# Junshuai-Song/Graph-Embedding

Hardware: AMD Instinct MI355X
Metric: walk-steps/sec (node2vec) (higher is better)
Workload: dtype int32 ids / f64 accept tests

## Files before the change

### graph-embedding_amd/csrc/gw_capi.cpp

```cpp
#include <stdarg.h>
#include <stdio.h>
#include <string.h>

#include <algorithm>
#include <string>
#include <vector>

#include <hip/hip_runtime_api.h>

#include "gw_internal.h"

int gw_load_edgelist_impl(gw_graph* g, const char* path, const char* delim, int semantics,
                          int directed, int weighted, int64_t vcount);
int gw_rmat_impl(gw_graph* g, int scale, int edge_factor, double a, double b, double c,
                 uint64_t seed);
int gw_rmat_java_impl(gw_graph* g, int64_t n, int64_t m, double a, double b, double c, uint64_t seed);
int gw_write_walks_impl(const gw_graph* g, const char* path, const int32_t* walks,
                        const int32_t* lens, int64_t nwalks, int walk_len, std::string* err);
int gw_write_sim_dense_impl(const char* path, const double* rows, const int32_t* row_ids,
                            int64_t nrows, int64_t n, int topk, const std::string& sep,
                            int decimals, std::string* err);
int gw_write_sim_topk_impl(const char* path, const int32_t* ids, const double* scores,
                           const int32_t* row_ids, int64_t nrows, int topk,
                           const std::string& sep, int decimals, std::string* err);
void gw_java_double_to_string(double v, std::string* out);
int gw_write_sim_cachemap_impl(const char* path, const int32_t* keys, const float* vals, const int32_t* sizes,
                               const int32_t* row_ids, int64_t nrows, int capacity, int topk,
                               const std::string& sep, std::string* err);
void gw_select_fixed_max_pq_impl(const double* rows, int64_t nrows, int64_t n, int k, double min_score,
                                 int32_t* out_ids);
int gw_hip_device_count(int* count);

static thread_local std::string tls_err;

void gw_set_tls_error(const std::string& s) { tls_err = s; }

int gw_fail(gw_graph* g, int code, const char* fmt, ...) {
  char buf[1024];
  va_list ap;
  va_start(ap, fmt);
  vsnprintf(buf, sizeof buf, fmt, ap);
  va_end(ap);
  if (g) g->err = buf;
  tls_err = buf;
  return code;
}

static int ret(gw_graph* g, int rc) {
  if (rc != GW_OK && g) tls_err = g->err;
  return rc;
}

extern "C" {

const char* gw_version(void) { return "graphwalk 0.1.0 (gfx950)"; }

const char* gw_last_error(const gw_graph* g) {
  if (g) return g->err.c_str();
  return tls_err.c_str();
}

const char* gw_strerror(int code) {
  switch (code) {
    case GW_OK: return "ok";
    case GW_ERR_INVALID: return "invalid argument";
    case GW_ERR_IO: return "I/O error";
    case GW_ERR_PARSE: return "parse error";
    case GW_ERR_NOMEM: return "out of memory";
    case GW_ERR_DEVICE: return "HIP device error";
    case GW_ERR_STATE: return "invalid call order";
    case GW_ERR_UNSUPPORTED: return "unsupported";
    case GW_ERR_RANGE: return "id out of range";
    case GW_ERR_KEY: return "missing key";
    case GW_ERR_ZERODIV: return "division by zero";
    case GW_ERR_CAPACITY: return "capacity exceeded";
    default: return "unknown error";
  }
}

gw_device_guard::gw_device_guard(int dev) {
  if (dev < 0) return;
  int cur = -1;
  if (hipGetDevice(&cur) != hipSuccess) {
    ok = false;
    return;
  }
  if (cur == dev) return;
  if (hipSetDevice(dev) != hipSuccess) {
    ok = false;
    return;
  }
  prev = cur;
}
gw_device_guard::~gw_device_guard() {
  if (prev >= 0) (void)hipSetDevice(prev);
}

int gw_device_count(int* count) {
  if (!count) return gw_fail(nullptr, GW_ERR_INVALID, "count is NULL");
  int rc = gw_hip_device_count(count);
  if (rc != GW_OK) return gw_fail(nullptr, rc, "no HIP device visible");
  return GW_OK;
}

int gw_graph_load_edgelist(const char* path, const char* delim, int semantics, int directed,
                           int weighted, int64_t vcount, gw_graph** out) {
  if (!path || !out) return gw_fail(nullptr, GW_ERR_INVALID, "path/out is NULL");
  *out = nullptr;
  if (semantics == GW_SEM_JAVA_MULTI && (weighted || directed))
    return gw_fail(nullptr, GW_ERR_UNSUPPORTED, "JAVA_MULTI graphs are undirected and unweighted (Graph.java:12)");
  gw_graph* g = new gw_graph();
  int rc = gw_load_edgelist_impl(g, path, delim, semantics, directed, weighted, vcount);
  if (rc != GW_OK) {
    tls_err = g->err;
    delete g;
    return rc;
  }
  *out = g;
  return GW_OK;
}

int gw_graph_from_edges(int64_t m, const int64_t* src, const int64_t* dst, const double* w,
                        int semantics, int directed, int64_t vcount, gw_graph** out) {
  if (!out || m < 0 || (m > 0 && (!src || !dst))) return gw_fail(nullptr, GW_ERR_INVALID, "bad edge arrays");
  *out = nullptr;
  gw_graph* g = new gw_graph();
  int rc;
  if (semantics == GW_SEM_NX_SIMPLE)
    rc = gw_build_nx_simple(g, m, src, dst, w, directed);
  else if (semantics == GW_SEM_JAVA_MULTI)
    rc = (w || directed) ? gw_fail(g, GW_ERR_UNSUPPORTED, "JAVA_MULTI graphs are undirected and unweighted")
                         : gw_build_java_multi(g, m, src, dst, vcount);
  else
    rc = gw_fail(g, GW_ERR_INVALID, "unknown semantics %d", semantics);
  if (rc != GW_OK) {
    tls_err = g->err;
    delete g;
    return rc;
  }
  *out = g;
  return GW_OK;
}

int gw_graph_from_csr(int64_t n, const int64_t* offsets, const int32_t* nbrs, const double* weights,
                      const int64_t* labels, const int32_t* node_order, int semantics, int directed,
                      gw_graph** out) {
  if (!out || n < 0 || !offsets) return gw_fail(nullptr, GW_ERR_INVALID, "bad CSR arguments");
  *out = nullptr;
  if (semantics != GW_SEM_NX_SIMPLE && semantics != GW_SEM_JAVA_MULTI)
    return gw_fail(nullptr, GW_ERR_INVALID, "unknown semantics %d", semantics);
  if (n >= (int64_t)INT32_MAX) return gw_fail(nullptr, GW_ERR_UNSUPPORTED, "too many vertices");
  if (offsets[0] != 0) return gw_fail(nullptr, GW_ERR_INVALID, "offsets[0] != 0");
  for (int64_t v = 0; v < n; ++v)
    if (offsets[v + 1] < offsets[v]) return gw_fail(nullptr, GW_ERR_INVALID, "offsets not monotone at %lld", (long long)v);
  const int64_t nnz = offsets[n];
  if (nnz > 0 && !nbrs) return gw_fail(nullptr, GW_ERR_INVALID, "nbrs is NULL");
  for (int64_t v = 0; v < n; ++v)
    for (int64_t k = offsets[v]; k < offsets[v + 1]; ++k) {
      if (nbrs[k] < 0 || nbrs[k] >= n) return gw_fail(nullptr, GW_ERR_RANGE, "neighbour id %d out of range", nbrs[k]);
      if (semantics == GW_SEM_NX_SIMPLE && k > offsets[v] && nbrs[k] <= nbrs[k - 1])
        return gw_fail(nullptr, GW_ERR_INVALID, "NX_SIMPLE rows must be strictly increasing (row %lld)", (long long)v);
    }
  gw_graph* g = new gw_graph();
  g->semantics = semantics;
  g->directed = directed ? 1 : 0;
  g->weighted = weights ? 1 : 0;
  g->n = n;
  g->nnz = nnz;
  g->offsets.assign(offsets, offsets + n + 1);
  g->nbrs.assign(nbrs, nbrs + nnz);
  if (weights) g->weights.assign(weights, weights + nnz);
  g->labels.resize(n);
  g->order.resize(n);
  std::vector<char> seen(n, 0);
  for (int64_t v = 0; v < n; ++v) {
    g->labels[v] = labels ? labels[v] : v;
    int32_t o = node_order ? node_order[v] : (int32_t)v;
    if (o < 0 || o >= n || seen[o]) {
      delete g;
      return gw_fail(nullptr, GW_ERR_INVALID, "node_order is not a permutation of [0,n)");
    }
    seen[o] = 1;
    g->order[v] = o;
  }
  g->max_degree = 0;
  for (int64_t v = 0; v < n; ++v) g->max_degree = std::max<int64_t>(g->max_degree, offsets[v + 1] - offsets[v]);
  *out = g;
  return GW_OK;
}

int gw_graph_rmat(int scale, int edge_factor, double a, double b, double c, uint64_t seed,
                  gw_graph** out) {
  if (!out) return gw_fail(nullptr, GW_ERR_INVALID, "out is NULL");
  *out = nullptr;
  gw_graph* g = new gw_graph();
  int rc = gw_rmat_impl(g, scale, edge_factor, a, b, c, seed);
  if (rc != GW_OK) {
    tls_err = g->err;
    delete g;
    return rc;
  }
  *out = g;
  return GW_OK;
}

int gw_graph_rmat_java(int64_t n, int64_t m, double a, double b, double c, uint64_t seed, gw_graph** out) {
  if (!out) return gw_fail(nullptr, GW_ERR_INVALID, "out is NULL");
  *out = nullptr;
  gw_graph* g = new gw_graph();
  int rc = gw_rmat_java_impl(g, n, m, a, b, c, seed);
  if (rc != GW_OK) {
    tls_err = g->err;
    delete g;
    return rc;
  }
  *out = g;
  return GW_OK;
}

int gw_graph_info(const gw_graph* g, gw_graph_info_t* info) {
  if (!g || !info) return gw_fail(nullptr, GW_ERR_INVALID, "NULL handle/info");
  info->n = g->n;
  info->nnz = g->nnz;
  info->max_degree = g->max_degree;
  info->edge_alias_entries = g->edge_alias_entries;
  info->semantics = g->semantics;
  info->directed = g->directed;
  info->weighted = g->weighted;
  info->device = g->device;
  info->sampler_bytes = (g->d.bs_nbr ? g->bitset_words * 4 + g->nnz * (int64_t)sizeof(gw_bs_nbr) : 0) +
                        (g->d.sent ? g->nnz * (int64_t)sizeof(gw_ts_ent) : 0) +
                        (g->d.eh ? 4 * g->nnz * (int64_t)sizeof(int32_t) : 0);
  info->n2v_mode = g->n2v_prepared ? g->n2v_mode : -1;
  info->listed = (g->n2v_prepared && g->n2v_mode == GW_N2V_REJECTION && g->d.bs_nbr) ? 1 : 0;
  return GW_OK;
}

int gw_graph_export_csr(const gw_graph* g, int64_t* offsets, int32_t* nbrs, double* weights,
                        int64_t* labels, int32_t* node_order) {
  if (!g) return gw_fail(nullptr, GW_ERR_INVALID, "NULL handle");
  if (offsets) memcpy(offsets, g->offsets.data(), sizeof(int64_t) * (g->n + 1));
  if (nbrs && g->nnz) memcpy(nbrs, g->nbrs.data(), sizeof(int32_t) * g->nnz);
  if (weights && g->nnz) {
    if (g->weighted)
      memcpy(weights, g->weights.data(), sizeof(double) * g->nnz);
    else
      for (int64_t i = 0; i < g->nnz; ++i) weights[i] = 1.0;
  }
  if (labels && g->n) memcpy(labels, g->labels.data(), sizeof(int64_t) * g->n);
  if (node_order && g->n) memcpy(node_order, g->order.data(), sizeof(int32_t) * g->n);
  return GW_OK;
}

int gw_graph_free(gw_graph* g) {
  if (!g) return GW_OK;
  {
    gw_device_guard dg(g->device);
    gw_dev_release(g);
  }
  delete g;
  return GW_OK;
}

int gw_graph_set_options(gw_graph* g, const gw_options_t* opt) {
  if (!g) return gw_fail(nullptr, GW_ERR_INVALID, "NULL handle");
  if (!opt) {
    g->opt = gw_options_t{0, 0, -1, 0, 0, 0, 0};
    return GW_OK;
  }
  if (opt->table_budget_bytes < 0 || opt->expected_steps < 0 || opt->listed < -1 || opt->listed > 1 ||
      opt->simrank_hbm_row < 0 || opt->simrank_hbm_row > 1 || opt->host_chunk_bytes < 0 ||
      opt->topsim_part_shrink < 0 || opt->topsim_part_shrink > 8 || opt->simrank_window < 0)
    return gw_fail(g, GW_ERR_INVALID, "option out of range");
  g->opt = *opt;
  return GW_OK;
}

int gw_graph_get_options(const gw_graph* g, gw_options_t* opt) {
  if (!g || !opt) return gw_fail(nullptr, GW_ERR_INVALID, "NULL argument");
  *opt = g->opt;
  return GW_OK;
}

int gw_graph_to_device(gw_graph* g, int device) {
  if (!g) return gw_fail(nullptr, GW_ERR_INVALID, "NULL handle");
  GW_GUARD_DEVICE(g, device);
  return ret(g, gw_dev_upload(g, device));
}

int gw_n2v_prepare(gw_graph* g, double p, double q, int mode) {
  if (!g) return gw_fail(nullptr, GW_ERR_INVALID, "NULL handle");
  GW_GUARD_DEVICE(g, g->device);
  if (!(p > 0) || !(q > 0)) return ret(g, gw_fail(g, GW_ERR_ZERODIV, "p and q must be > 0 (node2vec.py:70-76 divides by them)"));
  if (mode != GW_N2V_REPLAY && mode != GW_N2V_REJECTION && mode != GW_N2V_BITSET && mode != GW_N2V_AUTO)
    return ret(g, gw_fail(g, GW_ERR_INVALID, "unknown mode %d", mode));
  if (mode == GW_N2V_BITSET && (g->weighted || g->directed || g->semantics != GW_SEM_NX_SIMPLE))
    return ret(g, gw_fail(g, GW_ERR_UNSUPPORTED, "GW_N2V_BITSET needs an unweighted undirected NX_SIMPLE graph"));
  if (g->semantics != GW_SEM_NX_SIMPLE && !(p == 1.0 && q == 1.0))
    return ret(g, gw_fail(g, GW_ERR_UNSUPPORTED, "biased walks need NX_SIMPLE semantics (sorted rows)"));
  if (g->weighted) {
    for (int64_t v = 0; v < g->n; ++v) {
      double s = 0;
      for (int64_t k = g->offsets[v]; k < g->offsets[v + 1]; ++k) s += g->weights[k];
      if (g->offsets[v + 1] > g->offsets[v] && s == 0.0)
        return ret(g, gw_fail(g, GW_ERR_ZERODIV, "weights of vertex %lld sum to 0 (node2vec.py:95)", (long long)g->labels[v]));
    }
  }
  return ret(g, gw_dev_n2v_prepare(g, p, q, mode));
}

int gw_n2v_export_alias(const gw_graph* g_, int32_t* node_J, double* node_q, int64_t* edge_off,
                        int32_t* edge_J, double* edge_q);

int gw_alias_setup(int device, const double* probs, int64_t K, int64_t* J, double* q) {
  if (K < 0 || (K > 0 && (!probs || !J || !q))) return gw_fail(nullptr, GW_ERR_INVALID, "bad arrays");
  std::string err;
  GW_GUARD_DEVICE(nullptr, device);
  int rc = gw_dev_alias_setup(device, probs, K, J, q, &err);
  if (rc != GW_OK) return gw_fail(nullptr, rc, "%s", err.c_str());
  return GW_OK;
}

int gw_n2v_walks_replay(gw_graph* g, int walk_len, int64_t nwalks, const int32_t* starts,
                        const double* uniforms, int64_t n_uniforms, int32_t* out_walks,
                        int32_t* out_len, int64_t* uniforms_used) {
  if (!g) return gw_fail(nullptr, GW_ERR_INVALID, "NULL handle");
  GW_GUARD_DEVICE(g, g->device);
  if (!g->n2v_prepared || g->n2v_mode != GW_N2V_REPLAY)
    return ret(g, gw_fail(g, GW_ERR_STATE, "call gw_n2v_prepare(..., GW_N2V_REPLAY) first"));
  if (walk_len < 1 || nwalks < 0 || (nwalks > 0 && (!starts || !out_walks || !out_len)) ||
      n_uniforms < 0 || (n_uniforms > 0 && !uniforms))
    return ret(g, gw_fail(g, GW_ERR_INVALID, "bad arguments"));
  for (int64_t w = 0; w < nwalks; ++w)
    if (starts[w] < 0 || starts[w] >= g->n) return ret(g, gw_fail(g, GW_ERR_KEY, "start vertex %d not in graph", starts[w]));
  if (nwalks == 0) {
    if (uniforms_used) *uniforms_used = 0;
    return GW_OK;
  }
  return ret(g, gw_dev_n2v_walks_replay(g, walk_len, nwalks, starts, uniforms, n_uniforms, out_walks,
                                        out_len, uniforms_used));
}

int gw_n2v_walks(gw_graph* g, int walk_len, uint64_t seed, int64_t walk_begin, int64_t walk_count,
                 int shuffle, int32_t* out_walks_dev, int32_t* out_len_dev, uint64_t* counters_dev,
                 void* stream) {
  if (!g) return gw_fail(nullptr, GW_ERR_INVALID, "NULL handle");
  GW_GUARD_DEVICE(g, g->device);
  if (!g->n2v_prepared) return ret(g, gw_fail(g, GW_ERR_STATE, "call gw_n2v_prepare first"));
  if (walk_len < 1 || walk_begin < 0 || walk_count < 0 || (walk_count > 0 && !out_walks_dev))
    return ret(g, gw_fail(g, GW_ERR_INVALID, "bad arguments"));
  if (g->n == 0) return walk_count == 0 ? GW_OK : ret(g, gw_fail(g, GW_ERR_INVALID, "empty graph"));
  return ret(g, gw_dev_n2v_walks(g, walk_len, seed, walk_begin, walk_count, shuffle, out_walks_dev,
                                 out_len_dev, counters_dev, stream));
}

int gw_topsim_prepare(gw_graph* g, int variant, int sample, int step, int topk) {
  if (!g) return gw_fail(nullptr, GW_ERR_INVALID, "NULL handle");
  GW_GUARD_DEVICE(g, g->device);
  return ret(g, gw_dev_topsim_prepare(g, variant, sample, step, topk));
}

int gw_topsim(gw_graph* g, int variant, int sample, int step, double C, uint64_t seed,
              const int32_t* sources_dev, int64_t nsrc, int topk, int32_t* out_ids_dev,
              double* out_scores_dev, int64_t* stats_dev, void* stream) {
  if (!g) return gw_fail(nullptr, GW_ERR_INVALID, "NULL handle");
  GW_GUARD_DEVICE(g, g->device);
  if (g->device < 0) return ret(g, gw_fail(g, GW_ERR_STATE, "graph is not on a device"));
  if (nsrc < 0 || (nsrc > 0 && (!sources_dev || !out_ids_dev || !out_scores_dev)) || topk < 0)
    return ret(g, gw_fail(g, GW_ERR_INVALID, "bad arguments"));
  return ret(g, gw_dev_topsim(g, variant, sample, step, C, seed, sources_dev, nsrc, topk, out_ids_dev,
                              out_scores_dev, nullptr, stats_dev, stream));
}

int gw_topsim_dense(gw_graph* g, int variant, int sample, int step, double C, uint64_t seed,
                    const int32_t* sources_dev, int64_t nsrc, double* out_rows_dev,
                    int64_t* stats_dev, void* stream) {
  if (!g) return gw_fail(nullptr, GW_ERR_INVALID, "NULL handle");
  GW_GUARD_DEVICE(g, g->device);
  if (g->device < 0) return ret(g, gw_fail(g, GW_ERR_STATE, "graph is not on a device"));
  if (nsrc < 0 || (nsrc > 0 && (!sources_dev || !out_rows_dev)))
    return ret(g, gw_fail(g, GW_ERR_INVALID, "bad arguments"));
  return ret(g, gw_dev_topsim(g, variant, sample, step, C, seed, sources_dev, nsrc, 0, nullptr, nullptr,
                              out_rows_dev, stats_dev, stream));
}

int gw_topsim_sparse(gw_graph* g, int variant, int sample, int step, double C, uint64_t seed,
                     const int32_t* sources_dev, int64_t nsrc, int64_t capacity, int64_t* row_begin_dev,
                     int32_t* row_len_dev, int32_t* out_ids_dev, double* out_scores_dev, int64_t* used_dev,
                     int64_t* stats_dev, void* stream) {
  if (!g) return gw_fail(nullptr, GW_ERR_INVALID, "NULL handle");
  GW_GUARD_DEVICE(g, g->device);
  if (g->device < 0) return ret(g, gw_fail(g, GW_ERR_STATE, "graph is not on a device"));
  if (nsrc < 0 || capacity < 0 || !used_dev ||
      (nsrc > 0 && (!sources_dev || !row_begin_dev || !row_len_dev || (capacity > 0 && (!out_ids_dev || !out_scores_dev)))))
    return ret(g, gw_fail(g, GW_ERR_INVALID, "bad arguments"));
  if (hipMemsetAsync(used_dev, 0, sizeof(int64_t), (hipStream_t)stream) != hipSuccess)
    return ret(g, gw_fail(g, GW_ERR_DEVICE, "hipMemsetAsync(used_dev) failed"));
  gw_ts_sparse sp;
  sp.cap = capacity;
  sp.begin = row_begin_dev;
  sp.len = row_len_dev;
  sp.ids = out_ids_dev;
  sp.scores = out_scores_dev;
  sp.cursor = reinterpret_cast<unsigned long long*>(used_dev);
  return ret(g, gw_dev_topsim(g, variant, sample, step, C, seed, sources_dev, nsrc, 0, nullptr, nullptr, nullptr,
                              stats_dev, stream, &sp));
}

int gw_topsim_m(gw_graph* g, int variant, int capacity, int sample, int step, double C, uint64_t seed,
                const int32_t* sources_dev, int64_t nsrc, int32_t* out_keys_dev, float* out_vals_dev,
                int32_t* out_size_dev, int64_t* stats_dev, void* stream) {
  if (!g) return gw_fail(nullptr, GW_ERR_INVALID, "NULL handle");
  GW_GUARD_DEVICE(g, g->device);
  if (g->device < 0) return ret(g, gw_fail(g, GW_ERR_STATE, "graph is not on a device"));
  if (nsrc < 0 || capacity < 1 || (nsrc > 0 && (!sources_dev || !out_keys_dev || !out_vals_dev || !out_size_dev)))
    return ret(g, gw_fail(g, GW_ERR_INVALID, "bad arguments"));
  return ret(g, gw_dev_topsim_m(g, variant, capacity, sample, step, C, seed, sources_dev, nsrc, out_keys_dev,
                                out_vals_dev, out_size_dev, stats_dev, stream));
}

int gw_topsim_double(gw_graph* g, int sample, int step, double C, uint64_t seed, double* sim_dev, void* stream) {
  if (!g) return gw_fail(nullptr, GW_ERR_INVALID, "NULL handle");
  GW_GUARD_DEVICE(g, g->device);
  if (g->n > 0 && !sim_dev) return ret(g, gw_fail(g, GW_ERR_INVALID, "bad arguments"));
  return ret(g, gw_dev_topsim_double(g, sample, step, C, seed, sim_dev, stream));
}

int gw_topsim_dev(gw_graph* g, int sample, int step, int topK, int singleStep, double C, uint64_t seed,
                  const int32_t* cand_dev, double* sim_dev, void* stream) {
  if (!g) return gw_fail(nullptr, GW_ERR_INVALID, "NULL handle");
  GW_GUARD_DEVICE(g, g->device);
  if (g->n > 0 && (!sim_dev || (topK > 0 && !cand_dev))) return ret(g, gw_fail(g, GW_ERR_INVALID, "bad arguments"));
  return ret(g, gw_dev_topsim_dev(g, sample, step, topK, singleStep, C, seed, cand_dev, sim_dev, stream));
}

int gw_double_random_walk(gw_graph* g, int sample, int step, double C, uint64_t seed, double* sim_dev, void* stream) {
  if (!g) return gw_fail(nullptr, GW_ERR_INVALID, "NULL handle");
  GW_GUARD_DEVICE(g, g->device);
  if (g->n > 0 && !sim_dev) return ret(g, gw_fail(g, GW_ERR_INVALID, "bad arguments"));
  return ret(g, gw_dev_double_random_walk(g, sample, step, C, seed, sim_dev, stream));
}

int gw_simrank_naive(gw_graph* g, double C, int iters, double* sim_dev, void* stream) {
  if (!g) return gw_fail(nullptr, GW_ERR_INVALID, "NULL handle");
  GW_GUARD_DEVICE(g, g->device);
  if (g->device < 0) return ret(g, gw_fail(g, GW_ERR_STATE, "graph is not on a device"));
  if (g->directed) return ret(g, gw_fail(g, GW_ERR_UNSUPPORTED, "naive SimRank needs an undirected graph"));
  if (iters < 0 || (g->n > 0 && !sim_dev)) return ret(g, gw_fail(g, GW_ERR_INVALID, "bad arguments"));
  return ret(g, gw_dev_simrank_naive(g, C, iters, sim_dev, stream));
}

int gw_write_walks_text(const gw_graph* g, const char* path, const int32_t* walks,
                        const int32_t* lens, int64_t nwalks, int walk_len) {
  if (!g || !path || (nwalks > 0 && !walks) || walk_len < 1)
    return gw_fail(nullptr, GW_ERR_INVALID, "bad arguments");
  std::string err;
  int rc = gw_write_walks_impl(g, path, walks, lens, nwalks, walk_len, &err);
  if (rc != GW_OK) return gw_fail(nullptr, rc, "%s", err.c_str());
  return GW_OK;
}

int gw_write_sim_text_dense(const char* path, const double* rows, const int32_t* row_ids,
                            int64_t nrows, int64_t n, int topk, const char* sep, int decimals) {
  if (!path || (nrows > 0 && !rows) || n < 0 || topk < 0 || decimals < 0 || decimals > 30)
    return gw_fail(nullptr, GW_ERR_INVALID, "bad arguments");
  std::string err;
  int rc = gw_write_sim_dense_impl(path, rows, row_ids, nrows, n, topk, sep ? sep : ",", decimals, &err);
  if (rc != GW_OK) return gw_fail(nullptr, rc, "%s", err.c_str());
  return GW_OK;
}

int gw_write_sim_text_topk(const char* path, const int32_t* ids, const double* scores,
                           const int32_t* row_ids, int64_t nrows, int topk, const char* sep,
                           int decimals) {
  if (!path || (nrows > 0 && (!ids || !scores)) || topk < 0 || decimals < 0 || decimals > 30)
    return gw_fail(nullptr, GW_ERR_INVALID, "bad arguments");
  std::string err;
  int rc = gw_write_sim_topk_impl(path, ids, scores, row_ids, nrows, topk, sep ? sep : ",", decimals, &err);
  if (rc != GW_OK) return gw_fail(nullptr, rc, "%s", err.c_str());
  return GW_OK;
}

int gw_write_sim_text_sparse(const char* path, const int64_t* row_begin, const int32_t* row_len, const int32_t* ids,
                             const double* scores, const int32_t* row_ids, int64_t nrows, int64_t n, int topk,
                             const char* sep, int decimals) {
  if (!path || n < 0 || topk < 0 || decimals < 0 || decimals > 30 || nrows < 0 ||
      (nrows > 0 && (!row_begin || !row_len)))
    return gw_fail(nullptr, GW_ERR_INVALID, "bad arguments");
  for (int64_t r = 0; r < nrows; ++r)
    if (row_len[r] > 0 && (!ids || !scores || row_begin[r] < 0))
      return gw_fail(nullptr, GW_ERR_INVALID, "bad arguments");
  std::string err;
  int rc = gw_write_sim_sparse_impl(path, row_begin, row_len, ids, scores, row_ids, nrows, n, topk, sep ? sep : ",",
                                    decimals, false, &err);
  if (rc != GW_OK) return gw_fail(nullptr, rc, "%s", err.c_str());
  return GW_OK;
}

int gw_select_fixed_max_pq(const double* rows, int64_t nrows, int64_t n, int k, double min_score, int32_t* out_ids) {
  if ((nrows > 0 && (!rows || !out_ids)) || n < 0 || k < 0) return gw_fail(nullptr, GW_ERR_INVALID, "bad arguments");
  gw_select_fixed_max_pq_impl(rows, nrows, n, k, min_score, out_ids);
  return GW_OK;
}

int gw_write_sim_text_cachemap(const char* path, const int32_t* keys, const float* vals, const int32_t* sizes,
                               const int32_t* row_ids, int64_t nrows, int capacity, int topk, const char* sep) {
  if (!path || (nrows > 0 && (!keys || !vals || !sizes)) || capacity < 1 || topk < 0)
    return gw_fail(nullptr, GW_ERR_INVALID, "bad arguments");
  for (int64_t r = 0; r < nrows; ++r)
    if (sizes[r] < 0 || sizes[r] > capacity) return gw_fail(nullptr, GW_ERR_INVALID, "row size outside [0, capacity]");
  std::string err;
  int rc = gw_write_sim_cachemap_impl(path, keys, vals, sizes, row_ids, nrows, capacity, topk, sep ? sep : ",", &err);
  if (rc != GW_OK) return gw_fail(nullptr, rc, "%s", err.c_str());
  return GW_OK;
}

int gw_format_java_double(double v, char* buf, int64_t buflen) {
  std::string s;
  gw_java_double_to_string(v, &s);
  if (!buf || buflen < (int64_t)s.size() + 1) return gw_fail(nullptr, GW_ERR_RANGE, "buffer too small (%lld B needed)",
                                                             (long long)s.size() + 1);
  memcpy(buf, s.c_str(), s.size() + 1);
  return GW_OK;
}

}
```

### graph-embedding_amd/csrc/gw_internal.h

```cpp
#pragma once
#include <stdint.h>

#include <string>
#include <vector>

#include "../../include/graphwalk.h"

#ifdef GW_DIAG
#include <cstdlib>
constexpr bool kGwDiag = true;
#define GW_DIAG_ENV(name) std::getenv(name)
#else
constexpr bool kGwDiag = false;
#define GW_DIAG_ENV(name) ((const char*)nullptr)
#endif

constexpr uint32_t GW_BS_PACK_D = 65536;
struct gw_bs_nbr {
  uint32_t x, d;
  uint32_t off;
  uint32_t meta;
  uint32_t r[12];
};
#if defined(__HIPCC__)
#define GW_BS_HD __host__ __device__
#else
#define GW_BS_HD
#endif
GW_BS_HD inline uint32_t gw_bs_pw(uint32_t d) { return d < GW_BS_PACK_D ? 11u : 10u; }
GW_BS_HD inline uint32_t gw_bs_bits(uint32_t d) { return 32u * gw_bs_pw(d); }
GW_BS_HD inline bool gw_bs_is_list(uint32_t c, uint32_t d) { return c <= 22u && d < GW_BS_PACK_D; }
GW_BS_HD inline bool gw_bs_is_inline(uint32_t d) { return d <= gw_bs_bits(d); }
GW_BS_HD inline int gw_bs_ef_l(uint32_t c, uint32_t d) { return 31 - __builtin_clz(d / c); }
GW_BS_HD inline bool gw_bs_is_ef(uint32_t c, uint32_t d) {
  if (gw_bs_is_list(c, d) || gw_bs_is_inline(d) || c == 0) return false;
  const int l = gw_bs_ef_l(c, d);
  return (uint64_t)c * l + c + ((d - 1) >> l) + 1 <= (uint64_t)gw_bs_bits(d);
}
static_assert(sizeof(gw_bs_nbr) == 64, "bitset entry must be one 64 B sector");

struct alignas(16) gw_ts_ent {
  int32_t x, d;
  int64_t off;
};

struct gw_dev_graph {
  int64_t n = 0, nnz = 0;
  int64_t* offsets = nullptr;
  int32_t* nbrs = nullptr;
  double* weights = nullptr;
  double* wsum = nullptr;
  int32_t* order = nullptr;
  int32_t* deg = nullptr;
  int32_t* node_J = nullptr;
  double* node_q = nullptr;
  int64_t* edge_off = nullptr;
  int32_t* edge_J = nullptr;
  double* edge_q = nullptr;
  uint32_t* bitmap = nullptr;
  int32_t* eh = nullptr;
  uint32_t* bs_region = nullptr;
  gw_bs_nbr* bs_nbr = nullptr;
  gw_ts_ent* sent = nullptr;
};



struct gw_topsim_ws {
  int variant = -1, sample = 0, step = 0, topk = 0;
  int blocks = 0;
  int64_t level_cap = 0;
  int64_t spawn_cap = 0;
  int64_t touch_cap = 0;
  int lds_row = 0;
  size_t lds_bytes = 0;
  int32_t* lvl_vertex = nullptr;
  int32_t* lvl_parent = nullptr;
  int32_t* lvl_deg = nullptr;
  int64_t* lvl_off = nullptr;
  gw_ts_ent* ent = nullptr;
  double* lvl_mass = nullptr;
  int32_t* child_off = nullptr;
  int32_t* spawn_node = nullptr;
  int32_t* spawn_level = nullptr;
  int32_t* spawn_first = nullptr;
  double* spawn_mass = nullptr;
  double* acc_row = nullptr;
  double* ov_list = nullptr;
  int32_t* touched = nullptr;
  int64_t app_cap = 0;
  double* app = nullptr;
  int32_t* claim = nullptr;
  long long* redo = nullptr;
  int pipe = 0;
  int diag_pipe = -1;
  int64_t enum_cap = 0;
  int32_t* enum_tgt = nullptr;
  double* enum_val = nullptr;
  int32_t* dsel_id = nullptr;
  double* dsel_val = nullptr;
  unsigned int* src_counter = nullptr;
  int* error_flag = nullptr;
  char kernel[32] = {0};
  int last_launches = 0;
};

struct gw_ts_sparse {
  int64_t cap = 0;
  int64_t* begin = nullptr;
  int32_t* len = nullptr;
  int32_t* ids = nullptr;
  double* scores = nullptr;
  unsigned long long* cursor = nullptr;
};

struct gw_graph {
  gw_options_t opt{0, 0, -1, 0, 0, 0, 0};
  int semantics = 0;
  int directed = 0;
  int weighted = 0;
  int64_t n = 0, nnz = 0, max_degree = 0;
  std::vector<int64_t> offsets;
  std::vector<int32_t> nbrs;
  std::vector<double> weights;
  std::vector<int64_t> labels;
  std::vector<int32_t> order;
  int device = -1;
  gw_dev_graph d;
  int n2v_prepared = 0;
  int n2v_mode = -1;
  double p = 1.0, q = 1.0;
  int64_t edge_alias_entries = 0;
  int64_t bitset_words = 0;
  double bs_model_s = -1.0;
  gw_topsim_ws ts;
  double* sr_work = nullptr;
  double* sr_x = nullptr;
  uint32_t* sr_ent = nullptr;
  uint16_t* sr_heads = nullptr;
  int64_t* sr_off = nullptr;
  int64_t* sr_poff = nullptr;
  int32_t* sr_rows = nullptr;
  int64_t sr_n = 0, sr_m = 0;
  std::string err;
};

struct gw_device_guard {
  int prev = -1;
  bool ok = true;
  explicit gw_device_guard(int dev);
  ~gw_device_guard();
  gw_device_guard(const gw_device_guard&) = delete;
  gw_device_guard& operator=(const gw_device_guard&) = delete;
};

#define GW_GUARD_DEVICE(g, dev)                                                              \
  gw_device_guard gw_dg_(dev);                                                               \
  if (!gw_dg_.ok) return gw_fail((g), GW_ERR_DEVICE, "cannot select HIP device %d", (int)(dev))

int gw_write_sim_sparse_impl(const char* path, const int64_t* begin, const int32_t* len, const int32_t* ids,
                             const double* scores, const int32_t* row_ids, int64_t nrows, int64_t n, int topk,
                             const std::string& sep, int decimals, bool append, std::string* err);

int gw_fail(gw_graph* g, int code, const char* fmt, ...);
void gw_set_tls_error(const std::string& s);

int gw_build_nx_simple(gw_graph* g, int64_t m, const int64_t* src,
                       const int64_t* dst, const double* w, int directed);
int gw_build_java_multi(gw_graph* g, int64_t m, const int64_t* src,
                        const int64_t* dst, int64_t vcount);

int gw_dev_upload(gw_graph* g, int device);
void gw_dev_release(gw_graph* g);
int gw_dev_n2v_prepare(gw_graph* g, double p, double q, int mode);
int gw_dev_alias_setup(int device, const double* probs, int64_t K, int64_t* J,
                       double* q, std::string* err);
int gw_dev_n2v_walks_replay(gw_graph* g, int walk_len, int64_t nwalks,
                            const int32_t* starts, const double* uniforms,
                            int64_t n_uniforms, int32_t* out_walks,
                            int32_t* out_len, int64_t* uniforms_used);
void gw_dev_bitset_release(gw_graph* g);
void gw_dev_simrank_release(gw_graph* g);
int gw_dev_topsim_double(gw_graph* g, int sample, int step, double C, uint64_t seed, double* sim_dev, void* stream);
int gw_dev_topsim_dev(gw_graph* g, int sample_total, int step, int topK, int singleStep, double C, uint64_t seed,
                      const int32_t* cand_dev, double* sim_dev, void* stream);
int gw_dev_double_random_walk(gw_graph* g, int sample, int step, double C, uint64_t seed, double* sim_dev,
                              void* stream);
int gw_dev_topsim_m(gw_graph* g, int variant, int capacity, int sample, int step, double C, uint64_t seed,
                    const int32_t* sources_dev, int64_t nsrc, int32_t* out_keys_dev, float* out_vals_dev,
                    int32_t* out_size_dev, int64_t* stats_dev, void* stream);
int gw_dev_simrank_naive(gw_graph* g, double C, int iters, double* sim_dev, void* stream);
int gw_dev_bitset_build(gw_graph* g, int64_t budget_bytes, bool lists_only = false);
double gw_bitset_build_model_s(gw_graph* g);
int gw_dev_walk_bitset_launch(gw_graph* g, int L, uint64_t seed, int64_t walk_begin, int64_t walk_count,
                              int shuffle, int32_t* out_dev, int32_t* len_dev, uint64_t* counters_dev,
                              void* stream);
int gw_dev_walk_listed_launch(gw_graph* g, int L, uint64_t seed, int64_t walk_begin, int64_t walk_count,
                              int shuffle, int32_t* out_dev, int32_t* len_dev, uint64_t* counters_dev,
                              void* stream);
int gw_dev_n2v_walks(gw_graph* g, int walk_len, uint64_t seed,
                     int64_t walk_begin, int64_t walk_count, int shuffle,
                     int32_t* out_walks_dev, int32_t* out_len_dev,
                     uint64_t* counters_dev, void* stream);
int gw_dev_topsim_prepare(gw_graph* g, int variant, int sample, int step,
                          int topk);
int gw_dev_topsim(gw_graph* g, int variant, int sample, int step, double C,
                  uint64_t seed, const int32_t* sources_dev, int64_t nsrc,
                  int topk, int32_t* out_ids_dev, double* out_scores_dev,
                  double* out_rows_dev, int64_t* stats_dev, void* stream,
                  const gw_ts_sparse* sparse = nullptr);
```

### graph-embedding_amd/csrc/gw_n2v.hip

```cpp
#include <hip/hip_runtime.h>
#include <hipcub/hipcub.hpp>

#include <algorithm>
#include <cmath>
#include <cstdlib>
#include <vector>

#include "gw_device_common.h"

namespace {

constexpr int kBlock = 256;

inline unsigned grid_for(int64_t n, int block = kBlock) {
  int64_t g = (n + block - 1) / block;
  return (unsigned)std::max<int64_t>(1, g);
}

template <typename T>
int dev_alloc(gw_graph* g, T** p, int64_t count) {
  *p = nullptr;
  if (count <= 0) return GW_OK;
  hipError_t e = hipMalloc((void**)p, sizeof(T) * (size_t)count);
  if (e != hipSuccess) {
    g->err = std::string("hipMalloc(") + std::to_string(sizeof(T) * (size_t)count) + " B): " + hipGetErrorString(e);
    *p = nullptr;
    return GW_ERR_NOMEM;
  }
  return GW_OK;
}

template <typename T>
void dev_free(T*& p) {
  if (p) (void)hipFree(p);
  p = nullptr;
}

__global__ void k_degree_wsum(int64_t n, const int64_t* __restrict__ off,
                              const double* __restrict__ w, int32_t* __restrict__ deg,
                              double* __restrict__ wsum) {
  int64_t v = (int64_t)blockIdx.x * blockDim.x + threadIdx.x;
  if (v >= n) return;
  int64_t b = off[v], e = off[v + 1];
  deg[v] = (int32_t)(e - b);
  if (w) {
    double s = 0.0;
    for (int64_t k = b; k < e; ++k) s += w[k];
    wsum[v] = s;
  }
}

__global__ void k_alias_nodes(int64_t n, const int64_t* __restrict__ off,
                              const double* __restrict__ w, int32_t* __restrict__ J,
                              double* __restrict__ q, int32_t* __restrict__ stack) {
  int64_t v = (int64_t)blockIdx.x * blockDim.x + threadIdx.x;
  if (v >= n) return;
  int64_t b = off[v], e = off[v + 1];
  int64_t K = e - b;
  if (K == 0) return;
  double norm = 0.0;
  if (w) {
    for (int64_t k = b; k < e; ++k) norm += w[k];
  } else {
    norm = (double)K;
  }
  for (int64_t k = 0; k < K; ++k) q[b + k] = (w ? w[b + k] : 1.0) / norm;
  gw_alias_build<int32_t>(q + b, J + b, stack + b, K);
}

__global__ void k_edge_sizes(int64_t nnz, const int32_t* __restrict__ nbrs,
                             const int32_t* __restrict__ deg, int64_t* __restrict__ sz) {
  int64_t e = (int64_t)blockIdx.x * blockDim.x + threadIdx.x;
  if (e >= nnz) return;
  sz[e] = deg[nbrs[e]];
}

__global__ void k_alias_edges(int64_t n, int64_t nnz, const int64_t* __restrict__ off,
                              const int32_t* __restrict__ nbrs, const double* __restrict__ w,
                              double p, double q, const int64_t* __restrict__ eoff,
                              int32_t* __restrict__ eJ, double* __restrict__ eq,
                              int32_t* __restrict__ stack) {
  int64_t e = (int64_t)blockIdx.x * blockDim.x + threadIdx.x;
  if (e >= nnz) return;
  int64_t lo = 0, hi = n;
  while (lo < hi) {
    int64_t mid = (lo + hi) >> 1;
    if (off[mid + 1] <= e)
      lo = mid + 1;
    else
      hi = mid;
  }
  const int32_t src = (int32_t)lo;
  const int32_t dst = nbrs[e];
  const int64_t db = off[dst], de = off[dst + 1];
  const int64_t K = de - db;
  if (K == 0) return;
  double* qt = eq + eoff[e];
  double norm = 0.0;
  for (int64_t k = 0; k < K; ++k) {
    const int32_t x = nbrs[db + k];
    const double wx = w ? w[db + k] : 1.0;
    double u;
    if (x == src) {
      u = wx / p;
    } else if (gw_row_find(nbrs, off[x], off[x + 1], src) >= 0) {
      u = wx;
    } else {
      u = wx / q;
    }
    qt[k] = u;
    norm += u;
  }
  for (int64_t k = 0; k < K; ++k) qt[k] = qt[k] / norm;
  gw_alias_build<int32_t>(qt, eJ + eoff[e], stack + eoff[e], K);
}

__global__ void k_alias_single(const double* __restrict__ probs, int64_t K,
                               int64_t* __restrict__ J, double* __restrict__ q,
                               int32_t* __restrict__ stack) {
  if (blockIdx.x != 0 || threadIdx.x != 0) return;
  for (int64_t k = 0; k < K; ++k) q[k] = probs[k];
  gw_alias_build<int64_t>(q, J, stack, K);
}

__global__ void k_walk_replay(gw_dev_graph G, int L, int64_t nwalks,
                              const int32_t* __restrict__ starts,
                              const double* __restrict__ U, int64_t nU,
                              const int64_t* __restrict__ uoff,
                              int32_t* __restrict__ out, int32_t* __restrict__ lens,
                              int* __restrict__ overrun) {
  int64_t w = (int64_t)blockIdx.x * blockDim.x + threadIdx.x;
  if (w >= nwalks) return;
  int32_t* row = out + w * (int64_t)L;
  int32_t cur = starts[w];
  row[0] = cur;
  int len = 1;
  int64_t o = uoff[w];
  int64_t slot = -1;
  while (len < L) {
    const int64_t b = G.offsets[cur], e = G.offsets[cur + 1];
    const int64_t d = e - b;
    if (d == 0) break;
    if (o + 2 > nU) {
      atomicOr(overrun, 1);
      break;
    }
    const double u1 = U[o], u2 = U[o + 1];
    o += 2;
    int64_t kk = (int64_t)floor(u1 * (double)d);
    if (kk >= d) kk = d - 1;
    const int32_t* J;
    const double* q;
    if (len == 1) {
      J = G.node_J + b;
      q = G.node_q + b;
    } else {
      const int64_t t0 = G.edge_off[slot];
      J = G.edge_J + t0;
      q = G.edge_q + t0;
    }
    const int64_t idx = (u2 < q[kk]) ? kk : (int64_t)J[kk];
    slot = b + idx;
    cur = G.nbrs[slot];
    row[len++] = cur;
  }
  for (int t = len; t < L; ++t) row[t] = -1;
  lens[w] = len;
}

struct N2VParams {
  double a_p, a_q;
  double M;
  double lo;
  double extra;
  double h_prev;
  uint32_t k0, k1;
  uint32_t pk0, pk1;
  uint32_t diag;
  double mix_o;
  double mix_p;
  double mix_prev;
};

template <bool WEIGHTED>
__device__ __forceinline__ int64_t draw_first_order(const gw_dev_graph& G, int64_t b,
                                                    int64_t d, uint32_t ux, uint32_t ulo, uint32_t uy) {
  int64_t kk = (int64_t)gw_index(ux, ulo, (uint32_t)d);
  if (!WEIGHTED) return kk;
  return (gw_u01(uy) < G.node_q[b + kk]) ? kk : (int64_t)G.node_J[b + kk];
}

__device__ __forceinline__ uint64_t gw_bm_bit(int64_t rowb, int64_t deg, int32_t key) {
  const uint32_t h = (uint32_t)key * 0x9E3779B1u;
  return 16ull * (uint64_t)rowb + (((uint64_t)h * (uint64_t)(16 * deg)) >> 32);
}

__device__ __forceinline__ bool gw_has_edge(const gw_dev_graph& G, int64_t rb, int64_t re,
                                            int32_t key) {
  if (G.eh) return gw_eh_has(G.eh, rb, re, key);
  if (G.bitmap) {
    const uint64_t bit = gw_bm_bit(rb, re - rb, key);
    if (!((G.bitmap[bit >> 5] >> (bit & 31)) & 1u)) return false;
  }
  return gw_row_find(G.nbrs, rb, re, key) >= 0;
}

__global__ void k_scale_ent(gw_dev_graph G, gw_ts_ent* __restrict__ ent) {
  const int64_t e = (int64_t)blockIdx.x * blockDim.x + threadIdx.x;
  if (e >= G.nnz) return;
  const int32_t x = G.nbrs[e];
  gw_ts_ent v;
  v.x = x;
  v.off = G.offsets[x];
  v.d = (int32_t)(G.offsets[x + 1] - v.off);
  ent[e] = v;
}

__global__ void k_build_ehash(gw_dev_graph G, int32_t* __restrict__ eh) {
  const int64_t e = (int64_t)blockIdx.x * blockDim.x + threadIdx.x;
  if (e >= G.nnz) return;
  int64_t lo = 0, hi = G.n;
  while (lo < hi) {
    const int64_t mid = (lo + hi) >> 1;
    if (G.offsets[mid + 1] <= e)
      lo = mid + 1;
    else
      hi = mid;
  }
  const int64_t rb = G.offsets[lo];
  const uint32_t nbk = (uint32_t)(G.offsets[lo + 1] - rb);
  const int32_t key = G.nbrs[e];
  int32_t* t = eh + 4 * rb;
  uint32_t h = gw_eh_slot(key, nbk);
  for (uint32_t i = 0; i < nbk; ++i) {
    for (int j = 0; j < 4; ++j) {
      const int32_t old = atomicCAS(&t[4 * h + j], -1, key);
      if (old == -1 || old == key) return;
    }
    h = h + 1 == nbk ? 0u : h + 1;
  }
}

__global__ void k_build_bitmap(int64_t n, const int64_t* __restrict__ off,
                               const int32_t* __restrict__ nbrs, uint32_t* __restrict__ bm) {
  int64_t v = (int64_t)blockIdx.x * blockDim.x + threadIdx.x;
  if (v >= n) return;
  const int64_t b = off[v], e = off[v + 1];
  for (int64_t k = b; k < e; ++k) {
    const uint64_t bit = gw_bm_bit(b, e - b, nbrs[k]);
    atomicOr(&bm[bit >> 5], 1u << (bit & 31));
  }
}

constexpr int kStage = 16;

template <bool FIRST_ORDER, bool WEIGHTED, bool DIRECTED, bool ENT, bool MIX = false>
__global__ void __launch_bounds__(kBlock)
k_walk_scale(gw_dev_graph G, N2VParams P, int L, int64_t walk_begin, int64_t walk_count,
             int shuffle, int32_t* __restrict__ out, int32_t* __restrict__ lens,
             unsigned long long* __restrict__ counters) {
  __shared__ int32_t s_stage[kBlock / 64][kStage][64];
  __shared__ int32_t s_ids[kBlock / 64][64];
  const int lane = threadIdx.x & 63;
  int32_t* stage = &s_stage[threadIdx.x >> 6][0][lane];
  const int64_t i = (int64_t)blockIdx.x * blockDim.x + threadIdx.x;
  const bool valid = i < walk_count;
  unsigned long long my_steps = 0, my_trials = 0;
  const int64_t w = walk_begin + (valid ? i : 0);
  int32_t cur = -1;
  int32_t prev = -1;
  int64_t pb = 0, pe = 0;
  double w_back = 1.0;
  bool back_ok = false;
  const bool vec_ok = (L & 3) == 0;
  int len = L;
  uint32_t trial = 0;
  const uint32_t c0 = (uint32_t)w, c1 = (uint32_t)((uint64_t)w >> 32);
  int64_t b = 0, e = 0;
  int64_t nb = 0;
  int32_t nd = 0;
  double Wcur = 0.0;
  if (valid) {
    const uint64_t it = (uint64_t)w / (uint64_t)G.n;
    const uint64_t pos = (uint64_t)w % (uint64_t)G.n;
    const uint64_t sp = shuffle ? gw_feistel_perm(pos, (uint64_t)G.n, P.pk0, P.pk1, (uint32_t)it) : pos;
    cur = G.order[sp];
    len = 1;
    b = G.offsets[cur];
    e = G.offsets[cur + 1];
    Wcur = WEIGHTED ? G.wsum[cur] : (double)(e - b);
  }
  stage[0] = cur;
  for (;;) {
    const bool active = len < L && e != b;
    if (__ballot(active) == 0ull) break;
    bool ready = false;
    int flen = 0;
    if (active) {
      const int64_t d = e - b;
      bool acc;
      int64_t slot;
      int32_t next;
      if (FIRST_ORDER || len == 1) {
        gw_u4 u = gw_philox(c0, c1, (uint32_t)len, 0u, P.k0, P.k1);
        trial = 1;
        slot = b + draw_first_order<WEIGHTED>(G, b, d, u.x, u.z, u.y);
        if (FIRST_ORDER && ENT) {
          const gw_ts_ent en = gw_ts_load(G.sent + slot);
          next = en.x;
          nb = en.off;
          nd = en.d;
        } else {
          next = G.nbrs[slot];
        }
        acc = true;
      } else if (MIX && pe - pb < d) {
        const gw_u4 u = gw_philox(c0, c1, (uint32_t)len, trial, P.k0, P.k1);
        ++trial;
        const int64_t dp = pe - pb;
        const double Ac = (double)d * P.a_q;
        const double H = P.mix_o + Ac + (double)dp * P.mix_p;
        const double r = gw_u01(u.z) * H;
        if (r < P.mix_o) {
          slot = -1;
          next = prev;
          acc = true;
        } else {
          const bool from_cur = r < P.mix_o + Ac;
          slot = (from_cur ? b : pb) + (int64_t)gw_index(u.x, u.y, (uint32_t)(from_cur ? d : dp));
          if (ENT) {
            const gw_ts_ent en = gw_ts_load(G.sent + slot);
            next = en.x;
            nb = en.off;
            nd = en.d;
          } else {
            next = G.nbrs[slot];
          }
          if (from_cur)
            acc = next != prev || gw_u01(u.w) < P.mix_prev;
          else
            acc = next != prev && gw_has_edge(G, b, e, next);
          if (trial >= (1u << 24) && from_cur) acc = true;
        }
      } else {
        const gw_u4 u = gw_philox(c0, c1, (uint32_t)len, trial, P.k0, P.k1);
        ++trial;
        const double out_area = (back_ok && P.extra > 0.0) ? P.extra * w_back : 0.0;
        const double A = P.M * Wcur + out_area;
        if (out_area > 0.0 && gw_u01(u.z) * A < out_area) {
          slot = -1;
          next = prev;
          acc = true;
        } else {
          const uint32_t ulo =
              WEIGHTED ? gw_philox(c0, c1, (uint32_t)len, (trial - 1u) | 0x80000000u, P.k0, P.k1).x : u.y;
          slot = b + draw_first_order<WEIGHTED>(G, b, d, u.x, ulo, u.y);
          if (ENT) {
            const gw_ts_ent en = gw_ts_load(G.sent + slot);
            next = en.x;
            nb = en.off;
            nd = en.d;
          } else {
            next = G.nbrs[slot];
          }
          const double t = gw_u01(u.w) * P.M;
          if (next == prev) {
            acc = t < P.h_prev;
          } else if (t < P.lo) {
            acc = true;
          } else {
            bool adj;
            if (DIRECTED)
              adj = ENT ? gw_has_edge(G, nb, nb + nd, prev)
                           : gw_has_edge(G, G.offsets[next], G.offsets[next + 1], prev);
            else
              adj = gw_has_edge(G, pb, pe, next);
            acc = t < (adj ? 1.0 : P.a_q);
          }
          if (trial >= (1u << 24)) acc = true;
        }
      }
      if (acc) {
        my_trials += trial;
        trial = 0;
        if (DIRECTED) {
          if (!FIRST_ORDER && P.extra > 0.0) {
            const int64_t bs = gw_row_find(G.nbrs, G.offsets[next], G.offsets[next + 1], cur);
            back_ok = bs >= 0;
            w_back = (back_ok && WEIGHTED) ? G.weights[bs] : 1.0;
          }
        } else if (slot >= 0) {
          back_ok = true;
          w_back = WEIGHTED ? G.weights[slot] : 1.0;
        }
        const int64_t ob = pb, oe = pe;
        prev = cur;
        pb = b;
        pe = e;
        cur = next;
        stage[64 * (len & (kStage - 1))] = cur;
        ready = (len & (kStage - 1)) == kStage - 1;
        flen = len;
        ++len;
        if (FIRST_ORDER && ENT) {
          b = nb;
          e = nb + nd;
        } else if (ENT && !FIRST_ORDER && len > 2) {
          if (slot >= 0) {
            b = nb;
            e = nb + nd;
          } else {
            b = ob;
            e = oe;
          }
        } else {
          b = G.offsets[cur];
          e = G.offsets[cur + 1];
        }
        if (WEIGHTED) Wcur = G.wsum[cur];
        else Wcur = (double)(e - b);
      }
    }
    const unsigned long long rm = __ballot(ready);
    if (rm && !(kGwDiag && P.diag)) {
      if (vec_ok) {
        const int nready = __popcll(rm);
        int32_t* ids = s_ids[threadIdx.x >> 6];
        __builtin_amdgcn_wave_barrier();
        if (ready)
          ids[__builtin_amdgcn_mbcnt_hi((uint32_t)(rm >> 32), __builtin_amdgcn_mbcnt_lo((uint32_t)rm, 0u))] = lane;
        __builtin_amdgcn_wave_barrier();
        const int32_t* sw = &s_stage[threadIdx.x >> 6][0][0];
        for (int j = 0; 16 * j < nready; ++j) {
          const int q = 16 * j + (lane >> 2), p4 = 4 * (lane & 3);
          const int r = ids[q < nready ? q : nready - 1];
          const int lr = __shfl(flen, r, 64);
          const int64_t ir = ((int64_t)__shfl((int)(i >> 32), r, 64) << 32) | (uint32_t)__shfl((int)i, r, 64);
          if (q < nready) {
            const int4 v = make_int4(sw[64 * p4 + r], sw[64 * (p4 + 1) + r], sw[64 * (p4 + 2) + r], sw[64 * (p4 + 3) + r]);
            *reinterpret_cast<int4*>(out + ir * (int64_t)L + (lr - (kStage - 1)) + p4) = v;
          }
        }
        __builtin_amdgcn_wave_barrier();
      } else if (ready) {
        int32_t* dst = out + i * (int64_t)L + (flen - (kStage - 1));
        for (int j = 0; j < kStage; ++j) dst[j] = stage[64 * j];
      }
    }
  }
  if (valid) {
    int32_t* row = out + i * (int64_t)L;
    const int base = len & ~(kStage - 1);
    for (int t = base; t < len; ++t) row[t] = stage[64 * (t - base)];
    for (int t = len; t < L; ++t) row[t] = -1;
    if (lens) lens[i] = len;
    my_steps = (unsigned long long)(len - 1);
  }
  if (counters) {
    for (int off = 32; off > 0; off >>= 1) {
      my_steps += __shfl_down(my_steps, off, 64);
      my_trials += __shfl_down(my_trials, off, 64);
    }
    if ((threadIdx.x & 63) == 0) {
      atomicAdd(&counters[0], my_steps);
      atomicAdd(&counters[1], my_trials);
    }
  }
}

}

void gw_dev_release(gw_graph* g) {
  if (g->device < 0) return;
  (void)hipSetDevice(g->device);
  gw_dev_graph& d = g->d;
  dev_free(d.offsets);
  dev_free(d.nbrs);
  dev_free(d.weights);
  dev_free(d.wsum);
  dev_free(d.order);
  dev_free(d.deg);
  dev_free(d.node_J);
  dev_free(d.node_q);
  dev_free(d.edge_off);
  dev_free(d.edge_J);
  dev_free(d.edge_q);
  dev_free(d.bitmap);
  dev_free(d.eh);
  dev_free(d.sent);
  gw_dev_bitset_release(g);
  gw_dev_simrank_release(g);
  gw_topsim_ws& t = g->ts;
  dev_free(t.lvl_vertex);
  dev_free(t.lvl_parent);
  dev_free(t.lvl_deg);
  dev_free(t.lvl_off);
  dev_free(t.ent);
  dev_free(t.lvl_mass);
  dev_free(t.child_off);
  dev_free(t.spawn_node);
  dev_free(t.spawn_mass);
  dev_free(t.spawn_level);
  dev_free(t.spawn_first);
  dev_free(t.acc_row);
  dev_free(t.ov_list);
  dev_free(t.touched);
  dev_free(t.app);
  dev_free(t.enum_tgt);
  dev_free(t.enum_val);
  dev_free(t.dsel_id);
  dev_free(t.dsel_val);
  dev_free(t.src_counter);
  dev_free(t.error_flag);
  t = gw_topsim_ws();
  g->n2v_prepared = 0;
  g->bs_model_s = -1.0;
  g->device = -1;
}

int gw_dev_upload(gw_graph* g, int device) {
  int count = 0;
  if (hipGetDeviceCount(&count) != hipSuccess || count == 0) {
    g->err = "no HIP device visible (libgraphwalk has no CPU fallback)";
    return GW_ERR_DEVICE;
  }
  if (device < 0 || device >= count) {
    g->err = "device ordinal out of range";
    return GW_ERR_INVALID;
  }
  if (g->device >= 0) gw_dev_release(g);
  GW_HIP_TRY(hipSetDevice(device));
  g->device = device;
  gw_dev_graph& d = g->d;
  d.n = g->n;
  d.nnz = g->nnz;
  int rc;
  if ((rc = dev_alloc(g, &d.offsets, g->n + 1)) || (rc = dev_alloc(g, &d.nbrs, g->nnz)) ||
      (rc = dev_alloc(g, &d.order, g->n)) || (rc = dev_alloc(g, &d.deg, g->n))) {
    gw_dev_release(g);
    return rc;
  }
  GW_HIP_TRY(hipMemcpy(d.offsets, g->offsets.data(), sizeof(int64_t) * (g->n + 1), hipMemcpyHostToDevice));
  if (g->nnz) GW_HIP_TRY(hipMemcpy(d.nbrs, g->nbrs.data(), sizeof(int32_t) * g->nnz, hipMemcpyHostToDevice));
  if (g->n) GW_HIP_TRY(hipMemcpy(d.order, g->order.data(), sizeof(int32_t) * g->n, hipMemcpyHostToDevice));
  if (g->weighted) {
    if ((rc = dev_alloc(g, &d.weights, g->nnz)) || (rc = dev_alloc(g, &d.wsum, g->n))) {
      gw_dev_release(g);
      return rc;
    }
    if (g->nnz) GW_HIP_TRY(hipMemcpy(d.weights, g->weights.data(), sizeof(double) * g->nnz, hipMemcpyHostToDevice));
  }
  if (g->n) {
    k_degree_wsum<<<grid_for(g->n), kBlock>>>(g->n, d.offsets, d.weights, d.deg, d.wsum);
    GW_HIP_TRY(hipGetLastError());
  }
  GW_HIP_TRY(hipDeviceSynchronize());
  return GW_OK;
}

static int64_t table_budget(gw_graph* g) {
  size_t fr = 0, tot = 0;
  int64_t budget = hipMemGetInfo(&fr, &tot) == hipSuccess ? (int64_t)(fr / 2) : 0;
  if (g->opt.table_budget_bytes > 0) budget = std::min(budget, g->opt.table_budget_bytes);
  return budget;
}

static bool listed_pays(gw_graph* g, double q) {
  if (q >= 1.0) return false;
  if (g->opt.listed == 0) return false;
  if (g->opt.listed == 1 || g->opt.expected_steps <= 0) return true;
  const double save_s = (double)g->opt.expected_steps * (0.46 / 4.9e10);
  const double build_s = gw_bitset_build_model_s(g);
  if (build_s < 0) {
    (void)hipGetLastError();
    return false;
  }
  return save_s > build_s;
}

constexpr double kBitsetStepSeconds = 1.0 / 3.2e10;
constexpr double kRejTrialSeconds = 3.0e-11;

static int n2v_prepare_auto(gw_graph* g, double p, double q) {
  const bool bs_ok = !g->weighted && !g->directed && g->semantics == GW_SEM_NX_SIMPLE && !(p == 1.0 && q == 1.0) &&
                     g->nnz > 0 && g->nnz < (int64_t)0xFFFFFFFF;
  auto bitset_or_rejection = [&]() {
    int rc = gw_dev_n2v_prepare(g, p, q, GW_N2V_BITSET);
    if (rc == GW_ERR_CAPACITY || rc == GW_ERR_NOMEM || rc == GW_ERR_UNSUPPORTED) {
      (void)hipGetLastError();
      g->err.clear();
      rc = gw_dev_n2v_prepare(g, p, q, GW_N2V_REJECTION);
    }
    return rc;
  };
  if (!bs_ok) return gw_dev_n2v_prepare(g, p, q, GW_N2V_REJECTION);
  const int64_t steps = g->opt.expected_steps;
  if (steps <= 0) return bitset_or_rejection();
  const int32_t listed_opt = g->opt.listed;
  g->opt.listed = 0;
  int rc = gw_dev_n2v_prepare(g, p, q, GW_N2V_REJECTION);
  g->opt.listed = listed_opt;
  if (rc != GW_OK) return rc;
  auto keep_rejection = [&]() {
    if (listed_opt != 0 && listed_pays(g, q)) return gw_dev_n2v_prepare(g, p, q, GW_N2V_REJECTION);
    return GW_OK;
  };
  const int64_t pw = std::min<int64_t>(65536, std::max<int64_t>(g->n, 1));
  const int L = 80;
  int32_t* buf = nullptr;
  uint64_t* cnt = nullptr;
  double t_rej = -1.0;
  if (dev_alloc(g, &buf, pw * L) == GW_OK && dev_alloc(g, &cnt, 2) == GW_OK) {
    uint64_t h[2] = {0, 0};
    const bool ok = hipMemset(cnt, 0, 2 * sizeof(uint64_t)) == hipSuccess &&
                    gw_dev_n2v_walks(g, L, 0x5eedull, 0, pw, 1, buf, nullptr, cnt, nullptr) == GW_OK &&
                    hipMemcpy(h, cnt, sizeof h, hipMemcpyDeviceToHost) == hipSuccess;
    if (ok && h[0] > 0) t_rej = (double)h[1] / (double)h[0] * kRejTrialSeconds;
  }
  dev_free(buf);
  dev_free(cnt);
  (void)hipGetLastError();
  if (t_rej < 0) return keep_rejection();
  const double build = gw_bitset_build_model_s(g);
  (void)hipGetLastError();
  const double bitset_s = build + (double)steps * kBitsetStepSeconds;
  const double rejection_s = (double)steps * t_rej;
  if (build < 0 || bitset_s >= rejection_s) return keep_rejection();
  return bitset_or_rejection();
}

int gw_dev_n2v_prepare(gw_graph* g, double p, double q, int mode) {
  if (mode == GW_N2V_AUTO) return n2v_prepare_auto(g, p, q);
  if (g->device < 0) {
    g->err = "graph is not on a device (call gw_graph_to_device)";
    return GW_ERR_STATE;
  }
  GW_HIP_TRY(hipSetDevice(g->device));
  gw_dev_graph& d = g->d;
  dev_free(d.node_J);
  dev_free(d.node_q);
  dev_free(d.edge_off);
  dev_free(d.edge_J);
  dev_free(d.edge_q);
  g->edge_alias_entries = 0;
  g->n2v_prepared = 0;
  const bool need_node_alias = g->weighted || mode == GW_N2V_REPLAY;
  int rc;
  int32_t* stack = nullptr;
  if (need_node_alias && g->nnz) {
    if ((rc = dev_alloc(g, &d.node_J, g->nnz)) || (rc = dev_alloc(g, &d.node_q, g->nnz)) ||
        (rc = dev_alloc(g, &stack, g->nnz)))
      return rc;
    k_alias_nodes<<<grid_for(g->n), kBlock>>>(g->n, d.offsets, d.weights, d.node_J, d.node_q, stack);
    GW_HIP_TRY(hipGetLastError());
    GW_HIP_TRY(hipDeviceSynchronize());
    dev_free(stack);
  }
  if (mode == GW_N2V_REPLAY && g->nnz) {
    int64_t* sz = nullptr;
    if ((rc = dev_alloc(g, &d.edge_off, g->nnz + 1)) || (rc = dev_alloc(g, &sz, g->nnz + 1))) return rc;
    k_edge_sizes<<<grid_for(g->nnz), kBlock>>>(g->nnz, d.nbrs, d.deg, sz);
    GW_HIP_TRY(hipMemset(sz + g->nnz, 0, sizeof(int64_t)));
    size_t tmp_bytes = 0;
    GW_HIP_TRY(hipcub::DeviceScan::ExclusiveSum(nullptr, tmp_bytes, sz, d.edge_off, g->nnz + 1));
    void* tmp = nullptr;
    if ((rc = dev_alloc(g, (char**)&tmp, (int64_t)tmp_bytes + 1))) return rc;
    GW_HIP_TRY(hipcub::DeviceScan::ExclusiveSum(tmp, tmp_bytes, sz, d.edge_off, g->nnz + 1));
    GW_HIP_TRY(hipDeviceSynchronize());
    dev_free(tmp);
    dev_free(sz);
    int64_t total = 0;
    GW_HIP_TRY(hipMemcpy(&total, d.edge_off + g->nnz, sizeof(int64_t), hipMemcpyDeviceToHost));
    if (total > (int64_t)1 << 30) {
      dev_free(d.edge_off);
      g->err = "per-edge alias tables need " + std::to_string(total) +
               " entries (sum of deg^2); use GW_N2V_REJECTION at this scale";
      return GW_ERR_CAPACITY;
    }
    if ((rc = dev_alloc(g, &d.edge_J, total)) || (rc = dev_alloc(g, &d.edge_q, total)) ||
        (rc = dev_alloc(g, &stack, total)))
      return rc;
    k_alias_edges<<<grid_for(g->nnz), kBlock>>>(g->n, g->nnz, d.offsets, d.nbrs, d.weights, p, q,
                                                d.edge_off, d.edge_J, d.edge_q, stack);
    GW_HIP_TRY(hipGetLastError());
    GW_HIP_TRY(hipDeviceSynchronize());
    dev_free(stack);
    g->edge_alias_entries = total;
  }
  dev_free(d.bitmap);
  dev_free(d.eh);
  gw_dev_bitset_release(g);
  g->bitset_words = 0;
  const char* nobm = GW_DIAG_ENV("GW_DIAG_NO_BITMAP");
  const char* noeh = GW_DIAG_ENV("GW_DIAG_NO_EHASH");
  if (mode == GW_N2V_REJECTION && !(p == 1.0 && q == 1.0) && g->nnz && g->semantics == GW_SEM_NX_SIMPLE &&
      !(noeh && noeh[0] == '1')) {
    size_t fr = 0, tot = 0;
    const int64_t slots = 4 * g->nnz;
    if (hipMemGetInfo(&fr, &tot) == hipSuccess && (int64_t)fr / 2 > slots * 4) {
      if (dev_alloc(g, &d.eh, slots) == GW_OK) {
        GW_HIP_TRY(hipMemset(d.eh, 0xFF, sizeof(int32_t) * (size_t)slots));
        k_build_ehash<<<grid_for(g->nnz), kBlock>>>(d, d.eh);
        GW_HIP_TRY(hipGetLastError());
        GW_HIP_TRY(hipDeviceSynchronize());
      } else {
        d.eh = nullptr;
        (void)hipGetLastError();
      }
    }
  }
  if (mode == GW_N2V_REJECTION && !(p == 1.0 && q == 1.0) && !d.eh && g->nnz && !(nobm && nobm[0] == '1')) {
    const int64_t words = (16 * g->nnz + 31) / 32 + 1;
    if ((rc = dev_alloc(g, &d.bitmap, words))) return rc;
    GW_HIP_TRY(hipMemset(d.bitmap, 0, sizeof(uint32_t) * words));
    k_build_bitmap<<<grid_for(g->n), kBlock>>>(g->n, d.offsets, d.nbrs, d.bitmap);
    GW_HIP_TRY(hipGetLastError());
    GW_HIP_TRY(hipDeviceSynchronize());
  }
  dev_free(d.sent);
  const bool fo = (p == 1.0 && q == 1.0);
  bool listed = false;
  if (mode == GW_N2V_REJECTION && !fo && g->nnz && !g->weighted && !g->directed &&
      g->semantics == GW_SEM_NX_SIMPLE && !GW_DIAG_ENV("GW_DIAG_NO_LISTS") && listed_pays(g, q)) {
    rc = gw_dev_bitset_build(g, table_budget(g), true);
    if (rc == GW_OK) {
      listed = true;
    } else if (rc == GW_ERR_CAPACITY || rc == GW_ERR_NOMEM || rc == GW_ERR_UNSUPPORTED) {
      gw_dev_bitset_release(g);
      (void)hipGetLastError();
      g->err.clear();
    } else {
      return rc;
    }
  }
  const char* nosent = GW_DIAG_ENV("GW_DIAG_NO_SENT");
  if ((mode == GW_N2V_REJECTION || fo) && !listed && g->nnz && !(nosent && nosent[0] == '1')) {
    const int64_t ent_bytes = g->nnz * (int64_t)sizeof(gw_ts_ent);
    if (ent_bytes <= table_budget(g)) {
      if (dev_alloc(g, &d.sent, g->nnz) == GW_OK) {
        k_scale_ent<<<grid_for(g->nnz), kBlock>>>(d, d.sent);
        GW_HIP_TRY(hipGetLastError());
        GW_HIP_TRY(hipDeviceSynchronize());
      } else {
        d.sent = nullptr;
        (void)hipGetLastError();
      }
    }
  }
  if (mode == GW_N2V_BITSET && !(p == 1.0 && q == 1.0)) {
    if ((rc = gw_dev_bitset_build(g, table_budget(g)))) return rc;
  }
  g->p = p;
  g->q = q;
  g->n2v_mode = mode;
  g->n2v_prepared = 1;
  return GW_OK;
}

int gw_dev_alias_setup(int device, const double* probs, int64_t K, int64_t* J,
                       double* q, std::string* err) {
  int count = 0;
  if (hipGetDeviceCount(&count) != hipSuccess || count == 0) {
    *err = "no HIP device visible (libgraphwalk has no CPU fallback)";
    return GW_ERR_DEVICE;
  }
  if (K <= 0) return GW_OK;
  if (hipSetDevice(device) != hipSuccess) {
    *err = "hipSetDevice failed";
    return GW_ERR_DEVICE;
  }
  double *dp = nullptr, *dq = nullptr;
  int64_t* dJ = nullptr;
  int32_t* st = nullptr;
  hipError_t e = hipMalloc((void**)&dp, K * sizeof(double));
  if (e == hipSuccess) e = hipMalloc((void**)&dq, K * sizeof(double));
  if (e == hipSuccess) e = hipMalloc((void**)&dJ, K * sizeof(int64_t));
  if (e == hipSuccess) e = hipMalloc((void**)&st, K * sizeof(int32_t));
  if (e == hipSuccess) e = hipMemcpy(dp, probs, K * sizeof(double), hipMemcpyHostToDevice);
  if (e == hipSuccess) {
    k_alias_single<<<1, 64>>>(dp, K, dJ, dq, st);
    e = hipGetLastError();
  }
  if (e == hipSuccess) e = hipMemcpy(J, dJ, K * sizeof(int64_t), hipMemcpyDeviceToHost);
  if (e == hipSuccess) e = hipMemcpy(q, dq, K * sizeof(double), hipMemcpyDeviceToHost);
  if (dp) (void)hipFree(dp);
  if (dq) (void)hipFree(dq);
  if (dJ) (void)hipFree(dJ);
  if (st) (void)hipFree(st);
  if (e != hipSuccess) {
    *err = hipGetErrorString(e);
    return GW_ERR_DEVICE;
  }
  return GW_OK;
}

int gw_dev_n2v_walks_replay(gw_graph* g, int L, int64_t nwalks, const int32_t* starts,
                            const double* uniforms, int64_t nU, int32_t* out_walks,
                            int32_t* out_len, int64_t* used) {
  GW_HIP_TRY(hipSetDevice(g->device));
  int rc;
  int32_t *d_starts = nullptr, *d_out = nullptr, *d_len = nullptr;
  double* d_U = nullptr;
  int64_t* d_uoff = nullptr;
  int* d_over = nullptr;
  auto cleanup = [&]() {
    dev_free(d_starts);
    dev_free(d_out);
    dev_free(d_len);
    dev_free(d_U);
    dev_free(d_uoff);
    dev_free(d_over);
  };
  if ((rc = dev_alloc(g, &d_starts, nwalks)) || (rc = dev_alloc(g, &d_out, nwalks * (int64_t)L)) ||
      (rc = dev_alloc(g, &d_len, nwalks)) || (rc = dev_alloc(g, &d_U, std::max<int64_t>(nU, 1))) ||
      (rc = dev_alloc(g, &d_uoff, nwalks)) || (rc = dev_alloc(g, &d_over, 1))) {
    cleanup();
    return rc;
  }
  GW_HIP_TRY(hipMemcpy(d_starts, starts, nwalks * sizeof(int32_t), hipMemcpyHostToDevice));
  if (nU) GW_HIP_TRY(hipMemcpy(d_U, uniforms, nU * sizeof(double), hipMemcpyHostToDevice));
  GW_HIP_TRY(hipMemset(d_over, 0, sizeof(int)));
  std::vector<int64_t> uoff(nwalks);
  std::vector<int32_t> lens(nwalks, L);
  for (int64_t w = 0; w < nwalks; ++w) {
    int64_t s = starts[w];
    if (g->offsets[s + 1] == g->offsets[s]) lens[w] = 1;
  }
  std::vector<int32_t> got(nwalks);
  int64_t first_unsettled = 0;
  for (int pass = 0;; ++pass) {
    int64_t acc = 0;
    for (int64_t w = 0; w < nwalks; ++w) {
      uoff[w] = acc;
      acc += 2 * (int64_t)(lens[w] - 1);
    }
    GW_HIP_TRY(hipMemcpy(d_uoff, uoff.data(), nwalks * sizeof(int64_t), hipMemcpyHostToDevice));
    GW_HIP_TRY(hipMemset(d_over, 0, sizeof(int)));
    const int64_t todo = nwalks - first_unsettled;
    k_walk_replay<<<grid_for(todo), kBlock>>>(g->d, L, todo, d_starts + first_unsettled, d_U, nU,
                                              d_uoff + first_unsettled, d_out + first_unsettled * (int64_t)L,
                                              d_len + first_unsettled, d_over);
    GW_HIP_TRY(hipGetLastError());
    GW_HIP_TRY(hipMemcpy(got.data(), d_len, nwalks * sizeof(int32_t), hipMemcpyDeviceToHost));
    int64_t mism = -1;
    for (int64_t w = first_unsettled; w < nwalks; ++w)
      if (got[w] != lens[w]) {
        mism = w;
        break;
      }
    if (mism < 0) {
      int over = 0;
      GW_HIP_TRY(hipMemcpy(&over, d_over, sizeof(int), hipMemcpyDeviceToHost));
      if (over) {
        cleanup();
        g->err = "uniform stream exhausted (supply 2*(walk_len-1) uniforms per walk)";
        return GW_ERR_INVALID;
      }
      if (used) *used = acc;
      break;
    }
    for (int64_t w = first_unsettled; w < nwalks; ++w) lens[w] = got[w];
    first_unsettled = mism + 1;
    if (first_unsettled >= nwalks) {
      int64_t a2 = 0;
      for (int64_t w = 0; w < nwalks; ++w) a2 += 2 * (int64_t)(lens[w] - 1);
      if (used) *used = a2;
      break;
    }
  }
  GW_HIP_TRY(hipMemcpy(out_walks, d_out, nwalks * (int64_t)L * sizeof(int32_t), hipMemcpyDeviceToHost));
  GW_HIP_TRY(hipMemcpy(out_len, d_len, nwalks * sizeof(int32_t), hipMemcpyDeviceToHost));
  cleanup();
  return GW_OK;
}

int gw_dev_n2v_walks(gw_graph* g, int L, uint64_t seed, int64_t walk_begin, int64_t walk_count,
                     int shuffle, int32_t* out_dev, int32_t* len_dev, uint64_t* counters_dev,
                     void* stream) {
  if (walk_count <= 0) return GW_OK;
  constexpr int64_t kMaxLaunch = (int64_t)1 << 31;
  if (walk_count > kMaxLaunch) {
    for (int64_t o = 0; o < walk_count; o += kMaxLaunch) {
      const int rc = gw_dev_n2v_walks(g, L, seed, walk_begin + o, std::min(kMaxLaunch, walk_count - o), shuffle,
                                      out_dev + o * (int64_t)L, len_dev ? len_dev + o : nullptr, counters_dev,
                                      stream);
      if (rc != GW_OK) return rc;
    }
    return GW_OK;
  }
  const bool first_order = (g->p == 1.0 && g->q == 1.0);
  if (!first_order && g->semantics != GW_SEM_NX_SIMPLE) {
    g->err = "second-order walks need sorted rows (NX_SIMPLE semantics)";
    return GW_ERR_UNSUPPORTED;
  }
  N2VParams P;
  P.a_p = 1.0 / g->p;
  P.a_q = 1.0 / g->q;
  P.M = std::max(1.0, P.a_q);
  P.lo = std::min(1.0, P.a_q);
  P.extra = P.a_p > P.M ? P.a_p - P.M : 0.0;
  P.h_prev = std::min(P.a_p, P.M);
  P.mix_o = std::max(0.0, P.a_p - P.a_q);
  P.mix_p = 1.0 - P.a_q;
  P.mix_prev = std::min(1.0, P.a_p / P.a_q);
  P.k0 = (uint32_t)seed;
  P.k1 = (uint32_t)(seed >> 32) ^ GW_TAG_N2V_STEP;
  P.pk0 = (uint32_t)seed;
  P.pk1 = (uint32_t)(seed >> 32) ^ GW_TAG_N2V_PERM;
  {
    const char* ns = GW_DIAG_ENV("GW_DIAG_NO_STORE");
    P.diag = (ns && ns[0] == '1') ? 1u : 0u;
  }
  if (g->n2v_mode == GW_N2V_BITSET && !first_order)
    return gw_dev_walk_bitset_launch(g, L, seed, walk_begin, walk_count, shuffle, out_dev, len_dev, counters_dev,
                                     stream);
  if (g->n2v_mode == GW_N2V_REJECTION && !first_order && g->d.bs_nbr)
    return gw_dev_walk_listed_launch(g, L, seed, walk_begin, walk_count, shuffle, out_dev, len_dev, counters_dev,
                                     stream);
  hipStream_t s = (hipStream_t)stream;
  const unsigned grid = grid_for(walk_count);
  unsigned long long* C = (unsigned long long*)counters_dev;
#define GW_LAUNCH_MIX(FO, WT, DI, MX)                                                                              \
  do {                                                                                                             \
    if (g->d.sent)                                                                                                 \
      k_walk_scale<FO, WT, DI, true, MX><<<grid, kBlock, 0, s>>>(g->d, P, L, walk_begin, walk_count, shuffle,      \
                                                                 out_dev, len_dev, C);                             \
    else                                                                                                           \
      k_walk_scale<FO, WT, DI, false, MX><<<grid, kBlock, 0, s>>>(g->d, P, L, walk_begin, walk_count, shuffle,     \
                                                                  out_dev, len_dev, C);                            \
  } while (0)
#define GW_LAUNCH(FO, WT, DI) GW_LAUNCH_MIX(FO, WT, DI, false)
  const bool wt = g->weighted != 0, di = g->directed != 0;
  if (first_order) {
    if (wt) GW_LAUNCH(true, true, false);
    else GW_LAUNCH(true, false, false);
  } else if (wt) {
    if (di) GW_LAUNCH(false, true, true);
    else GW_LAUNCH(false, true, false);
  } else {
    if (di) GW_LAUNCH(false, false, true);
    else if (P.a_q < 1.0) GW_LAUNCH_MIX(false, false, false, true);
    else GW_LAUNCH(false, false, false);
  }
#undef GW_LAUNCH
#undef GW_LAUNCH_MIX
  GW_HIP_TRY(hipGetLastError());
  return GW_OK;
}

__global__ void k_philox(const uint32_t* __restrict__ in, int64_t n, uint32_t* __restrict__ out) {
  const int64_t i = (int64_t)blockIdx.x * blockDim.x + threadIdx.x;
  if (i >= n) return;
  const uint32_t* a = in + 6 * i;
  const gw_u4 r = gw_philox(a[0], a[1], a[2], a[3], a[4], a[5]);
  uint32_t* o = out + 4 * i;
  o[0] = r.x;
  o[1] = r.y;
  o[2] = r.z;
  o[3] = r.w;
}

extern "C" int gw_philox4x32(int device, const uint32_t* in, int64_t n, uint32_t* out) {
  if (n < 0 || (n > 0 && (!in || !out))) return gw_fail(nullptr, GW_ERR_INVALID, "bad arrays");
  if (n == 0) return GW_OK;
  if (device < 0) {
    for (int64_t i = 0; i < n; ++i) {
      const uint32_t* a = in + 6 * i;
      const gw_u4 r = gw_philox(a[0], a[1], a[2], a[3], a[4], a[5]);
      out[4 * i] = r.x;
      out[4 * i + 1] = r.y;
      out[4 * i + 2] = r.z;
      out[4 * i + 3] = r.w;
    }
    return GW_OK;
  }
  int count = 0;
  if (hipGetDeviceCount(&count) != hipSuccess || count == 0)
    return gw_fail(nullptr, GW_ERR_DEVICE, "no HIP device visible (libgraphwalk has no CPU fallback)");
  if (device >= count) return gw_fail(nullptr, GW_ERR_INVALID, "device ordinal out of range");
  GW_GUARD_DEVICE(nullptr, device);
  uint32_t *d_in = nullptr, *d_out = nullptr;
  hipError_t e = hipMalloc((void**)&d_in, sizeof(uint32_t) * 6 * (size_t)n);
  if (e == hipSuccess) e = hipMalloc((void**)&d_out, sizeof(uint32_t) * 4 * (size_t)n);
  if (e == hipSuccess) e = hipMemcpy(d_in, in, sizeof(uint32_t) * 6 * (size_t)n, hipMemcpyHostToDevice);
  if (e == hipSuccess) {
    k_philox<<<grid_for(n), kBlock>>>(d_in, n, d_out);
    e = hipGetLastError();
  }
  if (e == hipSuccess) e = hipMemcpy(out, d_out, sizeof(uint32_t) * 4 * (size_t)n, hipMemcpyDeviceToHost);
  if (d_in) (void)hipFree(d_in);
  if (d_out) (void)hipFree(d_out);
  if (e != hipSuccess) return gw_fail(nullptr, GW_ERR_DEVICE, "%s", hipGetErrorString(e));
  return GW_OK;
}

int gw_hip_device_count(int* count) {
  int c = 0;
  if (hipGetDeviceCount(&c) != hipSuccess) c = 0;
  *count = c;
  return c > 0 ? GW_OK : GW_ERR_DEVICE;
}

extern "C" int gw_n2v_export_alias(const gw_graph* gc, int32_t* node_J, double* node_q,
                                   int64_t* edge_off, int32_t* edge_J, double* edge_q) {
  gw_graph* g = const_cast<gw_graph*>(gc);
  if (!g) return gw_fail(nullptr, GW_ERR_INVALID, "NULL handle");
  GW_GUARD_DEVICE(g, g->device);
  if (!g->n2v_prepared) return gw_fail(g, GW_ERR_STATE, "call gw_n2v_prepare first");
  GW_HIP_TRY(hipSetDevice(g->device));
  const gw_dev_graph& d = g->d;
  if ((node_J || node_q) && !d.node_J)
    return gw_fail(g, GW_ERR_STATE, "no per-node alias tables (unweighted REJECTION mode draws uniformly)");
  if (node_J && g->nnz) GW_HIP_TRY(hipMemcpy(node_J, d.node_J, sizeof(int32_t) * g->nnz, hipMemcpyDeviceToHost));
  if (node_q && g->nnz) GW_HIP_TRY(hipMemcpy(node_q, d.node_q, sizeof(double) * g->nnz, hipMemcpyDeviceToHost));
  if (edge_off || edge_J || edge_q) {
    if (g->n2v_mode != GW_N2V_REPLAY) return gw_fail(g, GW_ERR_STATE, "per-edge tables exist only in GW_N2V_REPLAY mode");
    if (edge_off) GW_HIP_TRY(hipMemcpy(edge_off, d.edge_off, sizeof(int64_t) * (g->nnz + 1), hipMemcpyDeviceToHost));
    if (edge_J && g->edge_alias_entries)
      GW_HIP_TRY(hipMemcpy(edge_J, d.edge_J, sizeof(int32_t) * g->edge_alias_entries, hipMemcpyDeviceToHost));
    if (edge_q && g->edge_alias_entries)
      GW_HIP_TRY(hipMemcpy(edge_q, d.edge_q, sizeof(double) * g->edge_alias_entries, hipMemcpyDeviceToHost));
  }
  return GW_OK;
}

extern "C" int gw_n2v_walks_host(gw_graph* g, int walk_len, uint64_t seed, int64_t walk_begin,
                                 int64_t walk_count, int shuffle, int32_t* out_walks, int32_t* out_len,
                                 uint64_t* counters) {
  if (!g) return gw_fail(nullptr, GW_ERR_INVALID, "NULL handle");
  GW_GUARD_DEVICE(g, g->device);
  if (!g->n2v_prepared) return gw_fail(g, GW_ERR_STATE, "call gw_n2v_prepare first");
  if (walk_len < 1 || walk_begin < 0 || walk_count < 0 || (walk_count > 0 && !out_walks))
    return gw_fail(g, GW_ERR_INVALID, "bad arguments");
  if (walk_count == 0) return GW_OK;
  GW_HIP_TRY(hipSetDevice(g->device));
  const int64_t chunk_bytes = g->opt.host_chunk_bytes > 0 ? g->opt.host_chunk_bytes : (int64_t)256 << 20;
  const int64_t chunk = std::max<int64_t>(1, std::min<int64_t>(walk_count, chunk_bytes / (4 * (int64_t)walk_len)));
  const int64_t nch = (walk_count + chunk - 1) / chunk;
  int32_t *d_out[2] = {nullptr, nullptr}, *d_len[2] = {nullptr, nullptr};
  uint64_t* d_cnt = nullptr;
  hipStream_t sc = nullptr, sx = nullptr;
  hipEvent_t done[2] = {nullptr, nullptr};
  auto release = [&]() {
    for (int b = 0; b < 2; ++b) {
      dev_free(d_out[b]);
      dev_free(d_len[b]);
      if (done[b]) (void)hipEventDestroy(done[b]);
    }
    dev_free(d_cnt);
    if (sc) (void)hipStreamDestroy(sc);
    if (sx) (void)hipStreamDestroy(sx);
  };
  int rc = GW_OK;
  const int nb = nch > 1 ? 2 : 1;
  for (int b = 0; b < nb && rc == GW_OK; ++b)
    if ((rc = dev_alloc(g, &d_out[b], chunk * (int64_t)walk_len)) == GW_OK) rc = dev_alloc(g, &d_len[b], chunk);
  if (rc == GW_OK) rc = dev_alloc(g, &d_cnt, 2);
  if (rc != GW_OK) {
    release();
    return rc;
  }
  hipError_t e = hipStreamCreateWithFlags(&sc, hipStreamNonBlocking);
  if (e == hipSuccess) e = hipStreamCreateWithFlags(&sx, hipStreamNonBlocking);
  for (int b = 0; b < nb && e == hipSuccess; ++b) e = hipEventCreateWithFlags(&done[b], hipEventDisableTiming);
  if (e == hipSuccess) e = hipMemsetAsync(d_cnt, 0, 2 * sizeof(uint64_t), sc);
  auto launch = [&](int64_t k) -> int {
    const int64_t c0 = k * chunk, cn = std::min(chunk, walk_count - c0);
    const int b = (int)(k & 1);
    int r = gw_dev_n2v_walks(g, walk_len, seed, walk_begin + c0, cn, shuffle, d_out[b], d_len[b], d_cnt, sc);
    if (r == GW_OK && hipEventRecord(done[b], sc) != hipSuccess) r = GW_ERR_DEVICE;
    return r;
  };
  if (e == hipSuccess) rc = launch(0);
  for (int64_t k = 0; k < nch && e == hipSuccess && rc == GW_OK; ++k) {
    if (k + 1 < nch && (rc = launch(k + 1)) != GW_OK) break;
    const int64_t c0 = k * chunk, cn = std::min(chunk, walk_count - c0);
    const int b = (int)(k & 1);
    e = hipStreamWaitEvent(sx, done[b], 0);
    if (e == hipSuccess)
      e = hipMemcpyAsync(out_walks + c0 * walk_len, d_out[b], cn * walk_len * sizeof(int32_t),
                         hipMemcpyDeviceToHost, sx);
    if (e == hipSuccess && out_len)
      e = hipMemcpyAsync(out_len + c0, d_len[b], cn * sizeof(int32_t), hipMemcpyDeviceToHost, sx);
    if (e == hipSuccess) e = hipStreamSynchronize(sx);
  }
  if (rc == GW_OK && e == hipSuccess) e = hipStreamSynchronize(sc);
  if (rc == GW_OK && e == hipSuccess && counters)
    e = hipMemcpy(counters, d_cnt, 2 * sizeof(uint64_t), hipMemcpyDeviceToHost);
  release();
  if (rc != GW_OK) return rc;
  if (e != hipSuccess) return gw_fail(g, GW_ERR_DEVICE, "%s", hipGetErrorString(e));
  return GW_OK;
}
```

### graph-embedding_amd/csrc/gw_n2v_bitset.hip

```cpp
#include <hip/hip_runtime.h>
#include <hipcub/hipcub.hpp>

#include <algorithm>
#include <cstdlib>
#include <string>
#include <vector>

#include "gw_device_common.h"

namespace {

constexpr int kB = 256;
constexpr int kBlk = 16;
constexpr int kDirBits = 512;
constexpr int kStage = 16;

constexpr int kPDir = 8;

__host__ __device__ __forceinline__ int64_t bs_ndir(int64_t d) { return d > kDirBits ? (d + kDirBits - 1) / kDirBits : 0; }
__host__ __device__ __forceinline__ int64_t bs_round(int64_t w) { return (w + kBlk - 1) / kBlk * kBlk; }
__host__ __device__ __forceinline__ int64_t bs_boff(int64_t d) {
  return (gw_bs_is_inline((uint32_t)d) || bs_ndir(d) <= kPDir) ? 0 : bs_round(bs_ndir(d));
}
__host__ __device__ __forceinline__ int64_t bs_words(int64_t d) {
  return gw_bs_is_inline((uint32_t)d) ? 0 : bs_boff(d) + bs_round((d + 31) / 32);
}

__device__ __forceinline__ bool bs_has_edge(const gw_dev_graph& G, int64_t rb, int64_t re, int32_t key) {
  if (G.eh) return gw_eh_has(G.eh, rb, re, key);
  if (G.bitmap) {
    const uint32_t h = (uint32_t)key * 0x9E3779B1u;
    const uint64_t bit = 16ull * (uint64_t)rb + (((uint64_t)h * (uint64_t)(16 * (re - rb))) >> 32);
    if (!((G.bitmap[bit >> 5] >> (bit & 31)) & 1u)) return false;
  }
  return gw_row_find(G.nbrs, rb, re, key) >= 0;
}

__host__ __device__ __forceinline__ uint32_t bs_filt_buckets(int64_t ndir, uint32_t d) {
  return 32u * (gw_bs_pw(d) - ((ndir > 0 && ndir <= kPDir) ? 5u : 1u));
}
__host__ __device__ __forceinline__ uint32_t bs_filt_word(int64_t ndir) { return (ndir > 0 && ndir <= kPDir) ? 5u : 1u; }

__device__ __forceinline__ int word_select(uint32_t x, uint32_t j) {
  int pos = 0;
#pragma unroll
  for (int w = 16; w >= 1; w >>= 1) {
    const uint32_t lowc = (uint32_t)__popc(x & ((1u << w) - 1u));
    if (j >= lowc) {
      j -= lowc;
      x >>= w;
      pos += w;
    }
  }
  return pos;
}


enum { BS_LIST = 0, BS_INLINE = 1, BS_EF = 2, BS_REGION = 3 };
constexpr uint32_t kFiltL = 320;

__device__ __forceinline__ int64_t bs_div32(int64_t k, uint32_t d, double inv, bool* exact) {
  int64_t q = (int64_t)((double)k * inv);
  int64_t r = (k << 32) - q * (int64_t)d;
  if (r < 0) {
    --q;
    r += d;
  } else if (r >= (int64_t)d) {
    ++q;
    r -= d;
  }
  *exact = r == 0;
  return q;
}
__device__ __forceinline__ void bs_draw_range(int64_t k, uint32_t d, double inv, uint32_t* ylo, uint32_t* yhi) {
  bool ex;
  *ylo = (uint32_t)bs_div32(k, d, inv, &ex);
  const int64_t q1 = bs_div32(k + 1, d, inv, &ex);
  *yhi = (uint32_t)(q1 - (ex ? 1 : 0));
}
__device__ __forceinline__ double bs_inv32(uint32_t d) { return 4294967296.0 / (double)d; }

__device__ __forceinline__ void bs_filter_only(uint32_t* w, int64_t k, uint32_t d, double inv) {
  uint32_t ulo, uhi;
  bs_draw_range(k, d, inv, &ulo, &uhi);
  const uint32_t b0 = gw_bounded(ulo, kFiltL), b1 = gw_bounded(uhi, kFiltL);
  for (uint32_t b = b0; b <= b1; ++b) atomicOr(&w[b >> 5], 1u << (b & 31));
}
__device__ __forceinline__ int bs_mode(uint32_t c, uint32_t d) {
  return gw_bs_is_list(c, d) ? BS_LIST : gw_bs_is_inline(d) ? BS_INLINE : gw_bs_is_ef(c, d) ? BS_EF : BS_REGION;
}

constexpr uint32_t kDualC = 6;
constexpr uint32_t kMetaDual = 0x40000000u;
constexpr uint32_t kMetaStash = 0x80000000u;

__device__ __forceinline__ uint32_t bs_meta(uint32_t c, uint32_t d) {
  const uint32_t mode = (uint32_t)bs_mode(c, d);
  uint32_t l = 0, U = 0;
  if (mode == BS_EF) {
    l = (uint32_t)gw_bs_ef_l(c, d);
    U = c + ((d - 1) >> l) + 1;
  }
  const uint32_t bblk = (mode == BS_REGION) ? (uint32_t)(bs_boff(d) / kBlk) : 0u;
  return mode | (l << 2) | (U << 7) | (bblk << 16);
}
__device__ __forceinline__ bool bs_dual(uint32_t c, uint32_t c_rev, uint32_t d, uint32_t du) {
  return c <= kDualC && c_rev <= kDualC && d < GW_BS_PACK_D && du < GW_BS_PACK_D;
}
__device__ __forceinline__ uint32_t bs_meta_slot(uint32_t c, uint32_t c_rev, uint32_t d, uint32_t du) {
  return bs_dual(c, c_rev, d, du) ? (kMetaDual | (c_rev << 2)) : bs_meta(c, d);
}

struct BsEmit {
  int mode;
  bool nobits;
  uint32_t* w;
  uint32_t* dir;
  uint16_t* pdir;
  uint32_t* bits;
  int64_t ndir;
  uint32_t d;
  double inv;
  int l;
  uint32_t U;
  __device__ void operator()(int64_t k, uint32_t idx, int64_t kprev) const {
    const uint32_t bit = 1u << (k & 31);
    if (mode == BS_LIST) {
      reinterpret_cast<uint16_t*>(w)[idx] = (uint16_t)k;
    } else if (mode == BS_INLINE) {
      atomicOr(&w[k >> 5], bit);
    } else if (mode == BS_EF) {
      const uint32_t hp = (uint32_t)(k >> l) + idx;
      atomicOr(&w[hp >> 5], 1u << (hp & 31));
      if (l > 0) {
        const uint32_t lowv = (uint32_t)k & ((1u << l) - 1u), off = U + idx * (uint32_t)l, sh = off & 31;
        atomicOr(&w[off >> 5], lowv << sh);
        if (sh + (uint32_t)l > 32u) atomicOr(&w[(off >> 5) + 1], lowv >> (32 - sh));
      }
    } else {
      if (!nobits) atomicOr(&bits[k >> 5], bit);
      set_dir((kprev < 0 ? -1 : kprev / kDirBits) + 1, k / kDirBits, idx);
      uint32_t ulo, uhi;
      bs_draw_range(k, d, inv, &ulo, &uhi);
      const uint32_t F = bs_filt_buckets(ndir, d), w0 = bs_filt_word(ndir);
      const uint32_t b0 = gw_bounded(ulo, F), b1 = gw_bounded(uhi, F);
      for (uint32_t b = b0; b <= b1; ++b) atomicOr(&w[w0 + (b >> 5)], 1u << (b & 31));
    }
  }
  __device__ void set_dir(int64_t g0, int64_t g1, uint32_t count) const {
    if (ndir == 0) return;
    for (int64_t g = g0; g <= g1 && g < ndir; ++g) {
      if (pdir)
        pdir[g] = (uint16_t)count;
      else
        dir[g] = count;
    }
  }
};

__device__ __forceinline__ uint32_t* bs_payload(gw_bs_nbr* en, uint32_t d) { return en->r + (d < GW_BS_PACK_D ? 1 : 2); }
__device__ __forceinline__ uint32_t bs_c(const gw_bs_nbr* en, uint32_t d) { return d < GW_BS_PACK_D ? en->r[0] >> 16 : en->r[1]; }

__device__ __forceinline__ BsEmit bs_emit(gw_bs_nbr* en, uint32_t* reg, const uint64_t* roff, int64_t e, uint32_t c,
                                          uint32_t d) {
  BsEmit E;
  E.mode = bs_mode(c, d);
  E.nobits = false;
  E.w = bs_payload(en, d);
  E.ndir = 0;
  E.dir = E.bits = nullptr;
  E.pdir = nullptr;
  E.d = d;
  E.inv = bs_inv32(d);
  E.l = 0;
  E.U = 0;
  if (E.mode == BS_EF) {
    E.l = gw_bs_ef_l(c, d);
    E.U = c + ((d - 1) >> E.l) + 1;
  } else if (E.mode == BS_REGION) {
    E.ndir = bs_ndir(d);
    E.dir = reg + roff[e];
    E.bits = E.dir + bs_boff(d);
    if (E.ndir <= kPDir) {
      E.pdir = reinterpret_cast<uint16_t*>(E.w + 1);
      E.dir = nullptr;
    }
  }
  return E;
}

__global__ void k_bs_sizes(gw_dev_graph G, const gw_bs_nbr* __restrict__ bsn, uint64_t* __restrict__ sz,
                           int lists_only) {
  const int64_t e = (int64_t)blockIdx.x * blockDim.x + threadIdx.x;
  if (e >= G.nnz) return;
  const uint32_t d = (uint32_t)G.deg[G.nbrs[e]];
  sz[e] = (!lists_only && !gw_bs_is_inline(d) && bs_mode(bs_c(bsn + e, d), d) == BS_REGION)
              ? (uint64_t)bs_words(d) : 0ull;
}

constexpr int kTB = 512;
constexpr int kTW = kTB / 64;
constexpr int kTriH = 4096;
constexpr int kTriS = 2 * kTriH;
constexpr int kTriEB = 512;
constexpr int kTriAhead = 4;
constexpr int32_t kTriNotOwned = INT32_MIN;

constexpr double kBuildProbeRate = 7.7e10;
constexpr double kBuildSlotSeconds = 5.0e-11;

struct TriItem {
  int32_t u, j0;
};

__global__ void k_bs_iota(int64_t n, int32_t* __restrict__ a) {
  const int64_t i = (int64_t)blockIdx.x * blockDim.x + threadIdx.x;
  if (i < n) a[i] = (int32_t)i;
}

__global__ void k_bs_nitems(gw_dev_graph G, const int32_t* __restrict__ order, uint32_t* __restrict__ nit) {
  const int64_t i = (int64_t)blockIdx.x * blockDim.x + threadIdx.x;
  if (i > G.n) return;
  nit[i] = i < G.n ? (uint32_t)((G.deg[order[i]] + kTriEB - 1) / kTriEB) : 0u;
}

__global__ void k_bs_items(gw_dev_graph G, const int32_t* __restrict__ order, const uint32_t* __restrict__ itoff,
                           TriItem* __restrict__ items) {
  const int64_t i = (int64_t)blockIdx.x * blockDim.x + threadIdx.x;
  if (i >= G.n) return;
  const int32_t u = order[i];
  const uint32_t b = itoff[i], e = itoff[i + 1];
  for (uint32_t t = b; t < e; ++t) items[t] = TriItem{u, (int32_t)((t - b) * kTriEB)};
}

struct TriSlot {
  BsEmit E;
  uint32_t* gw;
  bool filt;
  bool dual;
  __device__ void operator()(int64_t k, uint32_t idx, int64_t kprev) const {
    if (filt)
      bs_filter_only(E.w, k, E.d, E.inv);
    else
      E(k, idx, kprev);
  }
};

__device__ __forceinline__ TriSlot tri_slot(gw_bs_nbr* en, uint32_t* reg, const uint64_t* roff, int64_t e, uint32_t c,
                                            uint32_t d, int lists_only, uint32_t* stage, int lane) {
  TriSlot T;
  T.filt = lists_only && bs_mode(c, d) == BS_REGION;
  T.dual = (en->meta & kMetaDual) != 0u;
  T.E = bs_emit(en, reg, roff, e, c, d);
  T.gw = T.E.w;
  T.E.w = stage;
  if (T.E.pdir) T.E.pdir = reinterpret_cast<uint16_t*>(stage + 1);
  if (lane < 12) stage[lane] = 0u;
  __builtin_amdgcn_wave_barrier();
  return T;
}

__device__ __forceinline__ void tri_prologue(const TriSlot& T, int64_t e, const uint64_t* roff, int lane) {
  if (!T.filt && T.E.mode == BS_REGION && lane == 0) T.E.w[0] = (uint32_t)(roff[e] / kBlk);
}

__device__ __forceinline__ void tri_epilogue(const TriSlot& T, int64_t klast, uint32_t c, uint32_t c_rev, int lane) {
  if (T.filt) return;
  if (T.dual) {
    if (lane < 2 * (int)kDualC && (lane < (int)kDualC ? lane >= (int)c : lane - (int)kDualC >= (int)c_rev))
      reinterpret_cast<uint16_t*>(T.E.w)[lane] = 0xFFFFu;
    return;
  }
  if (T.E.mode == BS_LIST && lane >= (int)c && lane < 2 * (int)gw_bs_pw(T.E.d))
    reinterpret_cast<uint16_t*>(T.E.w)[lane] = 0xFFFFu;
  if (T.E.mode != BS_REGION) return;
  for (int64_t g = (klast < 0 ? -1 : klast / kDirBits) + 1 + lane; g < T.E.ndir; g += 64) T.E.set_dir(g, g, c);
}

__device__ __forceinline__ void tri_flush(const TriSlot& T, bool merge, int lane) {
  __builtin_amdgcn_wave_barrier();
  const int pw = (int)gw_bs_pw(T.E.d);
  if (lane < pw) {
    const uint32_t v = T.E.w[lane];
    if (!merge)
      T.gw[lane] = v;
    else if (v)
      atomicOr(&T.gw[lane], v);
  }
  __builtin_amdgcn_wave_barrier();
}

__device__ __forceinline__ void tri_header(gw_bs_nbr* en, uint32_t x, uint32_t d, uint32_t off, uint32_t meta,
                                           uint32_t kp, uint32_t c) {
  *reinterpret_cast<uint4*>(en) = make_uint4(x, d, off, meta);
  *reinterpret_cast<uint2*>(&en->r[0]) =
      d < GW_BS_PACK_D ? make_uint2((kp & 0xFFFFu) | (c << 16), 0u) : make_uint2(kp, c);
}

template <class F>
__device__ __forceinline__ void tri_emit(const F& f, bool on, int64_t pos, uint32_t* cnt, int64_t* last, int lane,
                                         uint16_t* rev, bool need_prev) {
  const unsigned long long m = __ballot(on);
  if (!m) return;
  const unsigned long long lt = m & ((1ull << lane) - 1ull);
  const int32_t p32 = (int32_t)pos;
  int64_t prev = *last;
  if (need_prev) {
    const int32_t pin = __shfl(p32, lt ? 63 - __clzll(lt) : 0, 64);
    if (lt) prev = pin;
  }
  if (on) {
    const uint32_t idx = *cnt + (uint32_t)__popcll(lt);
    f(pos, idx, prev);
    if (rev) rev[kDualC + idx] = (uint16_t)pos;
  }
  *last = __builtin_amdgcn_readlane(p32, 63 - __clzll(m));
  *cnt += (uint32_t)__popcll(m);
}

template <bool FILL>
__global__ void __launch_bounds__(kTB) __attribute__((amdgpu_waves_per_eu(4))) k_bs_tri(gw_dev_graph G, const TriItem* __restrict__ items, uint32_t nitems,
                                                gw_bs_nbr* __restrict__ bsn,
                                                const uint64_t* __restrict__ roff, uint32_t* __restrict__ reg,
                                                int lists_only) {
  __shared__ int32_t s_key[kTriS];
  __shared__ uint16_t s_pos[kTriS];
  __shared__ uint32_t s_cuv[kTriEB], s_cvu[kTriEB], s_cur[kTriEB];
  __shared__ int32_t s_luv[kTriEB], s_lvu[kTriEB], s_kp[kTriEB];
  __shared__ int32_t s_nx[kTriEB];
  __shared__ uint32_t s_stage[kTW][2][12];
  __shared__ uint32_t s_win[kTW][kTriH / 32];
  const int tid = threadIdx.x, lane = tid & 63, wave = tid >> 6;
  const int diag = kGwDiag ? (lists_only >> 8) : 0;
  lists_only &= 1;
  if (FILL) {
    for (int i = lane; i < kTriH / 32; i += 64) s_win[wave][i] = 0u;
  }
  for (uint32_t item = blockIdx.x; item < nitems; item += gridDim.x) {
    if (item != blockIdx.x) __syncthreads();
    const TriItem it = items[item];
    const int32_t u = it.u;
    const int64_t ub = G.offsets[u], du = G.offsets[u + 1] - ub;
    const int64_t j0 = it.j0, j1 = min(du, j0 + (int64_t)kTriEB);
    const int nch = (int)((du + kTriH - 1) / kTriH);
    const int64_t hk = min(du, (int64_t)kTriH);
    int lg = 6;
    while ((1 << lg) < 2 * hk) ++lg;
    const uint32_t S = 1u << lg, smask = S - 1u;
    const int sh = 32 - lg;
    for (int ch = 0; ch < nch; ++ch) {
      const int64_t p0 = (int64_t)ch * kTriH, p1 = min(du, p0 + kTriH);
      if (ch > 0) __syncthreads();
      for (uint32_t i = tid; i < S; i += kTB) s_key[i] = -1;
      __syncthreads();
      for (int64_t i = tid; i < p1 - p0; i += kTB) {
        const int32_t x = G.nbrs[ub + p0 + i];
        uint32_t h = ((uint32_t)x * 0x9E3779B1u) >> sh;
        while (atomicCAS(&s_key[h], -1, x) != -1) h = (h + 1) & smask;
        s_pos[h] = (uint16_t)i;
      }
      __syncthreads();
      const int32_t hi = ch == nch - 1 ? INT32_MAX : G.nbrs[ub + p1 - 1];
      int64_t jp = j0 + wave;
      int32_t pv_n = jp + kTW < j1 ? G.nbrs[ub + jp + kTW] : 0;
      int32_t pv = 0;
      int64_t pvb = 0, pve = 0;
      if (jp < j1) {
        pv = G.nbrs[ub + jp];
        pvb = G.offsets[pv];
        pve = G.offsets[pv + 1];
      }
      for (int64_t j = jp; j < j1; j += kTW) {
        const int32_t v = pv;
        const int64_t vb = pvb, dv = pve - pvb;
        if (j + kTW < j1) {
          pv = pv_n;
          pvb = G.offsets[pv];
          pve = G.offsets[pv + 1];
        }
        if (j + 2 * kTW < j1) pv_n = G.nbrs[ub + j + 2 * kTW];
        const int li = (int)(j - j0);
        if (ch > 0) {
          const int32_t nx = s_nx[li];
          if (nx == kTriNotOwned || (ch + 1 < nch && nx > hi)) continue;
        }
        if (!(du > dv || (du == dv && u <= v))) {
          if (nch > 1 && lane == 0) s_nx[li] = kTriNotOwned;
          continue;
        }
        const int64_t e = ub + j;
        uint32_t cuv = 0, cvu = 0, cur = 0;
        int64_t luv = -1, lvu = -1, kp = -1;
        if (ch > 0) {
          cuv = s_cuv[li];
          cvu = s_cvu[li];
          cur = s_cur[li];
          luv = s_luv[li];
          lvu = s_lvu[li];
          kp = s_kp[li];
        }
        int64_t k = (int64_t)cur + lane;
        int32_t x = k < dv ? G.nbrs[vb + k] : INT32_MAX;
        int32_t xa[kTriAhead - 1];
#pragma unroll
        for (int r = 0; r < kTriAhead - 1; ++r) xa[r] = k + 64 * (r + 1) < dv ? G.nbrs[vb + k + 64 * (r + 1)] : INT32_MAX;
        TriSlot Tuv, Tvu;
        int64_t er = -1;
        bool vu_win = false;
        if (FILL) {
          gw_bs_nbr* en = bsn + e;
          const uint32_t c = bs_c(en, (uint32_t)dv);
          Tuv = tri_slot(en, reg, roff, e, c, (uint32_t)dv, lists_only, s_stage[wave][0], lane);
          Tuv.E.nobits = true;
          if (ch == 0) tri_prologue(Tuv, e, roff, lane);
          if (u != v) {
            const uint32_t kpv = (uint32_t)dv < GW_BS_PACK_D ? (en->r[0] & 0xFFFFu) : en->r[0];
            er = vb + kpv;
            gw_bs_nbr* enr = bsn + er;
            const uint32_t cr = bs_c(enr, (uint32_t)du);
            Tvu = tri_slot(enr, reg, roff, er, cr, (uint32_t)du, lists_only, s_stage[wave][1], lane);
            if (ch == 0) tri_prologue(Tvu, er, roff, lane);
            vu_win = !Tvu.filt && Tvu.E.mode == BS_REGION;
            Tvu.E.nobits = vu_win;
          }
        }
        int32_t nx = INT32_MAX;
        for (;;) {
          const int64_t kf = k + 64 * kTriAhead;
          const int32_t xf = kf < dv ? G.nbrs[vb + kf] : INT32_MAX;
          const bool inr = k < dv && x <= hi;
          bool hit = false;
          uint32_t pu = 0;
          if (inr) {
            uint32_t h = ((uint32_t)x * 0x9E3779B1u) >> sh;
            for (;;) {
              const int32_t kk = s_key[h];
              if (kk == x) {
                hit = true;
                pu = (uint32_t)p0 + s_pos[h];
                break;
              }
              if (kk == -1) break;
              h = (h + 1) & smask;
            }
          }
          const unsigned long long mu = __ballot(inr && x == u);
          if (mu) kp = (int64_t)cur + (__ffsll(mu) - 1);
          const bool cu = hit && x != u;
          const bool cv = hit && x != v && u != v;
          if (FILL && !(diag & 1)) {
            if (!(diag & 2) && !Tuv.filt && Tuv.E.mode == BS_REGION) {
              const unsigned long long m = __ballot(cu);
              if (m) {
                const uint32_t sh = cur & 31u;
                const unsigned long long lo = m << sh;
                const uint32_t hi3 = sh ? (uint32_t)(m >> (64 - sh)) : 0u;
                const uint32_t wv = lane == 0 ? (uint32_t)lo : lane == 1 ? (uint32_t)(lo >> 32) : hi3;
                if (lane < 3 && wv) atomicOr(&Tuv.E.bits[(cur >> 5) + lane], wv);
              }
            }
            const bool dual = u != v && Tuv.dual;
            tri_emit(Tuv, cu, k, &cuv, &luv, lane, dual ? reinterpret_cast<uint16_t*>(Tvu.E.w) : nullptr,
                     !Tuv.filt && Tuv.E.mode == BS_REGION);
            if (u != v) {
              tri_emit(Tvu, cv, (int64_t)pu, &cvu, &lvu, lane, dual ? reinterpret_cast<uint16_t*>(Tuv.E.w) : nullptr,
                       !Tvu.filt && Tvu.E.mode == BS_REGION);
              if (cv && vu_win && !(diag & 2)) atomicOr(&s_win[wave][(pu - (uint32_t)p0) >> 5], 1u << (pu & 31u));
            }
          } else if (!FILL) {
            const unsigned long long m1 = __ballot(cu), m2 = __ballot(cv);
            cuv += (uint32_t)__popcll(m1);
            cvu += (uint32_t)__popcll(m2);
          }
          const int nin = __popcll(__ballot(inr));
          cur += (uint32_t)nin;
          if (nin < 64) {
            nx = __shfl(x, nin, 64);
            break;
          }
          k += 64;
          x = xa[0];
#pragma unroll
          for (int r = 0; r < kTriAhead - 2; ++r) xa[r] = xa[r + 1];
          xa[kTriAhead - 2] = xf;
        }
        if (FILL && ch + 1 == nch) {
          tri_epilogue(Tuv, luv, cuv, cvu, lane);
          if (u != v) tri_epilogue(Tvu, lvu, cvu, cuv, lane);
        }
        if (FILL && !(diag & 4)) {
          tri_flush(Tuv, nch > 1, lane);
          if (u != v) tri_flush(Tvu, nch > 1, lane);
          if (vu_win) {
            __builtin_amdgcn_wave_barrier();
            for (int i = lane; i < kTriH / 32; i += 64) {
              const uint32_t wv = s_win[wave][i];
              if (wv) {
                Tvu.E.bits[(p0 >> 5) + i] = wv;
                s_win[wave][i] = 0u;
              }
            }
            __builtin_amdgcn_wave_barrier();
          }
        }
        if (ch + 1 < nch) {
          if (lane == 0) {
            s_cuv[li] = cuv;
            s_cvu[li] = cvu;
            s_cur[li] = cur;
            s_luv[li] = (int32_t)luv;
            s_lvu[li] = (int32_t)lvu;
            s_kp[li] = (int32_t)kp;
            s_nx[li] = nx;
          }
          continue;
        }
        if (!FILL) {
          const uint32_t k32 = kp >= 0 ? (uint32_t)kp : 0xFFFFFFFFu;
          if (lane == 0)
            tri_header(bsn + e, (uint32_t)v, (uint32_t)dv, (uint32_t)vb,
                       bs_meta_slot(cuv, u != v ? cvu : 0xFFFFu, (uint32_t)dv, (uint32_t)du), k32, cuv);
          if (lane == 1 && u != v && kp >= 0)
            tri_header(bsn + vb + kp, (uint32_t)u, (uint32_t)du, (uint32_t)ub,
                       bs_meta_slot(cvu, cuv, (uint32_t)du, (uint32_t)dv), (uint32_t)j, cvu);
        }
      }
    }
  }
}

template <int NW>
__device__ __forceinline__ int regs_select(const uint32_t* wd, uint32_t j) {
  uint32_t S = 0, T = 0, below = 0, x = wd[0];
#pragma unroll
  for (int t = 0; t < NW; ++t) {
    S += (uint32_t)__popc(wd[t]);
    const bool le = S <= j;
    T += le ? 1u : 0u;
    below = le ? S : below;
    if (t + 1 < NW) x = le ? wd[t + 1] : x;
  }
  return 32 * (int)T + word_select(x, j - below);
}

constexpr int kPW = 11;
__device__ __forceinline__ uint32_t pickw(const uint32_t (&pl)[kPW], uint32_t idx) {
  const bool b0 = idx & 1u, b1 = idx & 2u, b2 = idx & 4u, b3 = idx & 8u;
  const uint32_t a0 = b0 ? pl[1] : pl[0], a1 = b0 ? pl[3] : pl[2], a2 = b0 ? pl[5] : pl[4];
  const uint32_t a3 = b0 ? pl[7] : pl[6], a4 = b0 ? pl[9] : pl[8];
  const uint32_t c0 = b1 ? a1 : a0, c1 = b1 ? a3 : a2, c2 = b1 ? pl[10] : a4;
  const uint32_t e0 = b2 ? c1 : c0;
  return b3 ? c2 : e0;
}

__device__ __forceinline__ uint32_t bits32(const uint32_t (&pl)[kPW], uint32_t pos) {
  const uint32_t w = pos >> 5;
  return __builtin_amdgcn_alignbit(pickw(pl, w + 1), pickw(pl, w), pos & 31u);
}

__device__ __forceinline__ bool ef_bucket_has(const uint32_t (&pl)[kPW], uint32_t U, uint32_t l, uint32_t s,
                                              uint32_t e0, uint32_t k, uint32_t lw) {
  uint32_t hw = bits32(pl, s), run = 0;
  while (hw == 0xFFFFFFFFu && run < 320u) {
    run += 32u;
    hw = bits32(pl, s + run);
  }
  run += (uint32_t)__builtin_ctz(~hw);
  if (l == 0) return run > 0;
  const uint32_t mask = (1u << l) - 1u, lowk = k & mask;
  uint32_t o = 0;
  for (uint32_t i = 0; i < run; ++i) {
    if (o + l > 32u) {
      lw = bits32(pl, U + (e0 + i) * l);
      o = 0;
    }
    const uint32_t f = (lw >> o) & mask;
    if (f >= lowk) return f == lowk;
    o += l;
  }
  return false;
}

__device__ __forceinline__ bool list_has(const uint32_t (&pl)[kPW], uint32_t k, bool dual = false) {
  bool hit = false;
#pragma unroll
  for (int t = 0; t < kPW; ++t)
    hit |= (t < (int)kDualC / 2 || !dual) && ((pl[t] & 0xFFFFu) == k || (pl[t] >> 16) == k);
  return hit;
}

struct BsParams {
  double a_p, a_q;
  uint32_t k0, k1, pk0, pk1;
  uint32_t diag;
};

__device__ __forceinline__ void unpack_entry(const uint32_t (&E)[16], uint32_t* kp, uint32_t* c, uint32_t (&pl)[kPW]) {
  const bool packed = E[1] < GW_BS_PACK_D;
  *kp = packed ? (E[4] & 0xFFFFu) : E[4];
  *c = packed ? (E[4] >> 16) : E[5];
#pragma unroll
  for (int q = 0; q < kPW - 1; ++q) pl[q] = packed ? E[5 + q] : E[6 + q];
  pl[kPW - 1] = packed ? E[15] : 0u;
}

__device__ __forceinline__ uint4 coop_piece(uint64_t sec, int lane, int j) {
  const int src = 16 * j + (lane >> 2);
  const uint64_t sj = ((uint64_t)(uint32_t)__shfl((int)(uint32_t)(sec >> 32), src, 64) << 32) |
                      (uint32_t)__shfl((int)(uint32_t)sec, src, 64);
  uint4 r = make_uint4(0u, 0u, 0u, 0u);
  if (sj != 0ull) r = reinterpret_cast<const uint4*>(sj)[lane & 3];
  return r;
}

__global__ void __launch_bounds__(kB) __attribute__((amdgpu_waves_per_eu(5, 5)))
k_walk_bitset(gw_dev_graph G, BsParams P, int L, int64_t walk_begin, int64_t walk_count, int shuffle,
              int32_t* __restrict__ out, int32_t* __restrict__ lens, unsigned long long* __restrict__ counters) {
  __shared__ int32_t s_stage[kB / 64][kStage][64];
  __shared__ uint4 s_ex[kB / 64][64];
  const int lane = threadIdx.x & 63;
  const int wv = threadIdx.x >> 6;
  int32_t* stage = &s_stage[wv][0][lane];
  uint4* ex = s_ex[wv];
  const uint4* __restrict__ ents = reinterpret_cast<const uint4*>(G.bs_nbr);

  const int64_t i = (int64_t)blockIdx.x * blockDim.x + threadIdx.x;
  const bool valid = i < walk_count;
  unsigned long long my_steps = 0;
  uint32_t my_trials = 0;
  const int64_t w = walk_begin + (valid ? i : 0);
  int32_t cur = -1;
  int len = L;
  if (valid) {
    const uint64_t it = (uint64_t)w / (uint64_t)G.n;
    const uint64_t pos = (uint64_t)w % (uint64_t)G.n;
    const uint64_t sp = shuffle ? gw_feistel_perm(pos, (uint64_t)G.n, P.pk0, P.pk1, (uint32_t)it) : pos;
    cur = G.order[sp];
    len = 1;
  }
  const bool vec_ok = (L & 3) == 0;
  const uint32_t c0 = (uint32_t)w, c1 = (uint32_t)((uint64_t)w >> 32);
  stage[0] = cur;
  uint32_t trial = 0;
  uint32_t b = 0, d = 0;
  if (valid) {
    b = (uint32_t)G.offsets[cur];
    d = (uint32_t)(G.offsets[cur + 1] - G.offsets[cur]);
  }
  uint32_t c = 0, kp = 0, meta = 0;
  uint32_t pl[kPW];
#pragma unroll
  for (int t = 0; t < kPW; ++t) pl[t] = 0xFFFFFFFFu;
  uint32_t ph = 0, t = 0;
  int64_t g = 0;
  uint32_t dw0 = 0u, dw1 = 0u, kb = 0u;
  uint32_t dg_iter = 0, dg_act = 0;
  for (;;) {
    const bool active = len < L && d != 0;
    if (__ballot(active) == 0ull) break;
    if (kGwDiag && (P.diag & 64)) {
      ++dg_iter;
      dg_act += active ? 1u : 0u;
    }
    uint32_t slot = 0xFFFFFFFFu;
    bool spec = false;
    uint32_t sw = 0u, sbit = 0u;
    uint64_t sec = 0ull;
    bool isblk = false;
    bool virt = false;
    if (active) {
      const uint32_t mode = meta & 3u;
      const int efl = (int)((meta >> 2) & 31u);
      const uint32_t efU = (meta >> 7) & 511u;
      const uint32_t* hreg = G.bs_region + (uint64_t)pl[0] * kBlk;
      const int64_t ndir = bs_ndir(d);
      int64_t k = 0;
      bool acc = false;
      if (ph == 3) {
        k = kb;
        acc = true;
        ph = 0;
      } else if (ph == 1) {
        const uint32_t lo = dw0, hi = g + 1 < ndir ? dw1 : c;
        if (t < lo || t >= hi) {
          g += t < lo ? -1 : 1;
          dw0 = hreg[g];
          dw1 = g + 1 < ndir ? hreg[g + 1] : 0u;
        } else {
          t -= lo;
          ph = 2;
        }
      } else {
        const gw_u4 u = gw_philox(c0, c1, (uint32_t)len, trial, P.k0, P.k1);
        ++trial;
        int op = 0;
        uint32_t j = 0;
        if (len == 1) {
          k = (int64_t)gw_index(u.x, u.z, d);
          acc = true;
        } else {
          bool other = trial > 1;
          if (!other) {
            const double Z = (P.a_p + (double)c) + (double)((int64_t)d - 1 - (int64_t)c) * P.a_q;
            const double r = gw_u01(u.x) * Z;
            if (r < P.a_p) {
              k = kp;
              acc = true;
            } else if (r - P.a_p < (double)c) {
              j = (uint32_t)(r - P.a_p);
              if (j >= c) j = c - 1;
              op = 1;
            } else {
              other = true;
            }
          }
          if (other) {
            k = (int64_t)gw_index(u.y, u.z, d);
            op = 2;
          }
        }
        if (kGwDiag && P.diag) {
          if (op == 1 && (P.diag & 1)) {
            k = (int64_t)((uint64_t)j * (uint64_t)d / c);
            acc = true;
            op = 0;
          }
          if (op == 2 && (P.diag & 2)) {
            acc = k != (int64_t)kp;
            op = 0;
          }
        }
        bool common = false;
        const uint32_t eh = (uint32_t)k >> efl;
        const bool ef_mem = op == 2 && mode == BS_EF && eh <= efU - c;
        int pos = 0;
        if ((op == 1 && (mode == BS_INLINE || mode == BS_EF)) || (ef_mem && eh > 0)) {
          const bool inv = op == 2;
          uint32_t wp[kPW];
#pragma unroll
          for (int q = 0; q < kPW; ++q) wp[q] = inv ? ~pl[q] : pl[q];
          pos = regs_select<kPW>(wp, inv ? eh - 1 : j);
        }
        const uint32_t es = (ef_mem && eh > 0) ? (uint32_t)pos + 1u : 0u;
        const uint32_t fb = gw_bounded(u.y, bs_filt_buckets(ndir, d));
        const uint32_t wpos = mode == BS_LIST     ? 16u * j
                              : mode == BS_INLINE ? (uint32_t)k
                              : mode == BS_EF     ? efU + (op == 1 ? j : es - eh) * (uint32_t)efl
                                                  : 32u * bs_filt_word(ndir) + fb;
        const uint32_t win = bits32(pl, wpos);
        if (op == 1) {
          if (mode == BS_INLINE) {
            k = (int64_t)pos;
            acc = true;
          } else if (mode == BS_EF) {
            k = ((int64_t)(uint32_t)(pos - (int)j) << efl) | (win & ((1u << efl) - 1u));
            acc = true;
          } else if (mode == BS_LIST) {
            k = (int64_t)(win & 0xFFFFu);
            acc = true;
          } else {
            if (ndir > kPDir) {
              g = (int64_t)((float)j * (float)ndir * __builtin_amdgcn_rcpf((float)c));
              if (g >= ndir) g = ndir - 1;
              dw0 = hreg[g];
              dw1 = g + 1 < ndir ? hreg[g + 1] : 0u;
              t = j;
              ph = 1;
            } else {
              uint32_t lo = 0;
              g = 0;
#pragma unroll
              for (int q = 1; q < kPDir; ++q) {
                const uint32_t dq = (pl[1 + (q >> 1)] >> (16 * (q & 1))) & 0xFFFFu;
                const bool in = q < ndir && dq <= j;
                g += in ? 1 : 0;
                lo = in ? dq : lo;
              }
              t = j - lo;
              ph = 2;
            }
          }
        } else if (op == 2) {
          if (mode == BS_LIST) {
            common = c != 0u && list_has(pl, (uint32_t)k, (meta & kMetaDual) != 0u);
          } else if (mode == BS_INLINE) {
            common = win & 1u;
          } else if (mode == BS_EF) {
            common = ef_mem && ef_bucket_has(pl, efU, (uint32_t)efl, es, es - eh, (uint32_t)k, win);
          } else if (k != (int64_t)kp && trial < (1u << 24)) {
            if (win & 1u) {
              sw = (kGwDiag && (P.diag & 8)) ? G.bs_region[((uint32_t)k >> 5) & 0xFFFFu]
                                : hreg[(meta >> 16) * kBlk + (k >> 5)];
              sbit = (uint32_t)(k & 31);
              spec = true;
            }
          }
          acc = (k != (int64_t)kp && !common) || trial >= (1u << 24);
        }
      }
      if (ph == 2 && !acc) {
        sec = (kGwDiag && (P.diag & 4)) ? (uint64_t)(G.bs_region + kBlk * ((pl[0] + (uint32_t)g) & 0xFFFu))
                           : (uint64_t)(hreg + ((meta >> 16) + (uint32_t)g) * kBlk);
        isblk = true;
      }
      if (acc) {
        if ((meta & kMetaStash) && k == (int64_t)kp) {
          virt = true;
        } else {
          slot = b + (uint32_t)k;
          sec = (uint64_t)(ents + (uint64_t)slot * 4u);
        }
      }
    }
    const uint4 r0 = coop_piece(sec, lane, 0), r1 = coop_piece(sec, lane, 1);
    const uint4 r2 = coop_piece(sec, lane, 2), r3 = coop_piece(sec, lane, 3);
    if (spec && ((sw >> sbit) & 1u)) {
      slot = 0xFFFFFFFFu;
      sec = 0ull;
    }
    uint32_t E[16];
#pragma unroll
    for (int q = 0; q < 4; ++q) {
      __builtin_amdgcn_wave_barrier();
      if ((lane & 3) == q) {
        ex[lane >> 2] = r0;
        ex[16 + (lane >> 2)] = r1;
        ex[32 + (lane >> 2)] = r2;
        ex[48 + (lane >> 2)] = r3;
      }
      __builtin_amdgcn_wave_barrier();
      const uint4 v = ex[lane];
      E[4 * q] = v.x;
      E[4 * q + 1] = v.y;
      E[4 * q + 2] = v.z;
      E[4 * q + 3] = v.w;
    }
    __builtin_amdgcn_wave_barrier();
    if (isblk) {
      kb = (uint32_t)(g * kDirBits) + (uint32_t)regs_select<kBlk>(E, t);
      ph = 3;
    }
    if (slot != 0xFFFFFFFFu) {
      const uint32_t ou = (uint32_t)cur, od = d, ob = b, ok = slot - b;
      cur = (int32_t)E[0];
      d = E[1];
      b = E[2];
      meta = E[3];
      unpack_entry(E, &kp, &c, pl);
      if (meta & kMetaDual) {
        pl[6] = ou;
        pl[7] = od;
        pl[8] = ob;
        pl[9] = ok;
        meta |= kMetaStash;
      }
    }
    if (virt) {
      const uint32_t tc = (uint32_t)cur, td = d, tb = b, tk = kp;
      cur = (int32_t)pl[6];
      d = pl[7];
      b = pl[8];
      kp = pl[9];
      pl[6] = tc;
      pl[7] = td;
      pl[8] = tb;
      pl[9] = tk;
#pragma unroll
      for (int q = 0; q < (int)kDualC / 2; ++q) {
        const uint32_t t = pl[q];
        pl[q] = pl[q + kDualC / 2];
        pl[q + kDualC / 2] = t;
      }
      const uint32_t c_rev = (meta >> 2) & 7u;
      meta = kMetaDual | kMetaStash | (c << 2);
      c = c_rev;
    }
    const bool moved = slot != 0xFFFFFFFFu || virt;
    if (moved) {
      my_trials += trial;
      trial = 0;
    }
    bool ready = false;
    int flen = 0;
    if (moved) {
      stage[64 * (len & (kStage - 1))] = cur;
      ready = (len & (kStage - 1)) == kStage - 1;
      flen = len;
      ++len;
    }
    const unsigned long long rm = __ballot(ready);
    if (rm && !(kGwDiag && (P.diag & 32))) {
      if (vec_ok) {
        const int nready = __popcll(rm);
        int32_t* ids = reinterpret_cast<int32_t*>(ex);
        __builtin_amdgcn_wave_barrier();
        if (ready)
          ids[__builtin_amdgcn_mbcnt_hi((uint32_t)(rm >> 32), __builtin_amdgcn_mbcnt_lo((uint32_t)rm, 0u))] = lane;
        __builtin_amdgcn_wave_barrier();
        const int32_t* sw = &s_stage[wv][0][0];
        for (int j = 0; 16 * j < nready; ++j) {
          const int q = 16 * j + (lane >> 2), p4 = 4 * (lane & 3);
          const int r = ids[q < nready ? q : nready - 1];
          const int lr = __shfl(flen, r, 64);
          const int64_t ir = ((int64_t)__shfl((int)(i >> 32), r, 64) << 32) | (uint32_t)__shfl((int)i, r, 64);
          if (q < nready) {
            const int4 v = make_int4(sw[64 * p4 + r], sw[64 * (p4 + 1) + r], sw[64 * (p4 + 2) + r], sw[64 * (p4 + 3) + r]);
            *reinterpret_cast<int4*>(out + ir * (int64_t)L + (lr - (kStage - 1)) + p4) = v;
          }
        }
        __builtin_amdgcn_wave_barrier();
      } else if (ready) {
        int32_t* dst = out + i * (int64_t)L + (flen - (kStage - 1));
        for (int j = 0; j < kStage; ++j) dst[j] = stage[64 * j];
      }
    }
  }
  if (valid) {
    int32_t* row = out + i * (int64_t)L;
    const int base = len & ~(kStage - 1);
    for (int t = base; t < len; ++t) row[t] = stage[64 * (t - base)];
    for (int t = len; t < L; ++t) row[t] = -1;
    if (lens) lens[i] = len;
    my_steps = (unsigned long long)(len - 1);
  }
  if (counters) {
    for (int off = 32; off > 0; off >>= 1) {
      my_steps += __shfl_down(my_steps, off, 64);
      my_trials += __shfl_down(my_trials, off, 64);
    }
    if ((threadIdx.x & 63) == 0) {
      atomicAdd(&counters[0], my_steps);
      atomicAdd(&counters[1], my_trials);
    }
    if (kGwDiag && (P.diag & 64)) {
      unsigned long long a = dg_act;
      for (int off = 32; off > 0; off >>= 1) a += __shfl_down(a, off, 64);
      if ((threadIdx.x & 63) == 0) {
        atomicAdd(&counters[2], 64ull * dg_iter);
        atomicAdd(&counters[3], a);
      }
    }
  }
}

struct LsParams {
  double a_q, M, lo, extra, h_prev;
  uint32_t k0, k1, pk0, pk1;
};

__device__ __forceinline__ bool payload_has(const uint32_t (&pl)[kPW], uint32_t meta, uint32_t c, uint32_t k) {
  const uint32_t mode = meta & 3u;
  const uint32_t efl = (meta >> 2) & 31u, efU = (meta >> 7) & 511u;
  if (mode == BS_LIST) return list_has(pl, k, (meta & 0x8000u) != 0u);
  const uint32_t eh = k >> efl;
  uint32_t es = 0;
  if (mode == BS_EF && eh > 0) {
    uint32_t wp[kPW];
#pragma unroll
    for (int q = 0; q < kPW; ++q) wp[q] = ~pl[q];
    es = (uint32_t)regs_select<kPW>(wp, eh - 1) + 1u;
  }
  const uint32_t win = bits32(pl, mode == BS_INLINE ? k : efU + (es - eh) * efl);
  if (mode == BS_INLINE) return win & 1u;
  return eh <= efU - c && ef_bucket_has(pl, efU, efl, es, es - eh, k, win);
}

__global__ void __launch_bounds__(kB) __attribute__((amdgpu_waves_per_eu(5, 5)))
k_walk_listed(gw_dev_graph G, LsParams P, int L, int64_t walk_begin, int64_t walk_count, int shuffle,
              int32_t* __restrict__ out, int32_t* __restrict__ lens, unsigned long long* __restrict__ counters) {
  __shared__ int32_t s_stage[kB / 64][kStage][64];
  __shared__ uint4 s_ex[kB / 64][64];
  const int lane = threadIdx.x & 63;
  const int wv = threadIdx.x >> 6;
  int32_t* stage = &s_stage[wv][0][lane];
  uint4* ex = s_ex[wv];
  const uint4* __restrict__ ents = reinterpret_cast<const uint4*>(G.bs_nbr);

  const int64_t i = (int64_t)blockIdx.x * blockDim.x + threadIdx.x;
  const bool valid = i < walk_count;
  unsigned long long my_steps = 0, my_trials = 0;
  const int64_t w = walk_begin + (valid ? i : 0);
  int32_t cur = -1, prev = -1;
  int len = L;
  if (valid) {
    const uint64_t it = (uint64_t)w / (uint64_t)G.n;
    const uint64_t pos = (uint64_t)w % (uint64_t)G.n;
    const uint64_t sp = shuffle ? gw_feistel_perm(pos, (uint64_t)G.n, P.pk0, P.pk1, (uint32_t)it) : pos;
    cur = G.order[sp];
    len = 1;
  }
  const bool vec_ok = (L & 3) == 0;
  const uint32_t c0 = (uint32_t)w, c1 = (uint32_t)((uint64_t)w >> 32);
  stage[0] = cur;
  uint32_t trial = 0;
  uint32_t b = 0, d = 0, pb = 0, pd = 0;
  if (valid) {
    b = (uint32_t)G.offsets[cur];
    d = (uint32_t)(G.offsets[cur + 1] - G.offsets[cur]);
  }
  uint32_t meta = BS_REGION;
  uint32_t pl[kPW];
#pragma unroll
  for (int t = 0; t < kPW; ++t) pl[t] = 0u;
  bool pend = false;
  int32_t px = 0;
  uint32_t pdx = 0, poff = 0, pmeta = 0;
  double t = 0.0;
  bool filt = false;
  uint32_t fb = 0;
  for (;;) {
    const bool active = len < L && d != 0;
    if (__ballot(active) == 0ull) break;
    uint64_t sec = 0ull;
    uint32_t k = 0;
    bool ret = false;
    uint32_t hs = 0;
    int4 h0 = make_int4(-1, -1, -1, -1);
    if (pend) {
      hs = gw_eh_slot(px, pd);
      h0 = gw_eh_row(G.eh, pb)[hs];
    }
    if (active && !pend) {
      if (len == 1) {
        const gw_u4 u = gw_philox(c0, c1, 1u, 0u, P.k0, P.k1);
        trial = 1;
        k = gw_index(u.x, u.z, d);
      } else {
        const gw_u4 u = gw_philox(c0, c1, (uint32_t)len, trial, P.k0, P.k1);
        ++trial;
        const double A = P.M * (double)d + P.extra;
        if (P.extra > 0.0 && gw_u01(u.z) * A < P.extra) {
          ret = true;
        } else {
          k = gw_index(u.x, u.y, d);
          t = gw_u01(u.w) * P.M;
          fb = (uint32_t)(((uint64_t)u.x * kFiltL) >> 32);
        }
      }
      if (!ret) sec = (uint64_t)(ents + (uint64_t)(b + k) * 4u);
    }
    const uint4 r0 = coop_piece(sec, lane, 0), r1 = coop_piece(sec, lane, 1);
    const uint4 r2 = coop_piece(sec, lane, 2), r3 = coop_piece(sec, lane, 3);
    uint32_t E[16];
#pragma unroll
    for (int q = 0; q < 4; ++q) {
      __builtin_amdgcn_wave_barrier();
      if ((lane & 3) == q) {
        ex[lane >> 2] = r0;
        ex[16 + (lane >> 2)] = r1;
        ex[32 + (lane >> 2)] = r2;
        ex[48 + (lane >> 2)] = r3;
      }
      __builtin_amdgcn_wave_barrier();
      const uint4 v = ex[lane];
      E[4 * q] = v.x;
      E[4 * q + 1] = v.y;
      E[4 * q + 2] = v.z;
      E[4 * q + 3] = v.w;
    }
    __builtin_amdgcn_wave_barrier();
    bool acc = ret, take = false;
    if (pend) {
      const int r0 = gw_eh_scan(h0, px);
      const bool adj = r0 > 0 || (r0 < 0 && gw_eh_has_from(G.eh, pb, pd, hs, px));
      acc = t < (adj ? 1.0 : P.a_q) || trial >= (1u << 24);
      pend = false;
    } else if (sec != 0ull) {
      const int32_t next = (int32_t)E[0];
      if (len == 1) {
        acc = true;
      } else if (next == prev) {
        acc = t < P.h_prev;
      } else if (t < P.lo) {
        acc = true;
      } else if ((meta & 3u) != BS_REGION) {
        acc = t < (payload_has(pl, meta, meta >> 16, k) ? 1.0 : P.a_q);
      } else if (filt && !((pickw(pl, fb >> 5) >> (fb & 31)) & 1u)) {
        acc = t < P.a_q;
      } else if (G.eh) {
        pend = true;
        filt = false;
        px = next;
      } else {
        acc = t < (bs_has_edge(G, pb, (int64_t)pb + pd, next) ? 1.0 : P.a_q);
      }
      if (trial >= (1u << 24) && !pend) acc = true;
      take = true;
    }
    if (take && (pend || acc)) {
      uint32_t ekp, ec;
      unpack_entry(E, &ekp, &ec, pl);
      pdx = E[1];
      poff = E[2];
      pmeta = (E[3] & 0x7FFFu) | ((E[3] & kMetaDual) ? 0x8000u : 0u) | (min(ec, 0xFFFFu) << 16);
    }
    bool ready = false;
    int flen = 0;
    if (acc) {
      my_trials += trial;
      trial = 0;
      const int32_t next = ret ? prev : take ? (int32_t)E[0] : px;
      const uint32_t ob = pb, od = pd;
      prev = cur;
      pb = b;
      pd = d;
      cur = next;
      if (ret) {
        b = ob;
        d = od;
        meta = BS_REGION;
      } else {
        d = pdx;
        b = poff;
        meta = pmeta;
      }
      filt = !ret && (meta & 3u) == BS_REGION;
      stage[64 * (len & (kStage - 1))] = cur;
      ready = (len & (kStage - 1)) == kStage - 1;
      flen = len;
      ++len;
    }
    const unsigned long long rm = __ballot(ready);
    if (rm) {
      if (vec_ok) {
        const int nready = __popcll(rm);
        int32_t* ids = reinterpret_cast<int32_t*>(ex);
        __builtin_amdgcn_wave_barrier();
        if (ready)
          ids[__builtin_amdgcn_mbcnt_hi((uint32_t)(rm >> 32), __builtin_amdgcn_mbcnt_lo((uint32_t)rm, 0u))] = lane;
        __builtin_amdgcn_wave_barrier();
        const int32_t* sw = &s_stage[wv][0][0];
        for (int j = 0; 16 * j < nready; ++j) {
          const int q = 16 * j + (lane >> 2), p4 = 4 * (lane & 3);
          const int r = ids[q < nready ? q : nready - 1];
          const int lr = __shfl(flen, r, 64);
          const int64_t ir = ((int64_t)__shfl((int)(i >> 32), r, 64) << 32) | (uint32_t)__shfl((int)i, r, 64);
          if (q < nready) {
            const int4 v = make_int4(sw[64 * p4 + r], sw[64 * (p4 + 1) + r], sw[64 * (p4 + 2) + r], sw[64 * (p4 + 3) + r]);
            *reinterpret_cast<int4*>(out + ir * (int64_t)L + (lr - (kStage - 1)) + p4) = v;
          }
        }
        __builtin_amdgcn_wave_barrier();
      } else if (ready) {
        int32_t* dst = out + i * (int64_t)L + (flen - (kStage - 1));
        for (int j = 0; j < kStage; ++j) dst[j] = stage[64 * j];
      }
    }
  }
  if (valid) {
    int32_t* row = out + i * (int64_t)L;
    const int base = len & ~(kStage - 1);
    for (int t = base; t < len; ++t) row[t] = stage[64 * (t - base)];
    for (int t = len; t < L; ++t) row[t] = -1;
    if (lens) lens[i] = len;
    my_steps = (unsigned long long)(len - 1);
  }
  if (counters) {
    for (int off = 32; off > 0; off >>= 1) {
      my_steps += __shfl_down(my_steps, off, 64);
      my_trials += __shfl_down(my_trials, off, 64);
    }
    if ((threadIdx.x & 63) == 0) {
      atomicAdd(&counters[0], my_steps);
      atomicAdd(&counters[1], my_trials);
    }
  }
}

template <typename T>
int bs_alloc(gw_graph* g, T** p, int64_t count) {
  *p = nullptr;
  if (count <= 0) count = 1;
  hipError_t e = hipMalloc((void**)p, sizeof(T) * (size_t)count);
  if (e != hipSuccess) {
    g->err = std::string("hipMalloc(bitset ") + std::to_string(sizeof(T) * (size_t)count) + " B): " + hipGetErrorString(e);
    *p = nullptr;
    return GW_ERR_NOMEM;
  }
  return GW_OK;
}

template <typename T>
void bs_free(T*& p) {
  if (p) (void)hipFree(p);
  p = nullptr;
}

}

void gw_dev_bitset_release(gw_graph* g) {
  bs_free(g->d.bs_region);
  bs_free(g->d.bs_nbr);
}

__device__ __forceinline__ int64_t bs_row_of(const gw_dev_graph& G, int64_t e) {
  int64_t lo = 0, hi = G.n;
  while (lo < hi) {
    const int64_t mid = (lo + hi) >> 1;
    if (G.offsets[mid + 1] <= e)
      lo = mid + 1;
    else
      hi = mid;
  }
  return lo;
}

constexpr int kWorkChunk = 16;
__global__ void k_bs_work(gw_dev_graph G, unsigned long long* __restrict__ acc) {
  const int64_t e0 = ((int64_t)blockIdx.x * blockDim.x + threadIdx.x) * kWorkChunk;
  unsigned long long w = 0;
  if (e0 < G.nnz) {
    const int64_t e1 = e0 + kWorkChunk < G.nnz ? e0 + kWorkChunk : G.nnz;
    int64_t u = bs_row_of(G, e0);
    int64_t ue = G.offsets[u + 1];
    int64_t du = ue - G.offsets[u];
    for (int64_t e = e0; e < e1; ++e) {
      if (e >= ue) {
        u = bs_row_of(G, e);
        ue = G.offsets[u + 1];
        du = ue - G.offsets[u];
      }
      const int32_t v = G.nbrs[e];
      const int64_t dv = G.deg[v];
      if (du > dv || (du == dv && u <= v)) w += (unsigned long long)dv;
    }
  }
  for (int o = 32; o > 0; o >>= 1) w += __shfl_down(w, o, 64);
  if ((threadIdx.x & 63) == 0 && w) atomicAdd(acc, w);
}

int gw_dev_bitset_build(gw_graph* g, int64_t budget_bytes, bool lists_only) {
  gw_dev_graph& d = g->d;
  gw_dev_bitset_release(g);
  const int64_t nnz = g->nnz, n = g->n;
  if (nnz == 0) return GW_OK;
  if (nnz >= (int64_t)0xFFFFFFFF) {
    g->err = "bitset mode supports < 2^32 - 1 adjacency entries: use GW_N2V_REJECTION";
    return GW_ERR_CAPACITY;
  }
  if (nnz * (int64_t)sizeof(gw_bs_nbr) > budget_bytes) {
    g->err = "bitset entries need " + std::to_string(nnz * (int64_t)sizeof(gw_bs_nbr)) + " B; over the " +
             std::to_string(budget_bytes) + " B budget: use GW_N2V_REJECTION";
    return GW_ERR_CAPACITY;
  }
  if (g->max_degree >= ((int64_t)1 << 27)) {
    g->err = "bitset mode supports vertex degrees < 2^27: use GW_N2V_REJECTION";
    return GW_ERR_UNSUPPORTED;
  }
  int rc;
  uint64_t* sz = nullptr;
  uint64_t* roff = nullptr;
  int32_t *ids = nullptr, *order = nullptr;
  int32_t* dkey = nullptr;
  uint32_t* nit = nullptr;
  uint32_t* itoff = nullptr;
  TriItem* items = nullptr;
  void* tmp = nullptr;
  auto cleanup = [&]() {
    bs_free(sz);
    bs_free(roff);
    bs_free(ids);
    bs_free(order);
    bs_free(nit);
    bs_free(itoff);
    bs_free(items);
    bs_free(tmp);
    bs_free(dkey);
  };
  auto fail = [&](int code) {
    cleanup();
    gw_dev_bitset_release(g);
    return code;
  };
#define BS_TRY(expr)                                                 \
  do {                                                               \
    hipError_t _e = (expr);                                          \
    if (_e != hipSuccess) {                                          \
      g->err = std::string(#expr) + ": " + hipGetErrorString(_e);    \
      return fail(GW_ERR_DEVICE);                                    \
    }                                                                \
  } while (0)
  if ((rc = bs_alloc(g, &d.bs_nbr, nnz)) || (rc = bs_alloc(g, &ids, n)) ||
      (rc = bs_alloc(g, &order, n)) || (rc = bs_alloc(g, &nit, n + 1)) || (rc = bs_alloc(g, &itoff, n + 1)))
    return fail(rc);
  const unsigned gn = (unsigned)((n + kB - 1) / kB), gn1 = (unsigned)((n + 1 + kB - 1) / kB);
  BS_TRY(hipMemset(d.bs_nbr, 0, (size_t)nnz * sizeof(gw_bs_nbr)));
  k_bs_iota<<<gn, kB>>>(n, ids);
  BS_TRY(hipGetLastError());
  size_t tb = 0, tb2 = 0;
  BS_TRY(hipcub::DeviceRadixSort::SortPairsDescending(nullptr, tb, (const int32_t*)nullptr, (int32_t*)nullptr,
                                                      (const int32_t*)nullptr, (int32_t*)nullptr, (int)n));
  BS_TRY(hipcub::DeviceScan::ExclusiveSum(nullptr, tb2, nit, itoff, (int)(n + 1)));
  if ((rc = bs_alloc(g, (char**)&tmp, (int64_t)std::max(tb, tb2) + 1))) return fail(rc);
  if ((rc = bs_alloc(g, &dkey, n))) return fail(rc);
  BS_TRY(hipcub::DeviceRadixSort::SortPairsDescending(tmp, tb, d.deg, dkey, ids, order, (int)n));
  int bs_diag = 0;
  if (const char* dg = GW_DIAG_ENV("GW_DIAG_BS_FILL")) bs_diag = std::atoi(dg);
  int64_t nbig = 0;
  if (bs_diag & 8) {
    std::vector<int32_t> hk((size_t)n);
    BS_TRY(hipMemcpy(hk.data(), dkey, (size_t)n * 4, hipMemcpyDeviceToHost));
    while (nbig < n && hk[(size_t)nbig] > 64) ++nbig;
  }
  bs_free(dkey);
  k_bs_nitems<<<gn1, kB>>>(d, order, nit);
  BS_TRY(hipGetLastError());
  BS_TRY(hipcub::DeviceScan::ExclusiveSum(tmp, tb2, nit, itoff, (int)(n + 1)));
  uint32_t nitems = 0, isplit = 0;
  BS_TRY(hipMemcpy(&nitems, itoff + n, sizeof(uint32_t), hipMemcpyDeviceToHost));
  if (bs_diag & 8) BS_TRY(hipMemcpy(&isplit, itoff + nbig, sizeof(uint32_t), hipMemcpyDeviceToHost));
  if ((rc = bs_alloc(g, &items, std::max<int64_t>(nitems, 1)))) return fail(rc);
  k_bs_items<<<gn, kB>>>(d, order, itoff, items);
  BS_TRY(hipGetLastError());
  bs_free(tmp);
  bs_free(ids);
  bs_free(order);
  bs_free(nit);
  bs_free(itoff);
  auto tri = [&](bool fill, const TriItem* it, uint32_t cnt) {
    if (!cnt) return;
    const unsigned tgrid = std::min<uint32_t>(cnt, 1u << 20);
    if (fill)
      k_bs_tri<true><<<tgrid, kTB>>>(d, it, cnt, d.bs_nbr, roff, d.bs_region, (lists_only ? 1 : 0) | (bs_diag << 8));
    else
      k_bs_tri<false><<<tgrid, kTB>>>(d, it, cnt, d.bs_nbr, nullptr, nullptr, lists_only ? 1 : 0);
  };
  auto tri_all = [&](bool fill) {
    if (bs_diag & 8) {
      tri(fill, items, isplit);
      tri(fill, items + isplit, nitems - isplit);
    } else {
      tri(fill, items, nitems);
    }
  };
  tri_all(false);
  BS_TRY(hipGetLastError());
  if ((rc = bs_alloc(g, &sz, nnz + 1)) || (rc = bs_alloc(g, &roff, nnz + 1))) return fail(rc);
  const unsigned grid = (unsigned)((nnz + kB - 1) / kB);
  k_bs_sizes<<<grid, kB>>>(d, d.bs_nbr, sz, lists_only ? 1 : 0);
  BS_TRY(hipGetLastError());
  BS_TRY(hipMemset(sz + nnz, 0, sizeof(uint64_t)));
  size_t tmpb = 0;
  BS_TRY(hipcub::DeviceScan::ExclusiveSum(nullptr, tmpb, sz, roff, nnz + 1));
  if ((rc = bs_alloc(g, (char**)&tmp, (int64_t)tmpb + 1))) return fail(rc);
  BS_TRY(hipcub::DeviceScan::ExclusiveSum(tmp, tmpb, sz, roff, nnz + 1));
  BS_TRY(hipDeviceSynchronize());
  bs_free(tmp);
  bs_free(sz);
  uint64_t words = 0;
  BS_TRY(hipMemcpy(&words, roff + nnz, sizeof(uint64_t), hipMemcpyDeviceToHost));
  const int64_t need = (int64_t)words * 4 + nnz * (int64_t)sizeof(gw_bs_nbr);
  if (need > budget_bytes) {
    g->err = "per-edge bitsets need " + std::to_string(need) + " B; over the " + std::to_string(budget_bytes) +
             " B budget: use GW_N2V_REJECTION";
    return fail(GW_ERR_CAPACITY);
  }
  if (words == 0) words = 1;
  if ((rc = bs_alloc(g, &d.bs_region, (int64_t)words))) return fail(rc);
  BS_TRY(hipMemset(d.bs_region, 0, (size_t)words * 4));
  tri_all(true);
  BS_TRY(hipGetLastError());
  BS_TRY(hipDeviceSynchronize());
#undef BS_TRY
  cleanup();
  g->bitset_words = (int64_t)words;
  return GW_OK;
}

double gw_bitset_build_model_s(gw_graph* g) {
  if (g->bs_model_s >= 0.0) return g->bs_model_s;
  unsigned long long* acc = nullptr;
  if (hipMalloc((void**)&acc, sizeof(unsigned long long)) != hipSuccess) return -1.0;
  unsigned long long w = 0;
  bool ok = hipMemset(acc, 0, sizeof w) == hipSuccess;
  if (ok && g->nnz > 0) {
    const int64_t threads = (g->nnz + kWorkChunk - 1) / kWorkChunk;
    k_bs_work<<<(unsigned)((threads + kB - 1) / kB), kB>>>(g->d, acc);
    ok = hipGetLastError() == hipSuccess;
  }
  ok = ok && hipMemcpy(&w, acc, sizeof w, hipMemcpyDeviceToHost) == hipSuccess;
  (void)hipFree(acc);
  if (!ok) return -1.0;
  g->bs_model_s = 2.0 * (double)w / kBuildProbeRate + (double)g->nnz * kBuildSlotSeconds;
  return g->bs_model_s;
}

int gw_dev_walk_bitset_launch(gw_graph* g, int L, uint64_t seed, int64_t walk_begin, int64_t walk_count,
                              int shuffle, int32_t* out_dev, int32_t* len_dev, uint64_t* counters_dev,
                              void* stream) {
  BsParams P;
  P.a_p = 1.0 / g->p;
  P.a_q = 1.0 / g->q;
  P.k0 = (uint32_t)seed;
  P.k1 = (uint32_t)(seed >> 32) ^ GW_TAG_N2V_STEP;
  P.pk0 = (uint32_t)seed;
  P.pk1 = (uint32_t)(seed >> 32) ^ GW_TAG_N2V_PERM;
  const char* dg = GW_DIAG_ENV("GW_DIAG_BS");
  P.diag = dg ? (uint32_t)atoi(dg) : 0u;
  if (const char* ns = GW_DIAG_ENV("GW_DIAG_NO_STORE")) P.diag |= ns[0] == '1' ? 32u : 0u;
  const unsigned grid = (unsigned)std::max<int64_t>(1, (walk_count + kB - 1) / kB);
  k_walk_bitset<<<grid, kB, 0, (hipStream_t)stream>>>(g->d, P, L, walk_begin, walk_count, shuffle, out_dev,
                                                       len_dev, (unsigned long long*)counters_dev);
  GW_HIP_TRY(hipGetLastError());
  return GW_OK;
}

int gw_dev_walk_listed_launch(gw_graph* g, int L, uint64_t seed, int64_t walk_begin, int64_t walk_count,
                              int shuffle, int32_t* out_dev, int32_t* len_dev, uint64_t* counters_dev,
                              void* stream) {
  LsParams P;
  const double a_p = 1.0 / g->p;
  P.a_q = 1.0 / g->q;
  P.M = std::max(1.0, P.a_q);
  P.lo = std::min(1.0, P.a_q);
  P.extra = a_p > P.M ? a_p - P.M : 0.0;
  P.h_prev = std::min(a_p, P.M);
  P.k0 = (uint32_t)seed;
  P.k1 = (uint32_t)(seed >> 32) ^ GW_TAG_N2V_STEP;
  P.pk0 = (uint32_t)seed;
  P.pk1 = (uint32_t)(seed >> 32) ^ GW_TAG_N2V_PERM;
  const unsigned grid = (unsigned)std::max<int64_t>(1, (walk_count + kB - 1) / kB);
  k_walk_listed<<<grid, kB, 0, (hipStream_t)stream>>>(g->d, P, L, walk_begin, walk_count, shuffle, out_dev,
                                                       len_dev, (unsigned long long*)counters_dev);
  GW_HIP_TRY(hipGetLastError());
  return GW_OK;
}
```

### graph-embedding_amd/gwamd/_lib.py

```python
import ctypes
import os

try:
    import torch
except Exception:
    torch = None

_HERE = os.path.dirname(os.path.abspath(__file__))
LIB_PATH = os.environ.get("GW_LIB", os.path.join(_HERE, "libgraphwalk.so"))

GW_OK = 0
GW_ERR_INVALID = -1
GW_ERR_IO = -2
GW_ERR_PARSE = -3
GW_ERR_NOMEM = -4
GW_ERR_DEVICE = -5
GW_ERR_STATE = -6
GW_ERR_UNSUPPORTED = -7
GW_ERR_RANGE = -8
GW_ERR_KEY = -9
GW_ERR_ZERODIV = -10
GW_ERR_CAPACITY = -11

SEM_NX_SIMPLE = 0
SEM_JAVA_MULTI = 1
N2V_REPLAY = 0
N2V_REJECTION = 1
N2V_BITSET = 2
N2V_AUTO = 3
TOPSIM_SINGLE_SAMPLE = 0
TOPSIM_ENUMERATE = 1
TOPSIM_SINGLE_RW = 2
DOUBLE_SAMPLE = 0
DOUBLE_DEV = 1
DOUBLE_RANDOM_WALK = 2


class GraphWalkError(RuntimeError):
    def __init__(self, code, msg):
        super().__init__(f"[{code}] {msg}")
        self.code = code


class DeviceError(GraphWalkError):
    pass


class CapacityError(GraphWalkError):
    pass


class StateError(GraphWalkError):
    pass


class UnsupportedError(GraphWalkError):
    pass


class GraphInfo(ctypes.Structure):
    _fields_ = [("n", ctypes.c_int64), ("nnz", ctypes.c_int64),
                ("max_degree", ctypes.c_int64), ("edge_alias_entries", ctypes.c_int64),
                ("semantics", ctypes.c_int32), ("directed", ctypes.c_int32),
                ("weighted", ctypes.c_int32), ("device", ctypes.c_int32),
                ("sampler_bytes", ctypes.c_int64), ("n2v_mode", ctypes.c_int32), ("listed", ctypes.c_int32)]


class Options(ctypes.Structure):
    _fields_ = [("table_budget_bytes", ctypes.c_int64), ("expected_steps", ctypes.c_int64),
                ("listed", ctypes.c_int32), ("simrank_hbm_row", ctypes.c_int32),
                ("host_chunk_bytes", ctypes.c_int64), ("topsim_part_shrink", ctypes.c_int32),
                ("simrank_window", ctypes.c_int32)]


class SgnsParams(ctypes.Structure):
    _fields_ = [("struct_size", ctypes.c_int32), ("dim", ctypes.c_int32), ("window", ctypes.c_int32),
                ("negative", ctypes.c_int32), ("epochs", ctypes.c_int32), ("reserved0", ctypes.c_int32),
                ("alpha", ctypes.c_double), ("min_alpha", ctypes.c_double), ("sample", ctypes.c_double),
                ("seed", ctypes.c_uint64)]

    def __init__(self, dim=128, window=5, negative=5, epochs=5, alpha=0.025, min_alpha=0.0001, sample=1e-3, seed=0):
        super().__init__(ctypes.sizeof(SgnsParams), dim, window, negative, epochs, 0, alpha, min_alpha, sample, seed)


class SgnsStats(ctypes.Structure):
    _fields_ = [("tokens_kept", ctypes.c_int64), ("pairs", ctypes.c_int64), ("negatives", ctypes.c_int64),
                ("negatives_centre", ctypes.c_int64), ("targets_clipped", ctypes.c_int64)]

    def as_tuple(self):
        return tuple(getattr(self, f) for f, _ in self._fields_)


DEEPSIM_FALLBACK_ROW_MIN = 0
DEEPSIM_FALLBACK_POSITION = 1


class DeepSimParams(ctypes.Structure):
    _fields_ = [("struct_size", ctypes.c_int32), ("dim", ctypes.c_int32), ("window", ctypes.c_int32),
                ("batch", ctypes.c_int32), ("fallback", ctypes.c_int32), ("reserved0", ctypes.c_int32),
                ("vertex_num", ctypes.c_int64), ("learning_rate", ctypes.c_double), ("beta1", ctypes.c_double),
                ("beta2", ctypes.c_double), ("epsilon", ctypes.c_double), ("score_scale", ctypes.c_double),
                ("seed", ctypes.c_uint64)]

    def __init__(self, vertex_num=0, dim=128, window=10, batch=128, fallback=DEEPSIM_FALLBACK_ROW_MIN,
                 learning_rate=0.001, beta1=0.9, beta2=0.999, epsilon=1e-8, score_scale=1.0, seed=0):
        super().__init__(ctypes.sizeof(DeepSimParams), dim, window, batch, fallback, 0, vertex_num, learning_rate,
                         beta1, beta2, epsilon, score_scale, seed)


P = ctypes.c_void_p
I32 = ctypes.c_int32
I64 = ctypes.c_int64
U64 = ctypes.c_uint64
D = ctypes.c_double
CP = ctypes.c_char_p
PI32 = ctypes.POINTER(ctypes.c_int32)
PI64 = ctypes.POINTER(ctypes.c_int64)
PD = ctypes.POINTER(ctypes.c_double)
PP = ctypes.POINTER(ctypes.c_void_p)

SIGNATURES = {
    "gw_version": (CP, []),
    "gw_last_error": (CP, [P]),
    "gw_strerror": (CP, [ctypes.c_int]),
    "gw_device_count": (ctypes.c_int, [PI32]),
    "gw_philox4x32": (ctypes.c_int, [ctypes.c_int, P, I64, P]),
    "gw_graph_load_edgelist": (ctypes.c_int, [CP, CP, ctypes.c_int, ctypes.c_int, ctypes.c_int, I64, PP]),
    "gw_graph_from_edges": (ctypes.c_int, [I64, P, P, P, ctypes.c_int, ctypes.c_int, I64, PP]),
    "gw_graph_from_csr": (ctypes.c_int, [I64, P, P, P, P, P, ctypes.c_int, ctypes.c_int, PP]),
    "gw_graph_rmat": (ctypes.c_int, [ctypes.c_int, ctypes.c_int, D, D, D, U64, PP]),
    "gw_graph_rmat_java": (ctypes.c_int, [I64, I64, D, D, D, U64, PP]),
    "gw_graph_info": (ctypes.c_int, [P, ctypes.POINTER(GraphInfo)]),
    "gw_graph_set_options": (ctypes.c_int, [P, ctypes.POINTER(Options)]),
    "gw_graph_get_options": (ctypes.c_int, [P, ctypes.POINTER(Options)]),
    "gw_graph_export_csr": (ctypes.c_int, [P, P, P, P, P, P]),
    "gw_graph_free": (ctypes.c_int, [P]),
    "gw_graph_to_device": (ctypes.c_int, [P, ctypes.c_int]),
    "gw_n2v_prepare": (ctypes.c_int, [P, D, D, ctypes.c_int]),
    "gw_n2v_export_alias": (ctypes.c_int, [P, P, P, P, P, P]),
    "gw_alias_setup": (ctypes.c_int, [ctypes.c_int, P, I64, P, P]),
    "gw_n2v_walks_replay": (ctypes.c_int, [P, ctypes.c_int, I64, P, P, I64, P, P, PI64]),
    "gw_n2v_walks": (ctypes.c_int, [P, ctypes.c_int, U64, I64, I64, ctypes.c_int, P, P, P, P]),
    "gw_n2v_walks_host": (ctypes.c_int, [P, ctypes.c_int, U64, I64, I64, ctypes.c_int, P, P, P]),
    "gw_topsim_host": (ctypes.c_int, [P, ctypes.c_int, ctypes.c_int, ctypes.c_int, D, U64, P, I64,
                                      ctypes.c_int, P, P, P, P]),
    "gw_topsim_prepare":(ctypes.c_int, [P, ctypes.c_int, ctypes.c_int, ctypes.c_int, ctypes.c_int]),
    "gw_topsim_kernel": (ctypes.c_char_p, [P]),
    "gw_topsim_last_launches": (ctypes.c_int, [P]),
    "gw_topsim_kernel_attrs": (ctypes.c_int, [P, P, P, P]),
    "gw_topsim": (ctypes.c_int, [P, ctypes.c_int, ctypes.c_int, ctypes.c_int, D, U64, P, I64,
                                 ctypes.c_int, P, P, P, P]),
    "gw_topsim_dense": (ctypes.c_int, [P, ctypes.c_int, ctypes.c_int, ctypes.c_int, D, U64, P, I64,
                                       P, P, P]),
    "gw_topsim_sparse": (ctypes.c_int, [P, ctypes.c_int, ctypes.c_int, ctypes.c_int, D, U64, P, I64, I64,
                                        P, P, P, P, P, P, P]),
    "gw_topsim_write_text": (ctypes.c_int, [P, ctypes.c_int, ctypes.c_int, ctypes.c_int, D, U64, P, I64,
                                            ctypes.c_int, CP, CP, ctypes.c_int, P]),
    "gw_topsim_m": (ctypes.c_int, [P, ctypes.c_int, ctypes.c_int, ctypes.c_int, ctypes.c_int, D, U64, P, I64,
                                   P, P, P, P, P]),
    "gw_topsim_m_host": (ctypes.c_int, [P, ctypes.c_int, ctypes.c_int, ctypes.c_int, ctypes.c_int, D, U64, P,
                                        I64, P, P, P, P]),
    "gw_topsim_double": (ctypes.c_int, [P, ctypes.c_int, ctypes.c_int, D, U64, P, P]),
    "gw_topsim_dev": (ctypes.c_int, [P, ctypes.c_int, ctypes.c_int, ctypes.c_int, ctypes.c_int, D, U64, P, P, P]),
    "gw_double_random_walk": (ctypes.c_int, [P, ctypes.c_int, ctypes.c_int, D, U64, P, P]),
    "gw_double_sim_host": (ctypes.c_int, [P, ctypes.c_int, ctypes.c_int, ctypes.c_int, ctypes.c_int, ctypes.c_int,
                                          D, U64, P, P]),
    "gw_select_fixed_max_pq": (ctypes.c_int, [P, I64, I64, ctypes.c_int, D, P]),
    "gw_format_java_double": (ctypes.c_int, [D, ctypes.c_char_p, I64]),
    "gw_simrank_naive": (ctypes.c_int, [P, D, ctypes.c_int, P, P]),
    "gw_simrank_naive_host": (ctypes.c_int, [P, D, ctypes.c_int, P]),
    "gw_write_walks_text": (ctypes.c_int, [P, CP, P, P, I64, ctypes.c_int]),
    "gw_write_sim_text_dense": (ctypes.c_int, [CP, P, P, I64, I64, ctypes.c_int, CP, ctypes.c_int]),
    "gw_write_sim_text_topk": (ctypes.c_int, [CP, P, P, P, I64, ctypes.c_int, CP, ctypes.c_int]),
    "gw_write_sim_text_sparse": (ctypes.c_int, [CP, P, P, P, P, P, I64, I64, ctypes.c_int, CP, ctypes.c_int]),
    "gw_write_sim_text_cachemap": (ctypes.c_int, [CP, P, P, P, P, I64, ctypes.c_int, ctypes.c_int, CP]),
    "gw_sgns_create": (ctypes.c_int, [ctypes.c_int, I64, ctypes.POINTER(SgnsParams), PP]),
    "gw_sgns_free": (ctypes.c_int, [P]),
    "gw_sgns_last_error": (CP, [P]),
    "gw_sgns_build_vocab": (ctypes.c_int, [P, P, I64, ctypes.c_int]),
    "gw_sgns_train": (ctypes.c_int, [P, P, I64, ctypes.c_int, ctypes.c_int, ctypes.c_int, ctypes.c_int,
                                     ctypes.POINTER(SgnsStats), P]),
    "gw_sgns_export": (ctypes.c_int, [P, P, P, P]),
    "gw_sgns_sampler_export": (ctypes.c_int, [P, P, P, P]),
    "gw_sgns_vectors_dev": (ctypes.c_int, [P, PP, PI64]),
    "gw_sgns_auto_concurrency_for": (ctypes.c_int, [P, I64, PI32]),
    "gw_sgns_kernel_attrs": (ctypes.c_int, [P, ctypes.c_int, PI32, PI32, PI32]),
    "gw_write_word2vec_text": (ctypes.c_int, [CP, P, P, P, I64, ctypes.c_int]),
    "gw_deepsim_create": (ctypes.c_int, [ctypes.c_int, ctypes.POINTER(DeepSimParams), PP]),
    "gw_deepsim_free": (ctypes.c_int, [P]),
    "gw_deepsim_last_error": (CP, [P]),
    "gw_deepsim_set_simrank": (ctypes.c_int, [P, P, P, ctypes.c_int]),
    "gw_deepsim_set_walks": (ctypes.c_int, [P, P, I64, ctypes.c_int, P, I64]),
    "gw_deepsim_train": (ctypes.c_int, [P, I64, I64, P, P]),
    "gw_deepsim_gradients": (ctypes.c_int, [P, I64, P, P, P, P]),
    "gw_deepsim_batch": (ctypes.c_int, [P, I64, P, P, P, P, P]),
    "gw_deepsim_export": (ctypes.c_int, [P, PP, PP, PP]),
    "gw_deepsim_vectors_dev": (ctypes.c_int, [P, PP, PI64]),
    "gw_deepsim_kernel_attrs": (ctypes.c_int, [P, ctypes.c_int, ctypes.POINTER(CP), PI32, PI32, PI32, PI32]),
    "gw_write_deepsim_text": (ctypes.c_int, [CP, P, I64, ctypes.c_int]),
    "gw_comm_unique_id": (ctypes.c_int, [P]),
    "gw_comm_init": (ctypes.c_int, [P, ctypes.c_int, ctypes.c_int, ctypes.c_int, PP]),
    "gw_comm_allgather": (ctypes.c_int, [P, P, P, I64, ctypes.c_int, P]),
    "gw_comm_free": (ctypes.c_int, [P]),
    "gw_comm_last_error": (CP, [P]),
}

_lib = None


def lib():
    global _lib
    if _lib is None:
        if not os.path.exists(LIB_PATH):
            raise ImportError(
                f"libgraphwalk.so not found at {LIB_PATH}: run `python graph-embedding_amd/build.py` "
                "(there is no CPU fallback)")
        L = ctypes.CDLL(LIB_PATH)
        for name, (res, args) in SIGNATURES.items():
            f = getattr(L, name)
            f.restype = res
            f.argtypes = args
        _lib = L
    return _lib


def check(rc, handle=None, sgns=None, deepsim=None):
    if rc == GW_OK:
        return
    L = lib()
    if deepsim is not None:
        msg = L.gw_deepsim_last_error(None if deepsim is True else deepsim)
    else:
        msg = L.gw_sgns_last_error(sgns) if sgns is not None else L.gw_last_error(handle)
    msg = msg.decode(errors="replace")
    if rc == GW_ERR_INVALID:
        raise ValueError(msg)
    if rc == GW_ERR_IO:
        raise OSError(msg)
    if rc in (GW_ERR_PARSE,):
        raise ValueError(f"parse error: {msg}")
    if rc == GW_ERR_NOMEM:
        raise MemoryError(msg)
    if rc == GW_ERR_DEVICE:
        raise DeviceError(rc, msg)
    if rc == GW_ERR_STATE:
        raise StateError(rc, msg)
    if rc == GW_ERR_UNSUPPORTED:
        raise UnsupportedError(rc, msg)
    if rc == GW_ERR_RANGE:
        raise IndexError(msg)
    if rc == GW_ERR_KEY:
        raise KeyError(msg)
    if rc == GW_ERR_ZERODIV:
        raise ZeroDivisionError(msg)
    if rc == GW_ERR_CAPACITY:
        raise CapacityError(rc, msg)
    raise GraphWalkError(rc, msg)


def ptr(a):
    if a is None:
        return None
    if hasattr(a, "data_ptr"):
        return ctypes.c_void_p(a.data_ptr())
    return ctypes.c_void_p(a.ctypes.data)


def device_count():
    c = ctypes.c_int32(0)
    rc = lib().gw_device_count(ctypes.byref(c))
    return c.value if rc == GW_OK else 0
```

### include/graphwalk.h

```cpp
#ifndef GRAPHWALK_H
#define GRAPHWALK_H

#include <stdint.h>

#ifdef __cplusplus
extern "C" {
#endif

#define GW_OK 0
#define GW_ERR_INVALID (-1)
#define GW_ERR_IO (-2)
#define GW_ERR_PARSE (-3)
#define GW_ERR_NOMEM (-4)
#define GW_ERR_DEVICE (-5)
#define GW_ERR_STATE (-6)
#define GW_ERR_UNSUPPORTED (-7)
#define GW_ERR_RANGE (-8)
#define GW_ERR_KEY (-9)
#define GW_ERR_ZERODIV (-10)
#define GW_ERR_CAPACITY (-11)

#define GW_SEM_NX_SIMPLE 0
#define GW_SEM_JAVA_MULTI 1

#define GW_N2V_REPLAY 0
#define GW_N2V_REJECTION 1
#define GW_N2V_BITSET 2
#define GW_N2V_AUTO 3

#define GW_TOPSIM_SINGLE_SAMPLE 0
#define GW_TOPSIM_ENUMERATE 1
#define GW_TOPSIM_SINGLE_RW 2

typedef struct gw_graph gw_graph;

typedef struct gw_graph_info_t {
  int64_t n;
  int64_t nnz;
  int64_t max_degree;
  int64_t edge_alias_entries;
  int32_t semantics;
  int32_t directed;
  int32_t weighted;
  int32_t device;
  int64_t sampler_bytes;
  int32_t n2v_mode;
  int32_t listed;
} gw_graph_info_t;

typedef struct gw_options_t {
  int64_t table_budget_bytes;
  int64_t expected_steps;
  int32_t listed;
  int32_t simrank_hbm_row;
  int64_t host_chunk_bytes;
  int32_t topsim_part_shrink;
  int32_t simrank_window;
} gw_options_t;

typedef struct gw_topsim_stats_t {
  int64_t extensions;
  int64_t pair_updates;
  int64_t max_frontier;
  int64_t walkers;
} gw_topsim_stats_t;

const char* gw_version(void);
const char* gw_last_error(const gw_graph* g);
const char* gw_strerror(int code);
int gw_device_count(int* count);
int gw_philox4x32(int device, const uint32_t* in, int64_t n, uint32_t* out);

int gw_graph_load_edgelist(const char* path, const char* delim, int semantics,
                           int directed, int weighted, int64_t vcount,
                           gw_graph** out);
int gw_graph_from_edges(int64_t m, const int64_t* src, const int64_t* dst,
                        const double* w, int semantics, int directed,
                        int64_t vcount, gw_graph** out);
int gw_graph_from_csr(int64_t n, const int64_t* offsets, const int32_t* nbrs,
                      const double* weights, const int64_t* labels,
                      const int32_t* node_order, int semantics, int directed,
                      gw_graph** out);
int gw_graph_rmat(int scale, int edge_factor, double a, double b, double c,
                  uint64_t seed, gw_graph** out);
int gw_graph_rmat_java(int64_t n, int64_t m, double a, double b, double c,
                       uint64_t seed, gw_graph** out);
int gw_graph_info(const gw_graph* g, gw_graph_info_t* info);
int gw_graph_export_csr(const gw_graph* g, int64_t* offsets, int32_t* nbrs,
                        double* weights, int64_t* labels, int32_t* node_order);
int gw_graph_free(gw_graph* g);

int gw_graph_set_options(gw_graph* g, const gw_options_t* opt);
int gw_graph_get_options(const gw_graph* g, gw_options_t* opt);

int gw_graph_to_device(gw_graph* g, int device);

int gw_n2v_prepare(gw_graph* g, double p, double q, int mode);
int gw_n2v_export_alias(const gw_graph* g, int32_t* node_J, double* node_q,
                        int64_t* edge_off, int32_t* edge_J, double* edge_q);
int gw_alias_setup(int device, const double* probs, int64_t K, int64_t* J,
                   double* q);

int gw_n2v_walks_replay(gw_graph* g, int walk_len, int64_t nwalks,
                        const int32_t* starts, const double* uniforms,
                        int64_t n_uniforms, int32_t* out_walks, int32_t* out_len,
                        int64_t* uniforms_used);

int gw_n2v_walks(gw_graph* g, int walk_len, uint64_t seed, int64_t walk_begin,
                 int64_t walk_count, int shuffle, int32_t* out_walks_dev,
                 int32_t* out_len_dev, uint64_t* counters_dev, void* stream);

int gw_n2v_walks_host(gw_graph* g, int walk_len, uint64_t seed,
                      int64_t walk_begin, int64_t walk_count, int shuffle,
                      int32_t* out_walks, int32_t* out_len, uint64_t* counters);

int gw_topsim_prepare(gw_graph* g, int variant, int sample, int step, int topk);
const char* gw_topsim_kernel(const gw_graph* g);
int gw_topsim_last_launches(const gw_graph* g);
int gw_topsim_kernel_attrs(gw_graph* g, int32_t* vgprs, int32_t* scratch_bytes, int32_t* lds_bytes);
int gw_topsim(gw_graph* g, int variant, int sample, int step, double C,
              uint64_t seed, const int32_t* sources_dev, int64_t nsrc, int topk,
              int32_t* out_ids_dev, double* out_scores_dev, int64_t* stats_dev,
              void* stream);
int gw_topsim_dense(gw_graph* g, int variant, int sample, int step, double C,
                    uint64_t seed, const int32_t* sources_dev, int64_t nsrc,
                    double* out_rows_dev, int64_t* stats_dev, void* stream);

int gw_topsim_sparse(gw_graph* g, int variant, int sample, int step, double C,
                     uint64_t seed, const int32_t* sources_dev, int64_t nsrc,
                     int64_t capacity, int64_t* row_begin_dev,
                     int32_t* row_len_dev, int32_t* out_ids_dev,
                     double* out_scores_dev, int64_t* used_dev,
                     int64_t* stats_dev, void* stream);
int gw_topsim_write_text(gw_graph* g, int variant, int sample, int step,
                         double C, uint64_t seed, const int32_t* sources,
                         int64_t nsrc, int topk, const char* path,
                         const char* sep, int decimals, int64_t* stats);

int gw_topsim_host(gw_graph* g, int variant, int sample, int step, double C,
                   uint64_t seed, const int32_t* sources, int64_t nsrc,
                   int topk, int32_t* out_ids, double* out_scores,
                   double* out_rows, int64_t* stats);

int gw_topsim_m(gw_graph* g, int variant, int capacity, int sample, int step,
                double C, uint64_t seed, const int32_t* sources_dev, int64_t nsrc,
                int32_t* out_keys_dev, float* out_vals_dev, int32_t* out_size_dev,
                int64_t* stats_dev, void* stream);
int gw_topsim_m_host(gw_graph* g, int variant, int capacity, int sample,
                     int step, double C, uint64_t seed, const int32_t* sources,
                     int64_t nsrc, int32_t* out_keys, float* out_vals,
                     int32_t* out_size, int64_t* stats);

#define GW_DOUBLE_SAMPLE 0
#define GW_DOUBLE_DEV 1
#define GW_DOUBLE_RANDOM_WALK 2
int gw_topsim_double(gw_graph* g, int sample, int step, double C,
                     uint64_t seed, double* sim_dev, void* stream);
int gw_topsim_dev(gw_graph* g, int sample, int step, int topK, int singleStep,
                  double C, uint64_t seed, const int32_t* cand_dev,
                  double* sim_dev, void* stream);
int gw_double_random_walk(gw_graph* g, int sample, int step, double C,
                          uint64_t seed, double* sim_dev, void* stream);
int gw_double_sim_host(gw_graph* g, int kind, int sample, int step, int topK,
                       int singleStep, double C, uint64_t seed,
                       const int32_t* cand, double* sim);
int gw_select_fixed_max_pq(const double* rows, int64_t nrows, int64_t n, int k,
                           double min_score, int32_t* out_ids);
int gw_format_java_double(double v, char* buf, int64_t buflen);

int gw_simrank_naive(gw_graph* g, double C, int iters, double* sim_dev,
                     void* stream);
int gw_simrank_naive_host(gw_graph* g, double C, int iters, double* sim);

int gw_write_walks_text(const gw_graph* g, const char* path,
                        const int32_t* walks, const int32_t* lens,
                        int64_t nwalks, int walk_len);
int gw_write_sim_text_dense(const char* path, const double* rows,
                            const int32_t* row_ids, int64_t nrows, int64_t n,
                            int topk, const char* sep, int decimals);
int gw_write_sim_text_sparse(const char* path, const int64_t* row_begin,
                             const int32_t* row_len, const int32_t* ids,
                             const double* scores, const int32_t* row_ids,
                             int64_t nrows, int64_t n, int topk,
                             const char* sep, int decimals);
int gw_write_sim_text_topk(const char* path, const int32_t* ids,
                           const double* scores, const int32_t* row_ids,
                           int64_t nrows, int topk, const char* sep,
                           int decimals);

int gw_write_sim_text_cachemap(const char* path, const int32_t* keys,
                               const float* vals, const int32_t* sizes,
                               const int32_t* row_ids, int64_t nrows,
                               int capacity, int topk, const char* sep);

typedef struct gw_sgns gw_sgns;
typedef struct gw_sgns_params_t {
  int32_t struct_size;
  int32_t dim;
  int32_t window;
  int32_t negative;
  int32_t epochs;
  int32_t reserved0;
  double alpha;
  double min_alpha;
  double sample;
  uint64_t seed;
} gw_sgns_params_t;
typedef struct gw_sgns_stats_t {
  int64_t tokens_kept;
  int64_t pairs;
  int64_t negatives;
  int64_t negatives_centre;
  int64_t targets_clipped;
} gw_sgns_stats_t;
int gw_sgns_create(int device, int64_t n, const gw_sgns_params_t* params, gw_sgns** out);
int gw_sgns_free(gw_sgns* m);
const char* gw_sgns_last_error(const gw_sgns* m);
int gw_sgns_build_vocab(gw_sgns* m, const int32_t* walks, int64_t nwalks, int walk_len);
int gw_sgns_train(gw_sgns* m, const int32_t* walks, int64_t nwalks, int walk_len, int epoch_begin,
                  int epoch_count, int concurrency, gw_sgns_stats_t* stats, void* stream);
int gw_sgns_export(gw_sgns* m, float* syn0, float* syn1neg, int64_t* counts);
int gw_sgns_sampler_export(const gw_sgns* m, int32_t* J, uint32_t* thr, uint32_t* keep_thr);
int gw_sgns_vectors_dev(gw_sgns* m, float** ptr, int64_t* pitch);
int gw_sgns_auto_concurrency_for(const gw_sgns* m, int64_t nwalks, int32_t* concurrency);
int gw_sgns_kernel_attrs(gw_sgns* m, int walk_len, int32_t* vgprs, int32_t* scratch_bytes, int32_t* lds_bytes);
int gw_write_word2vec_text(const char* path, const float* syn0, const int64_t* counts, const int64_t* labels,
                           int64_t n, int dim);

#define GW_DEEPSIM_FALLBACK_ROW_MIN 0
#define GW_DEEPSIM_FALLBACK_POSITION 1
typedef struct gw_deepsim gw_deepsim;
typedef struct gw_deepsim_params_t {
  int32_t struct_size;
  int32_t dim;
  int32_t window;
  int32_t batch;
  int32_t fallback;
  int32_t reserved0;
  int64_t vertex_num;
  double learning_rate;
  double beta1;
  double beta2;
  double epsilon;
  double score_scale;
  uint64_t seed;
} gw_deepsim_params_t;
int gw_deepsim_create(int device, const gw_deepsim_params_t* params, gw_deepsim** out);
int gw_deepsim_free(gw_deepsim* m);
const char* gw_deepsim_last_error(const gw_deepsim* m);
int gw_deepsim_set_simrank(gw_deepsim* m, const int32_t* ids, const double* scores, int topk);
int gw_deepsim_set_walks(gw_deepsim* m, const int32_t* walks, int64_t nwalks, int walk_len, const int64_t* labels,
                         int64_t n_labels);
int gw_deepsim_train(gw_deepsim* m, int64_t step_begin, int64_t step_count, double* loss_out, void* stream);
int gw_deepsim_gradients(gw_deepsim* m, int64_t step, float* gw1, float* gb1, float* gw2, float* gb2);
int gw_deepsim_batch(gw_deepsim* m, int64_t step, int32_t* centre, int32_t* tgt_id, float* tgt_val, int32_t* tgt_n,
                     float* ysum);
int gw_deepsim_export(gw_deepsim* m, float* const par[4], float* const adam_m[4], float* const adam_v[4]);
int gw_deepsim_vectors_dev(gw_deepsim* m, float** ptr, int64_t* pitch);
int gw_deepsim_kernel_attrs(gw_deepsim* m, int cap, const char** names, int32_t* vgprs, int32_t* scratch_bytes,
                            int32_t* lds_bytes, int32_t* count);
int gw_write_deepsim_text(const char* path, const float* w1, int64_t n, int dim);

#define GW_COMM_ID_BYTES 128
#define GW_DTYPE_I32 0
#define GW_DTYPE_F64 1
typedef struct gw_comm gw_comm;
int gw_comm_unique_id(uint8_t* id);
int gw_comm_init(const uint8_t* id, int nranks, int rank, int device, gw_comm** out);
int gw_comm_allgather(gw_comm* c, const void* send_dev, void* recv_dev, int64_t count, int dtype, void* stream);
int gw_comm_free(gw_comm* c);
const char* gw_comm_last_error(const gw_comm* c);

#ifdef __cplusplus
}
#endif
#endif
```

Before: 34.58 billion.

## Build bitset neighbor tables in one triangle pass with raw bitmaps and encode

Adds a one-pass route for building the per-edge bitset tables. The triangle-intersection kernel writes raw adjacency bitmaps into a scratch buffer, and a new encode kernel then converts them into list, inline, Elias-Fano or region formats. This replaces the previous count pass followed by a second fill pass, so the expensive intersection runs once. It also adds a cost model for choosing between routes and a digest API for checking that both routes give the same tables. The cost is extra memory for the raw scratch buffer, with a fallback to the two-pass route when the budget is too small.

```diff
diff --git a/graph-embedding_amd/csrc/gw_capi.cpp b/graph-embedding_amd/csrc/gw_capi.cpp
--- a/graph-embedding_amd/csrc/gw_capi.cpp
+++ b/graph-embedding_amd/csrc/gw_capi.cpp
@@ -321,6 +321,15 @@
   return GW_OK;
 }
 
+int gw_n2v_table_digest(gw_graph* g, uint64_t digest[2], int32_t* route) {
+  if (!g) return gw_fail(nullptr, GW_ERR_INVALID, "NULL handle");
+  GW_GUARD_DEVICE(g, g->device);
+  if (!digest) return ret(g, gw_fail(g, GW_ERR_INVALID, "bad arguments"));
+  if (!g->n2v_prepared || !g->d.bs_nbr) return ret(g, gw_fail(g, GW_ERR_STATE, "no per-edge tables are resident"));
+  if (route) *route = g->bs_route;
+  return ret(g, gw_dev_bitset_digest(g, digest));
+}
+
 int gw_n2v_walks_replay(gw_graph* g, int walk_len, int64_t nwalks, const int32_t* starts,
                         const double* uniforms, int64_t n_uniforms, int32_t* out_walks,
                         int32_t* out_len, int64_t* uniforms_used) {
diff --git a/graph-embedding_amd/csrc/gw_internal.h b/graph-embedding_amd/csrc/gw_internal.h
--- a/graph-embedding_amd/csrc/gw_internal.h
+++ b/graph-embedding_amd/csrc/gw_internal.h
@@ -132,7 +132,10 @@
   double p = 1.0, q = 1.0;
   int64_t edge_alias_entries = 0;
   int64_t bitset_words = 0;
+  int bs_route = 0;
   double bs_model_s = -1.0;
+  double bs_model_1p_s = -1.0;
+  int64_t bs_model_raw_words = 0;
   gw_topsim_ws ts;
   double* sr_work = nullptr;
   double* sr_x = nullptr;
@@ -191,7 +194,8 @@
                     int32_t* out_size_dev, int64_t* stats_dev, void* stream);
 int gw_dev_simrank_naive(gw_graph* g, double C, int iters, double* sim_dev, void* stream);
 int gw_dev_bitset_build(gw_graph* g, int64_t budget_bytes, bool lists_only = false);
-double gw_bitset_build_model_s(gw_graph* g);
+double gw_bitset_build_model_s(gw_graph* g, bool lists_only = false);
+int gw_dev_bitset_digest(gw_graph* g, uint64_t digest[2]);
 int gw_dev_walk_bitset_launch(gw_graph* g, int L, uint64_t seed, int64_t walk_begin, int64_t walk_count,
                               int shuffle, int32_t* out_dev, int32_t* len_dev, uint64_t* counters_dev,
                               void* stream);
diff --git a/graph-embedding_amd/csrc/gw_n2v.hip b/graph-embedding_amd/csrc/gw_n2v.hip
--- a/graph-embedding_amd/csrc/gw_n2v.hip
+++ b/graph-embedding_amd/csrc/gw_n2v.hip
@@ -570,7 +570,7 @@
   if (g->opt.listed == 0) return false;
   if (g->opt.listed == 1 || g->opt.expected_steps <= 0) return true;
   const double save_s = (double)g->opt.expected_steps * (0.46 / 4.9e10);
-  const double build_s = gw_bitset_build_model_s(g);
+  const double build_s = gw_bitset_build_model_s(g, true);
   if (build_s < 0) {
     (void)hipGetLastError();
     return false;
diff --git a/graph-embedding_amd/csrc/gw_n2v_bitset.hip b/graph-embedding_amd/csrc/gw_n2v_bitset.hip
--- a/graph-embedding_amd/csrc/gw_n2v_bitset.hip
+++ b/graph-embedding_amd/csrc/gw_n2v_bitset.hip
@@ -109,6 +109,23 @@
 }
 __device__ __forceinline__ uint32_t bs_meta_slot(uint32_t c, uint32_t c_rev, uint32_t d, uint32_t du) {
   return bs_dual(c, c_rev, d, du) ? (kMetaDual | (c_rev << 2)) : bs_meta(c, d);
+}
+
+__device__ __forceinline__ void bs_ef_set(uint32_t* w, int64_t k, uint32_t idx, int l, uint32_t U) {
+  const uint32_t hp = (uint32_t)(k >> l) + idx;
+  atomicOr(&w[hp >> 5], 1u << (hp & 31));
+  if (l > 0) {
+    const uint32_t lowv = (uint32_t)k & ((1u << l) - 1u), off = U + idx * (uint32_t)l, sh = off & 31;
+    atomicOr(&w[off >> 5], lowv << sh);
+    if (sh + (uint32_t)l > 32u) atomicOr(&w[(off >> 5) + 1], lowv >> (32 - sh));
+  }
+}
+__device__ __forceinline__ void bs_filter_set(uint32_t* w, int64_t ndir, int64_t k, uint32_t d, double inv) {
+  uint32_t ulo, uhi;
+  bs_draw_range(k, d, inv, &ulo, &uhi);
+  const uint32_t F = bs_filt_buckets(ndir, d), w0 = bs_filt_word(ndir);
+  const uint32_t b0 = gw_bounded(ulo, F), b1 = gw_bounded(uhi, F);
+  for (uint32_t b = b0; b <= b1; ++b) atomicOr(&w[w0 + (b >> 5)], 1u << (b & 31));
 }
 
 struct BsEmit {
@@ -130,21 +147,11 @@
     } else if (mode == BS_INLINE) {
       atomicOr(&w[k >> 5], bit);
     } else if (mode == BS_EF) {
-      const uint32_t hp = (uint32_t)(k >> l) + idx;
-      atomicOr(&w[hp >> 5], 1u << (hp & 31));
-      if (l > 0) {
-        const uint32_t lowv = (uint32_t)k & ((1u << l) - 1u), off = U + idx * (uint32_t)l, sh = off & 31;
-        atomicOr(&w[off >> 5], lowv << sh);
-        if (sh + (uint32_t)l > 32u) atomicOr(&w[(off >> 5) + 1], lowv >> (32 - sh));
-      }
+      bs_ef_set(w, k, idx, l, U);
     } else {
       if (!nobits) atomicOr(&bits[k >> 5], bit);
       set_dir((kprev < 0 ? -1 : kprev / kDirBits) + 1, k / kDirBits, idx);
-      uint32_t ulo, uhi;
-      bs_draw_range(k, d, inv, &ulo, &uhi);
-      const uint32_t F = bs_filt_buckets(ndir, d), w0 = bs_filt_word(ndir);
-      const uint32_t b0 = gw_bounded(ulo, F), b1 = gw_bounded(uhi, F);
-      for (uint32_t b = b0; b <= b1; ++b) atomicOr(&w[w0 + (b >> 5)], 1u << (b & 31));
+      bs_filter_set(w, ndir, k, d, inv);
     }
   }
   __device__ void set_dir(int64_t g0, int64_t g1, uint32_t count) const {
@@ -208,6 +215,9 @@
 
 constexpr double kBuildProbeRate = 7.7e10;
 constexpr double kBuildSlotSeconds = 5.0e-11;
+constexpr double kBuildProbeRate1 = 8.8e10;
+constexpr double kBuildRawWordSeconds = 1.0e-11;
+constexpr double kBuildSlotSeconds1 = 1.9e-10;
 
 struct TriItem {
   int32_t u, j0;
@@ -318,7 +328,9 @@
   *cnt += (uint32_t)__popcll(m);
 }
 
-template <bool FILL>
+enum TriPass { TRI_COUNT = 0, TRI_FILL = 1, TRI_RAW = 2 };
+
+template <int PASS>
 __global__ void __launch_bounds__(kTB) __attribute__((amdgpu_waves_per_eu(4))) k_bs_tri(gw_dev_graph G, const TriItem* __restrict__ items, uint32_t nitems,
                                                 gw_bs_nbr* __restrict__ bsn,
                                                 const uint64_t* __restrict__ roff, uint32_t* __restrict__ reg,
@@ -330,10 +342,11 @@
   __shared__ int32_t s_nx[kTriEB];
   __shared__ uint32_t s_stage[kTW][2][12];
   __shared__ uint32_t s_win[kTW][kTriH / 32];
+  constexpr bool FILL = PASS == TRI_FILL, RAW = PASS == TRI_RAW;
   const int tid = threadIdx.x, lane = tid & 63, wave = tid >> 6;
   const int diag = kGwDiag ? (lists_only >> 8) : 0;
   lists_only &= 1;
-  if (FILL) {
+  if (FILL || RAW) {
     for (int i = lane; i < kTriH / 32; i += 64) s_win[wave][i] = 0u;
   }
   for (uint32_t item = blockIdx.x; item < nitems; item += gridDim.x) {
@@ -423,6 +436,12 @@
             vu_win = !Tvu.filt && Tvu.E.mode == BS_REGION;
             Tvu.E.nobits = vu_win;
           }
+        }
+        uint32_t *ruv = nullptr, *rvu = nullptr;
+        bool vu_hits = false;
+        if (RAW) {
+          ruv = reg + roff[e];
+          rvu = ruv + bs_round((dv + 31) / 32);
         }
         int32_t nx = INT32_MAX;
         for (;;) {
@@ -471,6 +490,17 @@
             const unsigned long long m1 = __ballot(cu), m2 = __ballot(cv);
             cuv += (uint32_t)__popcll(m1);
             cvu += (uint32_t)__popcll(m2);
+            if (RAW) {
+              if (m1) {
+                const uint32_t sh = cur & 31u;
+                const unsigned long long lo = m1 << sh;
+                const uint32_t hi3 = sh ? (uint32_t)(m1 >> (64 - sh)) : 0u;
+                const uint32_t wv = lane == 0 ? (uint32_t)lo : lane == 1 ? (uint32_t)(lo >> 32) : hi3;
+                if (lane < 3 && wv) atomicOr(&ruv[(cur >> 5) + lane], wv);
+              }
+              if (cv) atomicOr(&s_win[wave][(pu - (uint32_t)p0) >> 5], 1u << (pu & 31u));
+              vu_hits |= m2 != 0ull;
+            }
           }
           const int nin = __popcll(__ballot(inr));
           cur += (uint32_t)nin;
@@ -503,6 +533,16 @@
             __builtin_amdgcn_wave_barrier();
           }
         }
+        if (RAW && vu_hits) {
+          __builtin_amdgcn_wave_barrier();
+          for (int i = lane; i < (int)bs_round((p1 - p0 + 31) >> 5); i += 64) {
+            const uint32_t wv = s_win[wave][i];
+            const unsigned long long nz = __ballot(wv != 0u);
+            if ((nz >> (lane & ~(kBlk - 1))) & 0xFFFFull) rvu[(p0 >> 5) + i] = wv;
+            if (wv) s_win[wave][i] = 0u;
+          }
+          __builtin_amdgcn_wave_barrier();
+        }
         if (ch + 1 < nch) {
           if (lane == 0) {
             s_cuv[li] = cuv;
@@ -526,6 +566,192 @@
         }
       }
     }
+  }
+}
+
+__device__ __forceinline__ uint32_t wave_incl_sum(uint32_t v, int lane) {
+#pragma unroll
+  for (int o = 1; o < 64; o <<= 1) {
+    const uint32_t t = __shfl_up(v, o, 64);
+    if (lane >= o) v += t;
+  }
+  return v;
+}
+
+constexpr int kEncB = 256;
+constexpr int kEncW = 11;
+__global__ void __launch_bounds__(kEncB) k_bs_encode(gw_dev_graph G, gw_bs_nbr* __restrict__ bsn,
+                                                     const uint64_t* __restrict__ rawoff,
+                                                     const uint32_t* __restrict__ raw,
+                                                     const uint64_t* __restrict__ roff, uint32_t* __restrict__ reg) {
+  __shared__ uint32_t s_pay[kEncB / 64][64][kEncW];
+  const int lane = threadIdx.x & 63, wave = threadIdx.x >> 6;
+  const int64_t base = ((int64_t)blockIdx.x * (kEncB / 64) + wave) * 64;
+  if (base >= G.nnz) return;
+  const int64_t e = base + lane;
+  const bool valid = e < G.nnz;
+  uint32_t d = 0, meta = 0, c = 0;
+  uint64_t oa = 0, ob = 0;
+  uint32_t nwb = 0;
+  if (valid) {
+    const uint4 h = *reinterpret_cast<const uint4*>(bsn + e);
+    const uint2 r01 = *reinterpret_cast<const uint2*>(&bsn[e].r[0]);
+    d = h.y;
+    meta = h.w;
+    const bool packed = d < GW_BS_PACK_D;
+    c = packed ? r01.x >> 16 : r01.y;
+    if (d) {
+      const uint64_t na = (uint64_t)bs_round(((int64_t)d + 31) / 32);
+      const uint64_t ro = rawoff[e], rs = rawoff[e + 1] - ro;
+      if (rs) {
+        oa = ro;
+        ob = ro + na;
+        nwb = (uint32_t)(rs - na);
+      } else {
+        const uint64_t eo = (uint64_t)h.z + (packed ? (r01.x & 0xFFFFu) : r01.x);
+        const uint64_t ro2 = rawoff[eo];
+        nwb = (uint32_t)(rawoff[eo + 1] - ro2 - na);
+        ob = ro2;
+        oa = ro2 + nwb;
+      }
+    }
+  }
+  const bool dual = (meta & kMetaDual) != 0u;
+  const uint32_t c_rev = dual ? (meta & ~kMetaDual) >> 2 : 0u;
+  const bool small = d != 0u && gw_bs_is_inline(d) && (!dual || nwb <= (uint32_t)kBlk);
+  uint32_t* st = s_pay[wave][lane];
+#pragma unroll
+  for (int t = 0; t < kEncW; ++t) st[t] = 0u;
+  if (small) {
+    const uint4* pa = reinterpret_cast<const uint4*>(raw + oa);
+    uint32_t wa[12];
+#pragma unroll
+    for (int t = 0; t < 3; ++t) {
+      const uint4 q = pa[t];
+      wa[4 * t] = q.x;
+      wa[4 * t + 1] = q.y;
+      wa[4 * t + 2] = q.z;
+      wa[4 * t + 3] = q.w;
+    }
+    if (!gw_bs_is_list(c, d)) {
+#pragma unroll
+      for (int t = 0; t < kEncW; ++t) st[t] = wa[t];
+    } else {
+      uint16_t* hw = reinterpret_cast<uint16_t*>(st);
+      const uint32_t own = dual ? kDualC : 2u * (uint32_t)kEncW;
+      uint32_t idx = 0;
+#pragma unroll
+      for (int t = 0; t < kEncW; ++t) {
+        for (uint32_t w = wa[t]; w; w &= w - 1u) {
+          if (idx < own) hw[idx] = (uint16_t)(32 * t + __builtin_ctz(w));
+          ++idx;
+        }
+      }
+      for (; idx < own; ++idx) hw[idx] = 0xFFFFu;
+      if (dual) {
+        const uint4* pb = reinterpret_cast<const uint4*>(raw + ob);
+        idx = 0;
+        for (int t = 0; t < kBlk / 4; ++t) {
+          const uint4 q = pb[t];
+          const uint32_t wq[4] = {q.x, q.y, q.z, q.w};
+#pragma unroll
+          for (int s = 0; s < 4; ++s) {
+            for (uint32_t w = wq[s]; w; w &= w - 1u) {
+              if (idx < kDualC) hw[kDualC + idx] = (uint16_t)(32 * (4 * t + s) + __builtin_ctz(w));
+              ++idx;
+            }
+          }
+        }
+        for (; idx < kDualC; ++idx) hw[kDualC + idx] = 0xFFFFu;
+      }
+    }
+  }
+  __builtin_amdgcn_wave_barrier();
+  for (unsigned long long bm = __ballot(d != 0u && !small); bm; bm &= bm - 1ull) {
+    const int sl = __ffsll(bm) - 1;
+    const uint32_t sd = (uint32_t)__shfl((int)d, sl, 64), sc = (uint32_t)__shfl((int)c, sl, 64);
+    const uint32_t smeta = (uint32_t)__shfl((int)meta, sl, 64), snwb = (uint32_t)__shfl((int)nwb, sl, 64);
+    const uint64_t soa = ((uint64_t)(uint32_t)__shfl((int)(uint32_t)(oa >> 32), sl, 64) << 32) |
+                         (uint32_t)__shfl((int)(uint32_t)oa, sl, 64);
+    const uint64_t sob = ((uint64_t)(uint32_t)__shfl((int)(uint32_t)(ob >> 32), sl, 64) << 32) |
+                         (uint32_t)__shfl((int)(uint32_t)ob, sl, 64);
+    const int64_t se = base + sl;
+    const bool sdual = (smeta & kMetaDual) != 0u;
+    const int mode = sdual ? BS_LIST : bs_mode(sc, sd);
+    uint32_t* pay = s_pay[wave][sl] + (sd < GW_BS_PACK_D ? 0 : 1);
+    if (sd >= GW_BS_PACK_D && lane == 0) s_pay[wave][sl][0] = sc;
+    uint16_t* hw = reinterpret_cast<uint16_t*>(pay);
+    const uint32_t nw = (sd + 31u) / 32u, nwr = (uint32_t)bs_round(nw);
+    const int64_t ndir = bs_ndir(sd);
+    const uint32_t own = sdual ? kDualC : 2u * gw_bs_pw(sd);
+    int l = 0;
+    uint32_t U = 0;
+    uint32_t *dir = nullptr, *bits = nullptr;
+    const double inv = bs_inv32(sd);
+    if (mode == BS_EF) {
+      l = gw_bs_ef_l(sc, sd);
+      U = sc + ((sd - 1) >> l) + 1;
+    } else if (mode == BS_REGION) {
+      const uint64_t r0 = roff[se];
+      dir = reg + r0;
+      bits = dir + bs_boff(sd);
+      if (lane == 0) pay[0] = (uint32_t)(r0 / kBlk);
+      if (ndir > kPDir)
+        for (int64_t g = ndir + lane; g < bs_boff(sd); g += 64) dir[g] = 0u;
+    }
+    __builtin_amdgcn_wave_barrier();
+    const uint32_t* pa = raw + soa;
+    uint32_t cnt = 0;
+    for (uint32_t i0 = 0; i0 < (mode == BS_REGION ? nwr : nw); i0 += 64) {
+      const uint32_t i = i0 + lane;
+      uint32_t w = i < nwr ? pa[i] : 0u;
+      if (mode == BS_REGION && i < nwr) bits[i] = w;
+      const uint32_t pc = (uint32_t)__popc(w);
+      const uint32_t incl = wave_incl_sum(pc, lane);
+      uint32_t idx = cnt + incl - pc;
+      if (mode == BS_REGION && ndir > 0 && (i & (uint32_t)(kBlk - 1)) == 0u && i < nw) {
+        if (ndir <= kPDir)
+          hw[2 + (i >> 4)] = (uint16_t)idx;
+        else
+          dir[i >> 4] = idx;
+      }
+      for (; w; w &= w - 1u, ++idx) {
+        const int64_t k = 32 * (int64_t)i + __builtin_ctz(w);
+        if (mode == BS_LIST) {
+          if (idx < own) hw[idx] = (uint16_t)k;
+        } else if (mode == BS_EF) {
+          if (idx < sc) bs_ef_set(pay, k, idx, l, U);
+        } else {
+          bs_filter_set(pay, ndir, k, sd, inv);
+        }
+      }
+      cnt += (uint32_t)__shfl((int)incl, 63, 64);
+    }
+    if (mode == BS_LIST) {
+      if ((uint32_t)lane >= cnt && (uint32_t)lane < own) hw[lane] = 0xFFFFu;
+      if (sdual) {
+        const uint32_t* pb = raw + sob;
+        uint32_t cb = 0;
+        for (uint32_t i0 = 0; i0 < snwb; i0 += 64) {
+          const uint32_t i = i0 + lane;
+          uint32_t w = i < snwb ? pb[i] : 0u;
+          const uint32_t pc = (uint32_t)__popc(w);
+          const uint32_t incl = wave_incl_sum(pc, lane);
+          uint32_t idx = cb + incl - pc;
+          for (; w; w &= w - 1u, ++idx)
+            if (idx < kDualC) hw[kDualC + idx] = (uint16_t)(32u * i + (uint32_t)__builtin_ctz(w));
+          cb += (uint32_t)__shfl((int)incl, 63, 64);
+        }
+        if ((uint32_t)lane >= cb && (uint32_t)lane < kDualC) hw[kDualC + lane] = 0xFFFFu;
+      }
+    }
+    __builtin_amdgcn_wave_barrier();
+  }
+  uint32_t* ew = reinterpret_cast<uint32_t*>(bsn + base);
+  const int nsl = (int)min((int64_t)64, G.nnz - base);
+  for (int i = lane; i < nsl * kEncW; i += 64) {
+    const int s = i / kEncW, t = i - s * kEncW;
+    ew[16 * s + 5 + t] = s_pay[wave][s][t];
   }
 }
 
@@ -1191,6 +1417,40 @@
 void gw_dev_bitset_release(gw_graph* g) {
   bs_free(g->d.bs_region);
   bs_free(g->d.bs_nbr);
+  g->bs_route = GW_BS_ROUTE_NONE;
+}
+
+__global__ void k_bs_digest(const uint32_t* __restrict__ a, uint64_t nwords, unsigned long long* __restrict__ acc) {
+  unsigned long long s = 0;
+  for (uint64_t i = (uint64_t)blockIdx.x * blockDim.x + threadIdx.x; i < nwords; i += (uint64_t)gridDim.x * blockDim.x) {
+    uint64_t z = (i + 1) * 0x9E3779B97F4A7C15ull + (uint64_t)a[i];
+    z = (z ^ (z >> 30)) * 0xBF58476D1CE4E5B9ull;
+    z = (z ^ (z >> 27)) * 0x94D049BB133111EBull;
+    s += z ^ (z >> 31);
+  }
+  for (int o = 32; o > 0; o >>= 1) s += __shfl_down(s, o, 64);
+  if ((threadIdx.x & 63) == 0) atomicAdd(acc, s);
+}
+
+int gw_dev_bitset_digest(gw_graph* g, uint64_t digest[2]) {
+  unsigned long long* acc = nullptr;
+  GW_HIP_TRY(hipMalloc((void**)&acc, 2 * sizeof(unsigned long long)));
+  hipError_t e = hipMemset(acc, 0, 2 * sizeof(unsigned long long));
+  const uint64_t nw[2] = {(uint64_t)g->nnz * (sizeof(gw_bs_nbr) / 4), g->d.bs_region ? (uint64_t)g->bitset_words : 0ull};
+  const uint32_t* src[2] = {reinterpret_cast<const uint32_t*>(g->d.bs_nbr), g->d.bs_region};
+  for (int t = 0; t < 2 && e == hipSuccess; ++t) {
+    if (!nw[t]) continue;
+    const unsigned grid = (unsigned)std::min<uint64_t>((nw[t] + kB - 1) / kB, 1u << 16);
+    k_bs_digest<<<grid, kB>>>(src[t], nw[t], acc + t);
+    e = hipGetLastError();
+  }
+  unsigned long long h[2] = {0, 0};
+  if (e == hipSuccess) e = hipMemcpy(h, acc, sizeof h, hipMemcpyDeviceToHost);
+  (void)hipFree(acc);
+  GW_HIP_TRY(e);
+  digest[0] = h[0];
+  digest[1] = h[1];
+  return GW_OK;
 }
 
 __device__ __forceinline__ int64_t bs_row_of(const gw_dev_graph& G, int64_t e) {
@@ -1208,7 +1468,7 @@
 constexpr int kWorkChunk = 16;
 __global__ void k_bs_work(gw_dev_graph G, unsigned long long* __restrict__ acc) {
   const int64_t e0 = ((int64_t)blockIdx.x * blockDim.x + threadIdx.x) * kWorkChunk;
-  unsigned long long w = 0;
+  unsigned long long w = 0, r = 0;
   if (e0 < G.nnz) {
     const int64_t e1 = e0 + kWorkChunk < G.nnz ? e0 + kWorkChunk : G.nnz;
     int64_t u = bs_row_of(G, e0);
@@ -1222,11 +1482,41 @@
       }
       const int32_t v = G.nbrs[e];
       const int64_t dv = G.deg[v];
-      if (du > dv || (du == dv && u <= v)) w += (unsigned long long)dv;
-    }
-  }
-  for (int o = 32; o > 0; o >>= 1) w += __shfl_down(w, o, 64);
-  if ((threadIdx.x & 63) == 0 && w) atomicAdd(acc, w);
+      if (du > dv || (du == dv && u <= v)) {
+        w += (unsigned long long)dv;
+        r += (unsigned long long)(bs_round((dv + 31) / 32) + (u != v ? bs_round((du + 31) / 32) : 0));
+      }
+    }
+  }
+  for (int o = 32; o > 0; o >>= 1) {
+    w += __shfl_down(w, o, 64);
+    r += __shfl_down(r, o, 64);
+  }
+  if ((threadIdx.x & 63) == 0 && w) {
+    atomicAdd(acc, w);
+    atomicAdd(acc + 1, r);
+  }
+}
+
+constexpr int kRawChunk = 16;
+__global__ void k_bs_rawsz(gw_dev_graph G, uint64_t* __restrict__ sz) {
+  const int64_t e0 = ((int64_t)blockIdx.x * blockDim.x + threadIdx.x) * kRawChunk;
+  if (e0 >= G.nnz) return;
+  const int64_t e1 = e0 + kRawChunk < G.nnz ? e0 + kRawChunk : G.nnz;
+  int64_t u = bs_row_of(G, e0);
+  int64_t ue = G.offsets[u + 1];
+  int64_t du = ue - G.offsets[u];
+  for (int64_t e = e0; e < e1; ++e) {
+    if (e >= ue) {
+      u = bs_row_of(G, e);
+      ue = G.offsets[u + 1];
+      du = ue - G.offsets[u];
+    }
+    const int32_t v = G.nbrs[e];
+    const int64_t dv = G.deg[v];
+    const bool own = du > dv || (du == dv && u <= v);
+    sz[e] = own ? (uint64_t)(bs_round((dv + 31) / 32) + (u != v ? bs_round((du + 31) / 32) : 0)) : 0ull;
+  }
 }
 
 int gw_dev_bitset_build(gw_graph* g, int64_t budget_bytes, bool lists_only) {
@@ -1256,7 +1546,11 @@
   uint32_t* itoff = nullptr;
   TriItem* items = nullptr;
   void* tmp = nullptr;
+  uint64_t* rawoff = nullptr;
+  uint32_t* raw = nullptr;
   auto cleanup = [&]() {
+    bs_free(raw);
+    bs_free(rawoff);
     bs_free(sz);
     bs_free(roff);
     bs_free(ids);
@@ -1280,6 +1574,32 @@
       return fail(GW_ERR_DEVICE);                                    \
     }                                                                \
   } while (0)
+  const char* dg = GW_DIAG_ENV("GW_DIAG_BS_FILL");
+  bool onepass = false;
+  if (!lists_only && !dg && gw_bitset_build_model_s(g) >= 0.0 &&
+      nnz * (int64_t)sizeof(gw_bs_nbr) + 2 * g->bs_model_raw_words * 4 <= budget_bytes) {
+    const int64_t rawwords = g->bs_model_raw_words;
+    if (bs_alloc(g, &raw, rawwords) == GW_OK) {
+      BS_TRY(hipMemset(raw, 0, (size_t)rawwords * 4));
+      if ((rc = bs_alloc(g, &sz, nnz + 1)) || (rc = bs_alloc(g, &rawoff, nnz + 1))) return fail(rc);
+      const int64_t rthreads = (nnz + kRawChunk - 1) / kRawChunk;
+      k_bs_rawsz<<<(unsigned)((rthreads + kB - 1) / kB), kB>>>(d, sz);
+      BS_TRY(hipGetLastError());
+      BS_TRY(hipMemset(sz + nnz, 0, sizeof(uint64_t)));
+      size_t rb = 0;
+      BS_TRY(hipcub::DeviceScan::ExclusiveSum(nullptr, rb, sz, rawoff, nnz + 1));
+      if ((rc = bs_alloc(g, (char**)&tmp, (int64_t)rb + 1))) return fail(rc);
+      BS_TRY(hipcub::DeviceScan::ExclusiveSum(tmp, rb, sz, rawoff, nnz + 1));
+      BS_TRY(hipDeviceSynchronize());
+      bs_free(tmp);
+      bs_free(sz);
+      onepass = true;
+    } else {
+      (void)hipGetLastError();
+      g->err.clear();
+    }
+  }
+  (void)hipGetLastError();
   if ((rc = bs_alloc(g, &d.bs_nbr, nnz)) || (rc = bs_alloc(g, &ids, n)) ||
       (rc = bs_alloc(g, &order, n)) || (rc = bs_alloc(g, &nit, n + 1)) || (rc = bs_alloc(g, &itoff, n + 1)))
     return fail(rc);
@@ -1294,8 +1614,7 @@
   if ((rc = bs_alloc(g, (char**)&tmp, (int64_t)std::max(tb, tb2) + 1))) return fail(rc);
   if ((rc = bs_alloc(g, &dkey, n))) return fail(rc);
   BS_TRY(hipcub::DeviceRadixSort::SortPairsDescending(tmp, tb, d.deg, dkey, ids, order, (int)n));
-  int bs_diag = 0;
-  if (const char* dg = GW_DIAG_ENV("GW_DIAG_BS_FILL")) bs_diag = std::atoi(dg);
+  const int bs_diag = dg ? std::atoi(dg) : 0;
   int64_t nbig = 0;
   if (bs_diag & 8) {
     std::vector<int32_t> hk((size_t)n);
@@ -1317,26 +1636,28 @@
   bs_free(order);
   bs_free(nit);
   bs_free(itoff);
-  auto tri = [&](bool fill, const TriItem* it, uint32_t cnt) {
+  const unsigned grid = (unsigned)((nnz + kB - 1) / kB);
+  auto tri = [&](int pass, const TriItem* it, uint32_t cnt) {
     if (!cnt) return;
     const unsigned tgrid = std::min<uint32_t>(cnt, 1u << 20);
-    if (fill)
-      k_bs_tri<true><<<tgrid, kTB>>>(d, it, cnt, d.bs_nbr, roff, d.bs_region, (lists_only ? 1 : 0) | (bs_diag << 8));
+    if (pass == TRI_FILL)
+      k_bs_tri<TRI_FILL><<<tgrid, kTB>>>(d, it, cnt, d.bs_nbr, roff, d.bs_region, (lists_only ? 1 : 0) | (bs_diag << 8));
+    else if (pass == TRI_RAW)
+      k_bs_tri<TRI_RAW><<<tgrid, kTB>>>(d, it, cnt, d.bs_nbr, rawoff, raw, 0);
     else
-      k_bs_tri<false><<<tgrid, kTB>>>(d, it, cnt, d.bs_nbr, nullptr, nullptr, lists_only ? 1 : 0);
+      k_bs_tri<TRI_COUNT><<<tgrid, kTB>>>(d, it, cnt, d.bs_nbr, nullptr, nullptr, lists_only ? 1 : 0);
   };
-  auto tri_all = [&](bool fill) {
+  auto tri_all = [&](int pass) {
     if (bs_diag & 8) {
-      tri(fill, items, isplit);
-      tri(fill, items + isplit, nitems - isplit);
+      tri(pass, items, isplit);
+      tri(pass, items + isplit, nitems - isplit);
     } else {
-      tri(fill, items, nitems);
+      tri(pass, items, nitems);
     }
   };
-  tri_all(false);
+  tri_all(onepass ? TRI_RAW : TRI_COUNT);
   BS_TRY(hipGetLastError());
   if ((rc = bs_alloc(g, &sz, nnz + 1)) || (rc = bs_alloc(g, &roff, nnz + 1))) return fail(rc);
-  const unsigned grid = (unsigned)((nnz + kB - 1) / kB);
   k_bs_sizes<<<grid, kB>>>(d, d.bs_nbr, sz, lists_only ? 1 : 0);
   BS_TRY(hipGetLastError());
   BS_TRY(hipMemset(sz + nnz, 0, sizeof(uint64_t)));
@@ -1355,34 +1676,71 @@
              " B budget: use GW_N2V_REJECTION";
     return fail(GW_ERR_CAPACITY);
   }
-  if (words == 0) words = 1;
-  if ((rc = bs_alloc(g, &d.bs_region, (int64_t)words))) return fail(rc);
-  BS_TRY(hipMemset(d.bs_region, 0, (size_t)words * 4));
-  tri_all(true);
+  const bool noregion = words == 0;
+  if (noregion) words = 1;
+  if (onepass && bs_alloc(g, &d.bs_region, (int64_t)words) != GW_OK) {
+    (void)hipGetLastError();
+    g->err.clear();
+    bs_free(raw);
+    bs_free(rawoff);
+    onepass = false;
+  }
+  if (onepass) {
+    if (noregion) BS_TRY(hipMemset(d.bs_region, 0, 4));
+    k_bs_encode<<<(unsigned)((nnz + kEncB - 1) / kEncB), kEncB>>>(d, d.bs_nbr, rawoff, raw, roff, d.bs_region);
+    BS_TRY(hipGetLastError());
+    BS_TRY(hipDeviceSynchronize());
+    bs_free(raw);
+    bs_free(rawoff);
+    uint32_t* moved = nullptr;
+    if (bs_alloc(g, &moved, (int64_t)words) == GW_OK) {
+      BS_TRY(hipMemcpy(moved, d.bs_region, (size_t)words * 4, hipMemcpyDeviceToDevice));
+      bs_free(d.bs_region);
+      d.bs_region = moved;
+    } else {
+      (void)hipGetLastError();
+      g->err.clear();
+    }
+  } else {
+    if ((rc = bs_alloc(g, &d.bs_region, (int64_t)words))) return fail(rc);
+    BS_TRY(hipMemset(d.bs_region, 0, (size_t)words * 4));
+    tri_all(TRI_FILL);
+  }
   BS_TRY(hipGetLastError());
   BS_TRY(hipDeviceSynchronize());
 #undef BS_TRY
   cleanup();
   g->bitset_words = (int64_t)words;
+  g->bs_route = onepass ? GW_BS_ROUTE_ONEPASS : GW_BS_ROUTE_TWOPASS;
   return GW_OK;
 }
 
-double gw_bitset_build_model_s(gw_graph* g) {
-  if (g->bs_model_s >= 0.0) return g->bs_model_s;
+static double bs_model_pick(gw_graph* g, bool lists_only) {
+  size_t fr = 0, tot = 0;
+  int64_t budget = hipMemGetInfo(&fr, &tot) == hipSuccess ? (int64_t)(fr / 2) : 0;
+  if (g->opt.table_budget_bytes > 0) budget = std::min(budget, g->opt.table_budget_bytes);
+  const bool onepass = !lists_only && g->nnz * (int64_t)sizeof(gw_bs_nbr) + 2 * g->bs_model_raw_words * 4 <= budget;
+  return onepass ? g->bs_model_1p_s : g->bs_model_s;
+}
+double gw_bitset_build_model_s(gw_graph* g, bool lists_only) {
+  if (g->bs_model_s >= 0.0) return bs_model_pick(g, lists_only);
   unsigned long long* acc = nullptr;
-  if (hipMalloc((void**)&acc, sizeof(unsigned long long)) != hipSuccess) return -1.0;
-  unsigned long long w = 0;
+  if (hipMalloc((void**)&acc, 2 * sizeof(unsigned long long)) != hipSuccess) return -1.0;
+  unsigned long long w[2] = {0, 0};
   bool ok = hipMemset(acc, 0, sizeof w) == hipSuccess;
   if (ok && g->nnz > 0) {
     const int64_t threads = (g->nnz + kWorkChunk - 1) / kWorkChunk;
     k_bs_work<<<(unsigned)((threads + kB - 1) / kB), kB>>>(g->d, acc);
     ok = hipGetLastError() == hipSuccess;
   }
-  ok = ok && hipMemcpy(&w, acc, sizeof w, hipMemcpyDeviceToHost) == hipSuccess;
+  ok = ok && hipMemcpy(w, acc, sizeof w, hipMemcpyDeviceToHost) == hipSuccess;
   (void)hipFree(acc);
   if (!ok) return -1.0;
-  g->bs_model_s = 2.0 * (double)w / kBuildProbeRate + (double)g->nnz * kBuildSlotSeconds;
-  return g->bs_model_s;
+  g->bs_model_raw_words = (int64_t)w[1];
+  g->bs_model_1p_s = (double)w[0] / kBuildProbeRate1 + (double)w[1] * kBuildRawWordSeconds +
+                     (double)g->nnz * kBuildSlotSeconds1;
+  g->bs_model_s = 2.0 * (double)w[0] / kBuildProbeRate + (double)g->nnz * kBuildSlotSeconds;
+  return bs_model_pick(g, lists_only);
 }
 
 int gw_dev_walk_bitset_launch(gw_graph* g, int L, uint64_t seed, int64_t walk_begin, int64_t walk_count,
diff --git a/graph-embedding_amd/gwamd/_lib.py b/graph-embedding_amd/gwamd/_lib.py
--- a/graph-embedding_amd/gwamd/_lib.py
+++ b/graph-embedding_amd/gwamd/_lib.py
@@ -137,6 +137,7 @@
     "gw_graph_free": (ctypes.c_int, [P]),
     "gw_graph_to_device": (ctypes.c_int, [P, ctypes.c_int]),
     "gw_n2v_prepare": (ctypes.c_int, [P, D, D, ctypes.c_int]),
+    "gw_n2v_table_digest": (ctypes.c_int, [P, P, PI32]),
     "gw_n2v_export_alias": (ctypes.c_int, [P, P, P, P, P, P]),
     "gw_alias_setup": (ctypes.c_int, [ctypes.c_int, P, I64, P, P]),
     "gw_n2v_walks_replay": (ctypes.c_int, [P, ctypes.c_int, I64, P, P, I64, P, P, PI64]),
diff --git a/include/graphwalk.h b/include/graphwalk.h
--- a/include/graphwalk.h
+++ b/include/graphwalk.h
@@ -96,6 +96,10 @@
 int gw_graph_to_device(gw_graph* g, int device);
 
 int gw_n2v_prepare(gw_graph* g, double p, double q, int mode);
+#define GW_BS_ROUTE_NONE 0
+#define GW_BS_ROUTE_ONEPASS 1
+#define GW_BS_ROUTE_TWOPASS 2
+int gw_n2v_table_digest(gw_graph* g, uint64_t digest[2], int32_t* route);
 int gw_n2v_export_alias(const gw_graph* g, int32_t* node_J, double* node_q,
                         int64_t* edge_off, int32_t* edge_J, double* edge_q);
 int gw_alias_setup(int device, const double* probs, int64_t K, int64_t* J,
```

Result: slower. 33.65 billion (-2.7%).
